# baaivision/Painter

Measured on AMD Instinct MI355X. Metric: images/sec (896x448 pairs) ViT-L fwd+bwd, higher is better.
Workload: dtype bf16; 1 GPU; painter_vit_large_patch16_input896x448 bf16 batch=8/GPU fwd+bwd on 1xMI355X (BASELINE configs[1]); global_batch=8, image=896x448x3 stitched pair, mode=train (DropPath 0.1), parallelism=dp1, rccl_ranks=0, backend=n/a, grad_allreduce=n/a

## Files before the change

### include/painter_hip.h

```cpp
#ifndef PAINTER_HIP_H
#define PAINTER_HIP_H

#include <stdint.h>

#ifdef __cplusplus
extern "C" {
#endif

#ifndef __HIP__
typedef struct ihipStream_t* hipStream_t;
#endif

enum { PA_F32 = 0, PA_BF16 = 1 };
enum {
    PA_EPI_BIAS = 0,
    PA_EPI_BIAS_F32 = 1,
    PA_EPI_BIAS_GELU = 2,
    PA_EPI_BIAS_RESID = 3
};

#define PA_ABI_VERSION 9
int pa_abi_version(void);
int pa_debug_set(int which, int value);
int pa_debug_get(int which);

int pa_linear_fwd(int dtype, int epilogue, const void* x , int64_t ldx, const void* w ,
                  const float* bias , void* out, void* out2, int64_t ldo, const float* resid ,
                  const float* rowscale , int rows_per_sample, int M, int N, int K,
                  hipStream_t stream);
int pa_linear_fwd_skip(int dtype, int epilogue, const void* x, int64_t ldx, const void* w, const float* bias, void* out, void* out2,
                       int64_t ldo, const float* resid, const float* rowscale, int rows_per_sample, int M, int N, int K,
                       const float* rowskip, int skip_rows_per_sample, hipStream_t stream);
int pa_linear_pixshuf(int dtype, const void* x, int64_t ldx, const void* w , const float* bias,
                      void* out_nhwc, int batch, int Hp, int Wp, int P, int C, int K, hipStream_t stream);
int64_t pa_linear_dgrad_workspace_bytes(int M, int K);
int pa_linear_dgrad(int dtype, const void* dy , int64_t lddy, const void* w ,
                    const void* gelu_aux , void* dx , int64_t lddx, float* dx_colsum,
                    void* workspace, int M, int N, int K, hipStream_t stream);
int pa_linear_dgrad_skip(int dtype, const void* dy, int64_t lddy, const void* w, const void* gelu_aux, void* dx, int64_t lddx, float* dx_colsum,
                         void* workspace, int M, int N, int K, const float* rowskip , int skip_rows_per_sample,
                         hipStream_t stream);
int64_t pa_linear_wgrad_workspace_bytes(int dtype, int M, int N, int K);
int pa_linear_wgrad(int dtype, const void* dy , int64_t lddy, const void* x , int64_t ldx,
                    float* dw , void* workspace, int M, int N, int K, hipStream_t stream);
int64_t pa_colsum_workspace_bytes(int M, int N);
int pa_colsum(int dtype, const void* x , int64_t ld, int M, int N, float* out , void* workspace,
              hipStream_t stream);
int pa_slab_reduce(const float* in, float* out, int64_t n, int nz, int64_t stride, int accumulate, hipStream_t stream);

int pa_layernorm_fwd(int dtype, const float* x, int64_t ldx, const float* gamma, const float* beta, float eps,
                     void* y , int64_t ldy, float* mean, float* rstd,
                     int R, int D, hipStream_t stream);
int64_t pa_layernorm_bwd_workspace_bytes(int R, int D);
int pa_layernorm_bwd(int dtype, const void* dy, int64_t lddy, const float* x, int64_t ldx, const float* mean,
                     const float* rstd, const float* gamma, const float* dres, float* dx, int64_t lddx, void* dxT,
                     int64_t lddxT, const float* rowscale, int rows_per_sample, float* dgamma_dbeta, float* dxT_colsum,
                     void* workspace, int R, int D, hipStream_t stream);
int pa_layernorm_bwd_reduce(const void* workspace, float* dgamma_dbeta, float* dxT_colsum, int with_colsum, int R, int D,
                            hipStream_t stream);

int pa_relpos_rows_padded(int Hp, int Wp);
int pa_relpos_pack(int dtype, const float* rel_pos_h, const float* rel_pos_w, void* rcat, int Hp, int Wp, int head_dim,
                   hipStream_t stream);
int pa_relpos_pack_batch(int dtype, const void* tabs, void* rcat, void* rcatT, int nblocks, int Hp, int Wp, int head_dim, hipStream_t stream);
int64_t pa_attn_tables_bytes(int dtype, int batch, int L, int heads, int Hp, int Wp, int head_dim);
int pa_attn_set_generation(int generation);
int pa_attn_launch_counts(long long* out6);
int pa_attn_trace(int enable, unsigned long long* host_out);
int pa_attn_fwd(int dtype, const void* qkv, int64_t ldq, const void* rcat, void* out, int64_t ldo, float* lse,
                void* tables, int batch, int L, int heads, int Hp, int Wp, int head_dim, float scale, hipStream_t stream);
int pa_attn_fwd_skip(int dtype, const void* qkv, int64_t ldq, const void* rcat, void* out, int64_t ldo, float* lse,
                     void* tables, int batch, int L, int heads, int Hp, int Wp, int head_dim, float scale, const float* rowskip ,
                     hipStream_t stream);

int pa_relpos_pack_t(int dtype, const float* rel_pos_h, const float* rel_pos_w, void* rcatT, int Hp, int Wp, int head_dim,
                     hipStream_t stream);
int pa_attn_bwd_delta(int dtype, const void* out, int64_t ldo, const void* dout, int64_t lddo, float* delta, int batch,
                      int L, int heads, int head_dim, hipStream_t stream);
int pa_attn_bwd_prep_ok(int dtype, int L, int Hp, int Wp, int head_dim);
int pa_attn_bwd_prep(int dtype, const void* out, int64_t ldo, const void* dout, int64_t lddo, const float* lse, void* tables,
                     int batch, int L, int heads, int Hp, int Wp, int head_dim, float scale, hipStream_t stream);
int64_t pa_attn_bwd_aux_bytes(int batch, int L, int heads, int Hp, int Wp);
int64_t pa_attn_bwd_relpos_partials_bytes(int dtype, int batch, int L, int heads, int Hp, int Wp, int head_dim);
int pa_attn_bwd(int dtype, const void* qkv, int64_t ldq, const void* rcat, const void* rcatT, const void* dout,
                int64_t lddo, const float* lse, const float* delta, void* dqkv, void* dG, void* relpos_part, void* aux,
                void* tables, const void* out, int64_t ldo, int batch, int L, int heads, int Hp, int Wp, int head_dim, float scale,
                hipStream_t stream);
int pa_attn_bwd_skip(int dtype, const void* qkv, int64_t ldq, const void* rcat, const void* rcatT, const void* dout,
                     int64_t lddo, const float* lse, const float* delta, void* dqkv, void* dG, void* relpos_part, void* aux,
                     void* tables, const void* out, int64_t ldo, int batch, int L, int heads, int Hp, int Wp, int head_dim, float scale,
                     const float* rowskip , hipStream_t stream);
int64_t pa_attn_bwd_relpos_workspace_bytes(int dtype, int batch, int L, int heads, int Hp, int Wp, int head_dim);
int pa_attn_bwd_relpos_reduce(const void* relpos_part, float* drcat, void* workspace, int batch, int L, int heads, int Hp, int Wp,
                              int head_dim, hipStream_t stream);
int pa_attn_bwd_relpos(int dtype, const void* dG, const void* qkv, int64_t ldq, float* drcat, void* workspace,
                       int batch, int L, int heads, int Hp, int Wp, int head_dim, hipStream_t stream);

int pa_patch_weight_pack(int dtype, const float* w , void* out , int D, int P, hipStream_t stream);
int pa_patch_embed_fwd(int dtype, const float* imgs, const float* tgts, const void* w, int64_t ldw, const float* bias,
                       const float* mask_token, const float* seg_x, const float* seg_y, const float* pos,
                       const unsigned char* mask, int mask_batch_stride, const float* type_cls, const float* type_ins,
                       const float* seg_type, float* tokens, int batch, int Hp, int Wp, int P, int D, hipStream_t stream);
int pa_patch_cols_ok(int batch, int L, int P, int D);
int pa_patch_im2col(const float* imgs, const float* tgts, void* cols, int batch, int Hp, int Wp, int P, hipStream_t stream);
int pa_patch_embed_fwd_cols(const void* cols, const void* w , int64_t ldw, const float* bias, const float* mask_token,
                            const float* seg_x, const float* seg_y, const float* pos, const unsigned char* mask, int mask_batch_stride,
                            const float* type_cls, const float* type_ins, const float* seg_type, float* tokens, int batch, int L, int K,
                            int D, hipStream_t stream);
int64_t pa_patch_embed_wgrad_workspace_bytes(int D, int P);
int pa_patch_embed_wgrad(int dtype, const void* dpe , const float* imgs, const float* tgts,
                         float* dw , void* workspace, int batch, int Hp, int Wp, int P, int D,
                         hipStream_t stream);
int pa_patch_embed_dgrad(int dtype, const void* dpe, const void* w, int64_t ldw, float* dimgs, float* dtgts, const float* addend,
                         float alpha, int batch, int Hp, int Wp, int P, int D, hipStream_t stream);
int pa_pos_fwd(const int* idx , const float* val , int K, const float* pe , float* pos , int L, int D,
               hipStream_t stream);
int pa_pos_bwd(const int* idxT , const float* valT , int KT, const float* gx , const float* gy ,
               float* dpe , int S, int D, hipStream_t stream);
int pa_tokens_bwd(int dtype, const float* dx0, const unsigned char* mask, int mask_batch_stride, void* dpe, float* sums,
                  int batch, int L, int D, hipStream_t stream);

int pa_merge_fwd(const float* x, float* out, int64_t n_out, hipStream_t stream);
int pa_merge_bwd(int dtype, const float* dmerged, float* dx, void* dxT, const float* rowscale, int rows_per_sample,
                 int64_t rows_half, int D, hipStream_t stream);
int pa_scale_cast(int dtype, const float* in, void* out, const float* rowscale, int rows_per_sample, int64_t rows, int D,
                  hipStream_t stream);
int pa_cast_bf16(const float* in, void* out, int64_t n, hipStream_t stream);
int pa_debug_rmw(const float* src, float* scratch, int64_t n, int passes, int nblocks, hipStream_t stream);
int pa_ensemble_resid(const float* x0, const float* a, float* x1, int batch, int group, int L, int D, hipStream_t stream);

int pa_conv3x3_pack(int dtype, const float* w3 , void* w3r , void* wf ,
                    hipStream_t stream);
int pa_decoder_tail_fwd(int dtype, const void* x_nhwc, const void* w3r, const float* b3, const float* ln_gamma,
                        const float* ln_beta, const float* w1 , const float* b1, void* y3 ,
                        float* pred , int batch, int Hi, int Wi, float eps, hipStream_t stream);
int64_t pa_decoder_tail_bwd_workspace_bytes(int batch, int Hi, int Wi);
int pa_decoder_tail_bwd_pointwise(int dtype, const float* dpred, const void* y3, const float* ln_gamma,
                                  const float* ln_beta, const float* w1, void* dy3, float* grads, void* workspace,
                                  int batch, int Hi, int Wi, float eps, hipStream_t stream);
int pa_conv3x3_dgrad_unshuffle(int dtype, const void* dy3, const void* wf, void* dE, int batch, int Hp, int Wp, int P,
                               hipStream_t stream);
int64_t pa_conv3x3_wgrad_workspace_bytes(int batch, int Hi, int Wi);
int pa_conv3x3_wgrad(int dtype, const void* dy3, const void* x_nhwc, float* dw , void* workspace,
                     int batch, int Hi, int Wi, hipStream_t stream);

int pa_live_rows_max(void);
int pa_live_rows(const unsigned char* mask, int mask_batch_stride, int* rowmap, int* live, int* count, int batch, int Hp, int Wp,
                 hipStream_t stream);
int pa_conv3x3_dgrad_unshuffle_live(const void* dy3, const void* wf, void* dE_compact, const int* rowmap, const int* count, int batch,
                                    int Hp, int Wp, int P, hipStream_t stream);
int pa_gather_rows(const void* src, int64_t src_row_bytes, void* dst, int64_t dst_row_bytes, int64_t row_bytes, const int* live,
                   const int* count, int M, hipStream_t stream);
int pa_linear_dgrad_live(const void* dy, int64_t lddy, const void* w, void* dx, int64_t lddx, const int* live, const int* rowmap,
                         const int* count, int M, int N, int K, hipStream_t stream);
int pa_linear_wgrad_live(const void* dy, int64_t lddy, const void* x, int64_t ldx, float* dw, const int* count, int M, int N, int K,
                         hipStream_t stream);
int pa_colsum_live(int dtype, const void* x, int64_t ld, int M, int N, float* out, void* workspace, const int* count, hipStream_t stream);
int pa_fill_dead_rows(void* x, int64_t pitch_bytes, int64_t row_bytes, const int* rowmap, int M, hipStream_t stream);
int pa_decoder_live_ok(int dtype, int batch, int Hp, int Wp, int P, int Kin);

int64_t pa_loss_workspace_bytes(int batch, int Hi, int Wi);
int pa_loss_fwd(const float* pred, const float* tgts, float* valid, const unsigned char* mask, int mask_batch_stride,
                float* out, void* workspace, int batch, int Hi, int Wi, int P, int ignore_rule, float eps_den, int kind,
                float beta, hipStream_t stream);
int pa_loss_bwd(const float* pred, const float* tgts, const float* valid, const unsigned char* mask,
                int mask_batch_stride, const float* dloss, const float* loss_out, float* dpred, int batch, int Hi, int Wi,
                int P, int kind, float beta, hipStream_t stream);
int pa_patchify(const float* img, float* out, int batch, int Hp, int Wp, int P, hipStream_t stream);
int pa_pred_bwd(const float* pred, const float* tgts, const float* valid, const unsigned char* mask, int mask_batch_stride,
                const float* dloss, const float* loss_out, const float* dpatch, float* dpred, float* dpred_loss, int batch, int Hi,
                int Wi, int P, int kind, float beta, hipStream_t stream);

typedef struct PaOptTensor {
    void* p; const void* g; void* m; void* v;
    void* w16;
    int64_t n;
    int32_t group;
    int32_t first_chunk;
} PaOptTensor;
typedef struct PaOptGroups {
    float lr[64], wd[64];
} PaOptGroups;
int pa_opt_chunk_elems(void);
int64_t pa_grad_sumsq_workspace_bytes(int nchunks);
int pa_grad_sumsq(const PaOptTensor* table, int ntensors, int nchunks, float* out2, void* workspace, hipStream_t stream);
int pa_adamw_step(const PaOptTensor* table, int ntensors, int nchunks, const PaOptGroups* groups, double beta1, double beta2,
                  float eps, float* steps, const float* norm_info, const float* grad_scale, const float* found_inf,
                  float max_norm, hipStream_t stream);

int pa_resample_u8(const void* src, int src_h, int src_w, void* dst, int dst_h, int dst_w, int channels, const void* bounds,
                   const void* coeffs, int ksize, int vertical, hipStream_t stream);
int pa_gather_u8(const void* src, int src_h, int src_w, void* dst, int dst_h, int dst_w, int channels, const void* ytab,
                 const void* xtab, hipStream_t stream);
int pa_seggpt_stitch(const void* prompts, const void* targets, const void* target_div, const void* query, float* imgs,
                     float* tgts, int n_prompts, int res_h, int res_w, hipStream_t stream);
int pa_seggpt_decode(const float* pred, void* out_f64, int res_h, int res_w, int patch, hipStream_t stream);
int pa_seggpt_mask(const float* pred, void* out_u8, int res_h, int res_w, int patch, hipStream_t stream);
int pa_seggpt_blend(const float* pred, const void* image, void* out, int out_h, int out_w, const void* ytab, const void* xtab,
                    int res_h, int res_w, int patch, hipStream_t stream);

int pa_resample_u8_box(const void* src, int64_t src_row_bytes, int src_h, int src_w, void* dst, int dst_h, int dst_w, int channels,
                       const void* bounds, const void* coeffs, int ksize, int vertical, hipStream_t stream);
int pa_gather_u8_box(const void* src, int64_t src_row_bytes, int src_h, int src_w, void* dst, int dst_h, int dst_w, int channels,
                     const void* ytab, const void* xtab, hipStream_t stream);
int64_t pa_color_jitter_workspace_bytes(int batch);
int pa_color_jitter(void* images, const void* ops, const void* factors, const void* ops_host, void* workspace, int batch, int h, int w,
                    hipStream_t stream);
int pa_to_tensor_normalize(const void* images, const void* flip, float* canvas, int batch, int h, int w, int canvas_h, int row0,
                           hipStream_t stream);
int pa_resized_crop_f32(const float* src, float* dst, const void* boxes, int batch, int channels, int h, int w, int nearest,
                        hipStream_t stream);
int pa_resized_crop_f32_modes(const float* src, float* dst, const void* boxes, const void* modes, int batch, int channels, int h, int w,
                              hipStream_t stream);
typedef struct pa_crop_job {
    const void* src;
    void* dst;
    const void* xbounds;
    const void* xcoeffs;
    const void* ybounds;
    const void* ycoeffs;
    int64_t src_row_bytes;
    int32_t h, w;
    int32_t xksize, yksize;
    int32_t nearest;
    int32_t mid_row0;
} pa_crop_job;
int pa_resized_crop_u8_batch(const pa_crop_job* jobs, void* mid, int n_jobs, int max_h, int max_w, int out_h, int out_w, hipStream_t stream);
int64_t pa_pair_valid_workspace_bytes(int batch);
int pa_pair_valid(const float* tgts, float* valid, const void* modes, const void* thres, void* workspace, int batch, int plane,
                  hipStream_t stream);

int pa_painter_stitch(const void* prompt, const void* prompt_target, const void* queries, float* imgs, float* tgts, int n_queries,
                      int res_h, int res_w, hipStream_t stream);
typedef struct pa_decode_job {
    void* out;
    void* out2;
    int32_t sample;
    int32_t out_h, out_w;
    int32_t reserved;
} pa_decode_job;
int pa_painter_decode_u8(const float* pred, const pa_decode_job* jobs, int n_jobs, int n_samples, int max_h, int max_w, int res_h,
                         int res_w, int patch, int nearest, hipStream_t stream);
int pa_painter_decode_depth(const float* pred, const pa_decode_job* jobs, int n_jobs, int n_samples, int max_h, int max_w, int res_h,
                            int res_w, int patch, hipStream_t stream);
int pa_painter_decode_f64(const float* pred, const pa_decode_job* jobs, int n_jobs, int n_samples, int max_h, int max_w, int res_h,
                          int res_w, int patch, hipStream_t stream);
int pa_palette_argmin(const void* image, const float* palette, void* out_i32, int h, int w, int n_colours, int dist_type,
                      hipStream_t stream);
int64_t pa_inst_workspace_bytes(int h, int w, int n_colours, int n_thr, int nms_pre);
int64_t pa_inst_workspace_offset(int h, int w, int n_colours, int n_thr, int nms_pre, int section);
int pa_inst_stats(const void* image, const float* palette, const float* thresholds, void* n_u32, void* s_u64, int h, int w, int n_colours,
                  int n_thr, hipStream_t stream);
int pa_inst_intersections(const void* masks_u32, int n_rows, int words, void* inter_i32, int ld, hipStream_t stream);
int pa_inst_decode(const void* image, const float* palette, const float* thresholds, int h, int w, int n_colours, int n_thr, int nms_pre,
                   int max_num, float sigma, int kernel, void* workspace, void* out_count, float* out_scores, void* out_scores_f64,
                   void* out_candidates, void* out_masks, void* out_masks_u8, hipStream_t stream);

typedef struct pa_pano_segment {
    int id;
    int isthing;
    int category_id;
    int instance_id;
    int area;
    float score;
} pa_pano_segment;
int64_t pa_pano_workspace_bytes(int h, int w, int n_colours, int n_things, int max_inst);
int pa_pack_mask_bits(const void* masks_u8, int n_rows, int h, int w, void* out_u32, hipStream_t stream);
int pa_pano_vote(const void* image, const float* palette, const void* masks_u32, const void* n_dev, int h, int w, int n_colours, int n_things,
                 int dist_type, int max_inst, void* out_s_u64, void* out_classes, hipStream_t stream);
int pa_pano_merge(const void* semmap_i32, const void* masks_u32, const float* scores, const void* classes_i32, const void* n_dev, int h, int w,
                  int n_colours, int n_things, int max_inst, double overlap_threshold, double stuff_area_thresh, double instances_score_thresh,
                  void* workspace, void* out_panoptic, void* out_rgb, void* out_count, void* out_segments, hipStream_t stream);
int pa_pano_decode(const void* image, const float* palette, const void* masks_u32, const float* scores, const void* n_dev,
                   const void* classes_i32, int h, int w, int n_colours, int n_things, int dist_type, int max_inst, double overlap_threshold,
                   double stuff_area_thresh, double instances_score_thresh, void* workspace, void* out_panoptic, void* out_rgb, void* out_count,
                   void* out_segments, void* out_classes, hipStream_t stream);

int64_t pa_pose_workspace_bytes(int n, int n_keypoints);
int pa_pose_keypoints(const void* pictures, const void* flipped, const void* palette_i32, const void* pair_i32, int n, int h, int w,
                      int n_keypoints, int shift, void* workspace, float* out_preds, float* out_maxvals, hipStream_t stream);
int pa_pose_heatmaps(const void* pictures, const void* flipped, const void* palette_i32, const void* pair_i32, int n, int h, int w,
                     int n_keypoints, int shift, float* out_heatmaps, hipStream_t stream);

typedef struct pa_score_job {
    const void* picture;
    const void* gt;
    int32_t h, w;
} pa_score_job;
int pa_semseg_lds_bins(int n_colours);
int pa_semseg_confusion(const pa_score_job* jobs, int n_jobs, int64_t total_pixels, const float* palette, int n_colours, int dist_type,
                        int ignore_label, int bins, void* conf_i64, void* invalid_i64, hipStream_t stream);
typedef struct pa_depth_job {
// ... 50 lines not shown
```

### painter_amd/csrc/attn3.h

```cpp
#pragma once
#include "common.h"
bool attn3_ok(int L, int Hp, int Wp);
int64_t attn3_table_bytes(int Bn, int L, int H, int Hp, int Wp);
int attn3_fwd(const bf16* qkv, int64_t ldq, const bf16* rcat, bf16* out, int64_t ldo, float* lse, void* tables, int Bn, int L, int H,
              int Hp, int Wp, float scale, hipStream_t st, const float* rowskip = nullptr);
int attn3_bwd(const bf16* qkv, int64_t ldq, const bf16* rcatT, const bf16* dout, int64_t lddo, const float* lse, const float* delta,
              void* tables, bf16* dqkv, bf16* dG, float* part, int Bn, int L, int H, int Hp, int Wp, float scale, const bf16* out, int64_t ldo,
              hipStream_t st, const float* rowskip = nullptr);
int attn3_bwd_prep(const bf16* out, int64_t ldo, const bf16* dout, int64_t lddo, const float* lse, void* tables, int Bn, int L, int H, int Hp,
                   float scale, hipStream_t st);
int64_t attn3_relpos_partials_bytes(int Bn, int L, int H, int Hp, int Wp);
int attn3_relpos_reduce(const float* part, float* drcat, float* tmp, int Bn, int L, int H, int Hp, int Wp, hipStream_t st);
```

### painter_amd/csrc/attn3.hip

```cpp
#include "attn3_common.h"
#include "../../include/painter_hip.h"
#include "attn3.h"
#include <cstdlib>

#ifndef A3_PRIO
#define A3_PRIO 0
#endif
#ifndef A3_HOIST
#define A3_HOIST 1
#endif
#ifndef A3_NDL
#define A3_NDL true
#endif
#define A3_PRIO_UP() do { if (A3_PRIO) __builtin_amdgcn_s_setprio(1); } while (0)
#define A3_PRIO_DOWN() do { if (A3_PRIO) __builtin_amdgcn_s_setprio(0); } while (0)

namespace a3 {

template <int STAGES, bool SKIP = false>
__global__ __launch_bounds__(NT, STAGES == 1 ? 4 : 2) void fwd_kernel(const bf16* __restrict__ qkv, size_t ldq, const bf16* __restrict__ rcat,
                                                                      bf16* __restrict__ out, size_t ldo, float* __restrict__ lse,
                                                                      unsigned char* __restrict__ tables, int L, int H, int Hp, int NRP,
                                                                      float scale, int nblk, int xcd_map, int abl, const float* __restrict__ rowskip) {
    extern __shared__ __attribute__((aligned(16))) unsigned char smem[];
// ... 4 lines not shown
    else wg_coords(nblk, xcd_map, blk, bh, (L / 32) / NW);
    const int b = bh / H, h = bh % H, D = H * ATT_HD;
    const bf16* base = qkv + (size_t)b * L * ldq + h * ATT_HD;
    const bf16* kbase = base + D;
    const bf16* vbase = base + 2 * D;
    const int qt = blk * NW + wave;
    const bool valid = qt * 32 < L && !drop;
    const int q = qt * 32 + ql;
    const int ntile = L / 32;
    unsigned char* thT = smem + STAGES * STAGE_QK + wave * Hp * 64;
    unsigned char* eimg = smem + STAGES * STAGE_QK + NW * Hp * 64;
    unsigned char* twimg = eimg + wave * 2048;
    LaneAddr la;
    la.init(lane);
    EAddr ea;
    ea.init(lane);
    Stager ks, vs;
    ks.load(kbase, ldq, tid);
    vs.load(vbase, ldq, tid);

    bf16x8 qf[4];
    uint4 T0 = zero4(), T1 = zero4();
    if (valid) {
#pragma unroll
        for (int s = 0; s < 4; ++s) qf[s] = gfrag(base + (size_t)q * ldq, s, g);
        if (!(abl & 32)) build_tables3(twimg, thT, rcat, NRP, qf, q / WP, q % WP, Hp, 1.f / scale, lane, smem + tid * 2);
        T0 = *reinterpret_cast<const uint4*>(twimg + ql * 64 + 16 * g);
        T1 = *reinterpret_cast<const uint4*>(twimg + ql * 64 + 32 + 16 * g);
        if (tables != nullptr) {
            unsigned char* tt = tables + ((size_t)bh * ntile + qt) * ttile_bytes(Hp);
#pragma unroll
            for (int i = 0; i < 2; ++i) *reinterpret_cast<uint4*>(tt + (lane + 64 * i) * 16) = *reinterpret_cast<const uint4*>(twimg + (lane + 64 * i) * 16);
            for (int c = lane; c < Hp * 4; c += 64) *reinterpret_cast<uint4*>(tt + 2048 + c * 16) = *reinterpret_cast<const uint4*>(thT + c * 16);
        }
    }
    __syncthreads();
    build_eimg(eimg, tid);
    ks.store(smem, tid);
    vs.store(smem + IMG, tid);
    __syncthreads();

    f32x16 oacc[2];
    oacc[0] = zero16();
    oacc[1] = zero16();
    float m = 0.f, l = 0.f;
    const float sl = scale * LOG2E_F;
    const unsigned char* thw = thT + ql * 2;

    auto body = [&](auto pc, int a) {
        constexpr int P = decltype(pc)::value;
        const int j = a * PH + P;
        {
            const int jn = min(j + 1, ntile - 1);
            ks.load(kbase + (size_t)jn * 32 * ldq, ldq, tid);
            vs.load(vbase + (size_t)jn * 32 * ldq, ldq, tid);
        }
        const unsigned char* kimg = smem + (STAGES == 2 ? (j & 1) * STAGE_QK : 0);
        const unsigned char* vimg = kimg + IMG;
        if (valid) {
            const unsigned char* thr = thw + a * (RPP * 64);
            if constexpr (P == 0) win_set<0>(T1.w, thr);
            win_set<(P + 1) & 1>(T1.w, thr + (P + 1) * 64);
            const unsigned char* ei = eimg + P * EIMG;
            const bf16x8 ef0 = efrag(ei, ea, 0), ef1 = efrag(ei, ea, 1);
            bf16x8 kfr[4];
#pragma unroll
            for (int s = 0; s < 4; ++s) kfr[s] = rowfrag(kimg, la, s);
            __builtin_amdgcn_sched_barrier(0);
            f32x16 sacc = zero16();
            A3_PRIO_UP();
            sacc = mfma(ef0, as_frag(T0), sacc);
            sacc = mfma(ef1, as_frag(T1), sacc);
#pragma unroll
            for (int s = 0; s < 4; ++s) sacc = mfma(kfr[s], qf[s], sacc);
            A3_PRIO_DOWN();
            bf16x8 vtr[2][2];
            vtr[0][0] = trfrag(vimg, la, 0, 0);
            vtr[0][1] = trfrag(vimg, la, 0, 1);
            if constexpr (STAGES == 2) { vtr[1][0] = trfrag(vimg, la, 1, 0); vtr[1][1] = trfrag(vimg, la, 1, 1); }
            __builtin_amdgcn_sched_barrier(0);
            float p[16];
            const float nm = -m;
#pragma unroll
            for (int r = 0; r < 16; ++r) p[r] = fmaf(sacc[r], sl, nm);
            float tmax = max16(p);
            tmax = fmaxf(tmax, xor32(tmax));
            if (j == 0 || __any(tmax > THR)) {
                const float delta = (j == 0) ? tmax : fmaxf(tmax, 0.f);
                const float alpha = __builtin_amdgcn_exp2f(-delta);
                m += delta;
                l *= alpha;
#pragma unroll
                for (int r = 0; r < 16; ++r) { oacc[0][r] *= alpha; oacc[1][r] *= alpha; p[r] -= delta; }
            }
#pragma unroll
            for (int r = 0; r < 16; ++r) p[r] = __builtin_amdgcn_exp2f(p[r]);
            l += sum16(p);
            const bf16x8 pf0 = packfrag(p), pf1 = packfrag(p + 8);
            if constexpr (STAGES == 1) { vtr[1][0] = trfrag(vimg, la, 1, 0); vtr[1][1] = trfrag(vimg, la, 1, 1); }
            A3_PRIO_UP();
#pragma unroll
            for (int db = 0; db < 2; ++db) {
                oacc[db] = mfma(vtr[db][0], pf0, oacc[db]);
                oacc[db] = mfma(vtr[db][1], pf1, oacc[db]);
            }
            A3_PRIO_DOWN();
        }
        if constexpr (STAGES == 1) __syncthreads();
        if (j + 1 < ntile) {
            ks.store(smem + (STAGES == 2 ? ((j + 1) & 1) * STAGE_QK : 0), tid);
            vs.store(smem + (STAGES == 2 ? ((j + 1) & 1) * STAGE_QK : 0) + IMG, tid);
        }
        __syncthreads();
    };
    for (int a = 0; a < (((abl & 16) || drop) ? 0 : Hp / RPP); ++a) {
        body(std::integral_constant<int, 0>{}, a);
        body(std::integral_constant<int, 1>{}, a);
        body(std::integral_constant<int, 2>{}, a);
        body(std::integral_constant<int, 3>{}, a);
        body(std::integral_constant<int, 4>{}, a);
        body(std::integral_constant<int, 5>{}, a);
        body(std::integral_constant<int, 6>{}, a);
    }
    unsigned char* stg = smem + wave * IMG;
    if constexpr (STAGES == 1) { if (wave >= 2) stg = eimg + (wave - 2) * IMG; }
    if (valid) {
        const float lt = l + xor32(l);
        if (g == 0) {
            const float lse_q = (m + __builtin_amdgcn_logf(lt)) * LN2_F;
            lse[(size_t)bh * L + q] = lse_q;
            if (tables != nullptr) {
                unsigned char* tt = tables + ((size_t)bh * ntile + qt) * ttile_bytes(Hp);
                const float x = -lse_q * (1.f / scale);
                const bf16 hi = (bf16)x;
                *reinterpret_cast<bf16*>(tt + 2048 + Hp * 64 + ql * 2) = hi;
                *reinterpret_cast<bf16*>(tt + 2048 + (Hp + 1) * 64 + ql * 2) = (bf16)(x - (float)hi);
            }
        }
        stage_rows(stg, oacc, 1.f / lt, lane);
        write_rows(stg, out + (size_t)(b * L + qt * 32) * ldo + h * ATT_HD, ldo, lane);
    }
    if (drop && qt * 32 < L) {
        zero_rows(out + (size_t)(b * L + qt * 32) * ldo + h * ATT_HD, ldo, lane);
        if (g == 0) lse[(size_t)bh * L + q] = 0.f;
        if (tables != nullptr) {
            unsigned char* tt = tables + ((size_t)bh * ntile + qt) * ttile_bytes(Hp);
            for (int c = lane; c < ttile_bytes(Hp) / 16; c += 64) *reinterpret_cast<uint4*>(tt + c * 16) = zero4();
        }
    }
}

__device__ unsigned long long g_trace[2 * 2 * 64 * 8];
constexpr int NSMAX = 12;
template <int MINW, bool NDL, bool TR = false, bool FUSE = false>
__global__ __launch_bounds__(NT, MINW) void bwd_dq_kernel(const bf16* __restrict__ qkv, size_t ldq, const bf16* __restrict__ rcatT,
                                                          const bf16* __restrict__ dout, size_t lddo, const float* __restrict__ lse,
                                                          unsigned char* __restrict__ tables, bf16* __restrict__ dqkv,
                                                          bf16* __restrict__ dG, float* __restrict__ part, int L, int H, int Hp, int NRP,
                                                          float scale, int nblk, int xcd_map, int abl, int tile0, int pslot0,
                                                          const bf16* __restrict__ oatt, size_t ldo, const float* __restrict__ rowskip) {
    extern __shared__ __attribute__((aligned(16))) unsigned char smem[];
    const int tid = threadIdx.x, lane = tid & 63, wave = tid >> 6, g = lane >> 5, ql = lane & 31;
    const int trwg = blockIdx.x == 0 ? 0 : (blockIdx.x == gridDim.x / 2 ? 1 : -1);
    auto coarse = [&](int pt) {
        if constexpr (TR) {
            if constexpr (MINW < 3 && A3_HOIST) __builtin_amdgcn_sched_barrier(0);
            const unsigned long long t = __builtin_amdgcn_s_memtime();
            if (trwg >= 0 && wave < 2 && lane == 0) g_trace[((trwg * 2 + wave) * 64 + pt) * 8] = t;
            if constexpr (MINW < 3 && A3_HOIST) __builtin_amdgcn_sched_barrier(0);
        }
    };
    coarse(60);
    int blk, bh, pslot = blockIdx.x;
    bool drop = false;
    if (rowskip != nullptr) drop = wg_coords_skip(nblk, xcd_map, blk, bh, rowskip, H, &pslot);
    else wg_coords(nblk, xcd_map, blk, bh, (L / 32 - tile0) / NW);
    const int b = bh / H, h = bh % H, D = H * ATT_HD;
    const bf16* base = qkv + (size_t)b * L * ldq + h * ATT_HD;
    const bf16* kbase = base + D;
    const bf16* vbase = base + 2 * D;
    const int qt = tile0 + blk * NW + wave;
    const bool valid = qt * 32 < L;
    const int q = qt * 32 + ql;
    const int qh = q / WP, qw = q % WP;
    if (drop) {
        if (valid) {
            zero_rows(dqkv + (size_t)(b * L + qt * 32) * ldq + h * ATT_HD, ldq, lane);
            if (g == 0) *reinterpret_cast<float*>(tables + ((size_t)bh * (L / 32) + qt) * ttile_bytes(Hp) + 2048 + (Hp + 2) * 64 + ql * 4) = 0.f;
            if constexpr (!FUSE) {
                bf16* dgrow = dG + ((size_t)(b * L + qt * 32) * H + h) * NRP;
                for (int c = lane; c < 32 * (NRP / 8); c += 64)
                    *reinterpret_cast<uint4*>(dgrow + (size_t)(c / (NRP / 8)) * H * NRP + (c % (NRP / 8)) * 8) = zero4();
            }
        }
        if constexpr (FUSE) {
            float4* pw = reinterpret_cast<float4*>(part + (size_t)(pslot0 + pslot) * NRP * ATT_HD);
            for (int c = tid; c < NRP * ATT_HD / 4; c += NT) pw[c] = make_float4(0.f, 0.f, 0.f, 0.f);
        }
        return;
    }
    unsigned char* thT = smem + 2 * STAGE_QK + wave * Hp * 64;
    unsigned char* eimg = smem + 2 * STAGE_QK + NW * Hp * 64;
    unsigned char* rimg = eimg + PH * EIMG;
    const int rpitch = NRP * 2 + 16;
    LaneAddr la;
    la.init(lane);
    EAddr ea;
    ea.init(lane);
    const int ntile = L / 32;
    const float sl = scale * LOG2E_F;
    Stager ks, vs;
    ks.load(kbase, ldq, tid);
    vs.load(vbase, ldq, tid);
    const int rchunks = ATT_HD * (NRP / 8);

    bf16x8 qf[4], dof[4];
    uint4 T0 = zero4(), T1 = zero4();
    uint4 tch[4] = {zero4(), zero4(), zero4(), zero4()};
    float nlse2 = 0.f, ndlt = 0.f;
    unsigned char* tt = tables + ((size_t)bh * ntile + qt) * ttile_bytes(Hp);
    if (valid) {
#pragma unroll
        for (int s = 0; s < 4; ++s) {
            qf[s] = gfrag(base + (size_t)q * ldq, s, g);
            dof[s] = gfrag(dout + (size_t)(b * L + q) * lddo + h * ATT_HD, s, g);
        }
        if (oatt != nullptr) {
            float dl = 0.f;
#pragma unroll
            for (int s = 0; s < 4; ++s) {
                const bf16x8 of = gfrag(oatt + (size_t)(b * L + q) * ldo + h * ATT_HD, s, g);
#pragma unroll
                for (int t = 0; t < 8; ++t) dl = fmaf((float)of[t], (float)dof[s][t], dl);
            }
            dl += xor32(dl);
            ndlt = -dl;
            if (g == 0) *reinterpret_cast<float*>(tt + 2048 + (Hp + 2) * 64 + ql * 4) = ndlt;
        }
        T0 = *reinterpret_cast<const uint4*>(tt + ql * 64 + 16 * g);
        T1 = *reinterpret_cast<const uint4*>(tt + ql * 64 + 32 + 16 * g);
#pragma unroll
        for (int i = 0; i < 4; ++i)
            if (lane + 64 * i < Hp * 4) tch[i] = *reinterpret_cast<const uint4*>(tt + 2048 + (lane + 64 * i) * 16);
        nlse2 = -lse[(size_t)bh * L + q] * LOG2E_F;
        if (oatt == nullptr) ndlt = *reinterpret_cast<const float*>(tt + 2048 + (Hp + 2) * 64 + ql * 4);
    }
    build_eimg(eimg, tid);
    {
        const int per_row = NRP / 8;
        for (int c = tid; c < rchunks; c += 2 * NT) {
            const int c2 = c + NT;
            const uint4 v0 = *reinterpret_cast<const uint4*>(rcatT + (size_t)c * 8);
            const uint4 v1 = c2 < rchunks ? *reinterpret_cast<const uint4*>(rcatT + (size_t)c2 * 8) : zero4();
            *reinterpret_cast<uint4*>(rimg + (c / per_row) * rpitch + (c % per_row) * 16) = v0;
            if (c2 < rchunks) *reinterpret_cast<uint4*>(rimg + (c2 / per_row) * rpitch + (c2 % per_row) * 16) = v1;
        }
    }
    if (valid) {
#pragma unroll
        for (int i = 0; i < 4; ++i)
            if (lane + 64 * i < Hp * 4) *reinterpret_cast<uint4*>(thT + (lane + 64 * i) * 16) = tch[i];
        for (int c = lane + 256; c < Hp * 4; c += 64) *reinterpret_cast<uint4*>(thT + c * 16) = *reinterpret_cast<const uint4*>(tt + 2048 + c * 16);
    }
    f32x16 ndl;
#pragma unroll
    for (int r = 0; r < 16; ++r) ndl[r] = NDL ? ndlt : 0.f;
    ks.store(smem, tid);
    vs.store(smem + IMG, tid);
    __syncthreads();

    f32x16 dq[2], eacc;
    dq[0] = zero16();
    dq[1] = zero16();
    eacc = zero16();
    unsigned char* thw = thT + ql * 2;

    coarse(61);
    auto body = [&](auto pc, int a) {
        constexpr int P = decltype(pc)::value;
        const int j = a * PH + P;
        auto mark = [&](int pt) {
            if constexpr (TR) {
                if constexpr (MINW < 3 && A3_HOIST) __builtin_amdgcn_sched_barrier(0);
                const unsigned long long t = __builtin_amdgcn_s_memtime();
                if (trwg >= 0 && wave < 2 && lane == 0 && j < 60) g_trace[((trwg * 2 + wave) * 64 + j) * 8 + pt] = t;
                if constexpr (MINW < 3 && A3_HOIST) __builtin_amdgcn_sched_barrier(0);
            }
        };
        mark(0);
        if (j + 1 < ntile) {
            ks.load(kbase + (size_t)(j + 1) * 32 * ldq, ldq, tid);
            vs.load(vbase + (size_t)(j + 1) * 32 * ldq, ldq, tid);
        }
        const unsigned char* kimg = smem + (j & 1) * STAGE_QK;
        const unsigned char* vimg = kimg + IMG;
        if (valid) {
            unsigned char* thr = thw + a * (RPP * 64);
            if constexpr (P == 0) win_set<0>(T1.w, thr);
            win_set<(P + 1) & 1>(T1.w, thr + (P + 1) * 64);
            const unsigned char* ei = eimg + P * EIMG;
            const bf16x8 ef0 = efrag(ei, ea, 0), ef1 = efrag(ei, ea, 1);
            bf16x8 kfr[4], vfr[4];
#pragma unroll
            for (int s = 0; s < 4; ++s) { vfr[s] = rowfrag(vimg, la, s); kfr[s] = rowfrag(kimg, la, s); }
            if constexpr (MINW < 3 && A3_HOIST) __builtin_amdgcn_sched_barrier(0);
            if constexpr (TR) { asm volatile("s_waitcnt lgkmcnt(0)" ::: "memory"); }
            mark(1);
            f32x16 sacc = zero16(), dpacc;
            A3_PRIO_UP();
            sacc = mfma(ef0, as_frag(T0), sacc);
            dpacc = mfma(vfr[0], dof[0], ndl);
            sacc = mfma(ef1, as_frag(T1), sacc);
#pragma unroll
            for (int s = 1; s < 4; ++s) dpacc = mfma(vfr[s], dof[s], dpacc);
#pragma unroll
            for (int s = 0; s < 4; ++s) sacc = mfma(kfr[s], qf[s], sacc);
            A3_PRIO_DOWN();
            bf16x8 ktr[2][2], etr[2];
#pragma unroll
            for (int db = 0; db < 2; ++db) { ktr[db][0] = trfrag(kimg, la, db, 0); ktr[db][1] = trfrag(kimg, la, db, 1); }
            etr[0] = etrfrag(ei, ea, 0);
            etr[1] = etrfrag(ei, ea, 1);
            if constexpr (MINW < 3 && A3_HOIST) __builtin_amdgcn_sched_barrier(0);
            mark(2);
            float ds[16];
#pragma unroll
            for (int r = 0; r < 16; ++r) {
                const float pr = __builtin_amdgcn_exp2f(fmaf(sacc[r], sl, nlse2));
                ds[r] = NDL ? pr * dpacc[r] : pr * (dpacc[r] + ndlt);
            }
            const bf16x8 dsf0 = packfrag(ds), dsf1 = packfrag(ds + 8);
            mark(3);
            A3_PRIO_UP();
#pragma unroll
            for (int db = 0; db < 2; ++db) {
                dq[db] = mfma(ktr[db][0], dsf0, dq[db]);
                dq[db] = mfma(ktr[db][1], dsf1, dq[db]);
            }
            eacc = mfma(etr[0], dsf0, eacc);
            eacc = mfma(etr[1], dsf1, eacc);
            A3_PRIO_DOWN();
            if (g) {
                *reinterpret_cast<bf16*>(thr + P * 64) = (bf16)eacc[win_reg(P & 3)];
                eacc[win_reg(P & 3)] = 0.f;
                if constexpr (P == PH - 1) {
                    *reinterpret_cast<bf16*>(thr + (P + 1) * 64) = (bf16)eacc[win_reg((P + 1) & 3)];
                    eacc[win_reg((P + 1) & 3)] = 0.f;
                }
            }
        }
        mark(4);
        if (j + 1 < ntile) {
            ks.store(smem + ((j + 1) & 1) * STAGE_QK, tid);
            vs.store(smem + ((j + 1) & 1) * STAGE_QK + IMG, tid);
        }
        mark(5);
        __syncthreads();
        mark(6);
    };
    for (int a = 0; a < ((abl & 16) ? 0 : Hp / RPP); ++a) {
        body(std::integral_constant<int, 0>{}, a);
        body(std::integral_constant<int, 1>{}, a);
        body(std::integral_constant<int, 2>{}, a);
        body(std::integral_constant<int, 3>{}, a);
        body(std::integral_constant<int, 4>{}, a);
        body(std::integral_constant<int, 5>{}, a);
        body(std::integral_constant<int, 6>{}, a);
    }
    coarse(62);
    float* twg = reinterpret_cast<float*>(eimg + wave * (32 * WP * 4));
    unsigned char* stg = smem + wave * IMG;
    uint4 gfs[FUSE ? NSMAX : 1];
    if constexpr (FUSE) {
#pragma unroll
        for (int s = 0; s < NSMAX; ++s) gfs[s] = zero4();
    }
    if (valid) {
#pragma unroll
        for (int reg = 0; reg < 16; ++reg) {
            const int rho = acc_row(reg, lane);
            if (rho < 22) twg[ql * WP + rho] = eacc[reg];
            else if (rho >= 24 && rho < 30) twg[ql * WP + rho - 2] = eacc[reg];
        }
#pragma unroll
        for (int r = 0; r < 16; ++r) { dq[0][r] *= scale; dq[1][r] *= scale; }
        bf16* dgrow = dG + ((size_t)(b * L + q) * H + h) * NRP;
        const int nkh = 2 * Hp - 1;
        auto gather = [&](int s, float (&gv)[8]) {
            const int r0 = 16 * s + 8 * g;
            if (r0 + 7 < nkh) {
                const int kh0 = qh + Hp - 1 - r0;
                const unsigned char* base = thT + ql * 2 + (kh0 - 7) * 64;
#pragma unroll
                for (int t = 0; t < 8; ++t) {
                    const float v = (float)*reinterpret_cast<const bf16*>(base + (7 - t) * 64);
                    gv[t] = (unsigned)(kh0 - t) < (unsigned)Hp ? v : 0.f;
                }
            } else if (r0 >= nkh) {
                const int kw0 = qw + WP - 1 - (r0 - nkh);
                const float* base = twg + ql * WP + (kw0 - 7);
#pragma unroll
                for (int t = 0; t < 8; ++t) {
                    const float v = base[7 - t];
                    gv[t] = (unsigned)(kw0 - t) < (unsigned)WP ? v : 0.f;
                }
            } else {
#pragma unroll
                for (int t = 0; t < 8; ++t) {
                    const int r = r0 + t;
                    const int khh = qh + Hp - 1 - r;
                    const int kww = qw + WP - 1 - (r - nkh);
                    const bool okh = r < nkh && (unsigned)khh < (unsigned)Hp;
                    const bool okw = r >= nkh && (unsigned)kww < (unsigned)WP;
                    const float vh = (float)*reinterpret_cast<const bf16*>(thT + (okh ? khh : 0) * 64 + ql * 2);
                    const float vw = twg[ql * WP + (okw ? kww : 0)];
                    gv[t] = okh ? vh : (okw ? vw : 0.f);
                }
            }
        };
        const int nstep = NRP / 16;
        const unsigned char* r0 = rimg + ql * rpitch + 16 * g, *r1 = r0 + 32 * rpitch;
        auto rfrag = [&](const unsigned char* rp, int s) { return __builtin_bit_cast(bf16x8, *reinterpret_cast<const uint4*>(rp + 32 * s)); };
        bf16x8 rf[2] = {rfrag(r0, 0), rfrag(r1, 0)};
        float gcur[8];
        gather(0, gcur);
        auto rstep = [&](int s, uint4& keep) {
            const int sn = min(s + 1, nstep - 1);
            const bf16x8 rn[2] = {rfrag(r0, sn), rfrag(r1, sn)};
            float gnext[8];
            if (abl & 32) {
#pragma unroll
                for (int t = 0; t < 8; ++t) gnext[t] = gcur[t] + 1.f;
            } else {
                gather(sn, gnext);
            }
            const bf16x8 gf = packfrag(gcur);
            if constexpr (FUSE) keep = __builtin_bit_cast(uint4, gf);
            else if (!(abl & 2)) *reinterpret_cast<uint4*>(dgrow + 16 * s + 8 * g) = __builtin_bit_cast(uint4, gf);
#pragma unroll
            for (int db = 0; db < 2; ++db) {
                if (!(abl & 64)) dq[db] = mfma(rf[db], gf, dq[db]);
                rf[db] = rn[db];
            }
#pragma unroll
            for (int t = 0; t < 8; ++t) gcur[t] = gnext[t];
        };
        if constexpr (FUSE) {
#pragma unroll
            for (int s = 0; s < NSMAX; ++s)
                if (s < ((abl & 1) ? 0 : nstep)) rstep(s, gfs[s]);
        } else {
            uint4 none;
            for (int s = 0; s < ((abl & 1) ? 0 : nstep); ++s) rstep(s, none);
        }
        stage_rows(stg, dq, 1.f, lane);
        if (!(abl & 4)) write_rows(stg, dqkv + (size_t)(b * L + qt * 32) * ldq + h * ATT_HD, ldq, lane);
    }
    if constexpr (FUSE) {
        __syncthreads();
        const int nimg = (NRP + 63) >> 6;
        unsigned char* wimg = smem + wave * (nimg + 1) * IMG;
        if (valid) {
            const int rsw = vsw(ql);
#pragma unroll
            for (int s = 0; s < NSMAX; ++s)
                if (s < NRP / 16) *reinterpret_cast<uint4*>(wimg + (s >> 2) * IMG + ql * 128 + ((((2 * s + g) & 7) ^ rsw) << 4)) = gfs[s];
#pragma unroll
            for (int s = 0; s < 4; ++s)
                *reinterpret_cast<uint4*>(wimg + nimg * IMG + ql * 128 + (((2 * s + g) ^ rsw) << 4)) = __builtin_bit_cast(uint4, qf[s]);
        }
        __syncthreads();
        float* pw = part + (size_t)(pslot0 + pslot) * NRP * ATT_HD;
        for (int u = wave; u < 2 * (NRP / 32); u += NW) {
            const int rb = u >> 1, db = u & 1;
            f32x16 acc = zero16();
            for (int w2 = 0; w2 < NW; ++w2) {
                if ((tile0 + blk * NW + w2) * 32 >= L) break;
                const unsigned char* im = smem + w2 * (nimg + 1) * IMG;
#pragma unroll
                for (int ks = 0; ks < 2; ++ks)
                    acc = mfma(trfrag(im + (rb >> 1) * IMG, la, rb & 1, ks), trfrag(im + nimg * IMG, la, db, ks), acc);
            }
            float* pcol = pw + (size_t)(rb * 32 + 4 * g) * ATT_HD + db * 32 + ql;
#pragma unroll
            for (int reg = 0; reg < 16; ++reg) pcol[((reg & 3) + 8 * (reg >> 2)) * ATT_HD] = acc[reg];
        }
    }
    if constexpr (TR) { asm volatile("s_waitcnt vmcnt(0)" ::: "memory"); }
    coarse(63);
}

constexpr int DKV_TW = 2 * IMG, DKV_TH = DKV_TW + 2048, DKV_ND = DKV_TH + 512, DKV_STAGE = DKV_ND + 128;
template <int MINW>
__global__ __launch_bounds__(NT, MINW) void bwd_dkv_kernel(const bf16* __restrict__ qkv, size_t ldq, const bf16* __restrict__ dout,
                                                           size_t lddo, const unsigned char* __restrict__ tables, bf16* __restrict__ dqkv,
                                                           int L, int H, int Hp, float scale, int nblk, int xcd_map, int abl, int tile0,
                                                           const float* __restrict__ rowskip) {
    extern __shared__ __attribute__((aligned(16))) unsigned char smem[];
    const int tid = threadIdx.x, lane = tid & 63, wave = tid >> 6, g = lane >> 5, ql = lane & 31;
    int blk, bh;
    bool drop = false;
    if (rowskip != nullptr) drop = wg_coords_skip(nblk, xcd_map, blk, bh, rowskip, H);
    else wg_coords(nblk, xcd_map, blk, bh, (L / 32 - tile0) / NW);
    const int b = bh / H, h = bh % H, D = H * ATT_HD;
    const bf16* qbase = qkv + (size_t)b * L * ldq + h * ATT_HD;
    const bf16* dobase = dout + (size_t)b * L * lddo + h * ATT_HD;
    const int kt = tile0 + blk * NW + wave;
    const bool valid = kt * 32 < L;
    if (drop) {
        if (valid) {
            bf16* orow = dqkv + (size_t)(b * L + kt * 32) * ldq + h * ATT_HD;
            zero_rows(orow + D, ldq, lane);
            zero_rows(orow + 2 * D, ldq, lane);
        }
        return;
    }
    const int key = kt * 32 + ql;
    const int kh = key / WP, kw = key % WP;
    const int khlo = ((tile0 + blk * NW) * 32) / WP;
    const int kha = (kt * 32) / WP;
    const int ntile = L / 32;
    const int TB = ttile_bytes(Hp);
    const unsigned char* tbase = tables + (size_t)bh * ntile * TB;
    LaneAddr la;
    la.init(lane);
    EAddr ea;
    ea.init(lane);
    const float sl = scale * LOG2E_F;
    const int sa = kha & 3, sb = (kha + 1) & 3;

    bf16x8 kf[4], vf[4], eb0, eb1;
    int woff[2];
    {
        uint32_t e0[4] = {0, 0, 0, 0}, e1[4] = {0, 0, 0, 0};
#pragma unroll
        for (int t = 0; t < 8; ++t) {
            const uint32_t bit = 0x3F80u << (16 * (t & 1));
            if (kw == 8 * g + t) e0[t >> 1] |= bit;
            if (t < 6) {
                if (kw == 16 + 6 * g + t) e1[t >> 1] |= bit;
            } else {
                const int slot = 2 * g + (t - 6);
                if (slot == (kh & 3) || (slot != sa && slot != sb)) e1[t >> 1] |= bit;
            }
        }
        eb0 = __builtin_bit_cast(bf16x8, make_uint4(e0[0], e0[1], e0[2], e0[3]));
        eb1 = __builtin_bit_cast(bf16x8, make_uint4(e1[0], e1[1], e1[2], e1[3]));
#pragma unroll
        for (int hs = 0; hs < 2; ++hs) {
            const int slot = 2 * g + hs;
            int row;
            if (slot == sa) row = kha - khlo;
            else if (slot == sb) row = kha + 1 - khlo;
            else {
                int rank = 0;
                for (int s2 = 0; s2 < slot; ++s2) rank += (s2 != sa && s2 != sb) ? 1 : 0;
                row = 6 + rank;
            }
            woff[hs] = DKV_TH + row * 64 + ql * 2;
        }
    }
    if (valid) {
#pragma unroll
        for (int s = 0; s < 4; ++s) {
            kf[s] = gfrag(qbase + D + (size_t)key * ldq, s, g);
            vf[s] = gfrag(qbase + 2 * D + (size_t)key * ldq, s, g);
        }
    }
    Stager qs, dos;
    uint4 rx = zero4();
    int xsrc = 0, xdst = 0;
    if (tid < 128) {
        const int qi = tid >> 2, c = tid & 3;
        xsrc = tid * 16;
        xdst = DKV_TW + qi * 64 + ((c ^ ((qi >> 2) & 3)) << 4);
    } else if (tid < 160) {
        const int k = tid - 128, rs = k >> 2, c = k & 3;
        const int srow = rs < 6 ? min(khlo + rs, Hp - 1) : Hp + (rs - 6);
        xsrc = 2048 + srow * 64 + c * 16;
        xdst = DKV_TH + rs * 64 + c * 16;
    } else if (tid < 168) {
        xsrc = 2048 + (Hp + 2) * 64 + (tid - 160) * 16;
        xdst = DKV_ND + (tid - 160) * 16;
    }
    auto load_all = [&](int j) {
        qs.load(qbase + (size_t)j * 32 * ldq, ldq, tid);
        dos.load(dobase + (size_t)j * 32 * lddo, lddo, tid);
        if (tid < 168) rx = *reinterpret_cast<const uint4*>(tbase + (size_t)j * TB + xsrc);
    };
    auto store_all = [&](int stage) {
        unsigned char* s0 = smem + stage * DKV_STAGE;
        qs.store(s0, tid);
        dos.store(s0 + IMG, tid);
        if (tid < 168) *reinterpret_cast<uint4*>(s0 + xdst) = rx;
    };
    load_all(0);
    store_all(0);
    __syncthreads();

    f32x16 dk[2], dv[2];
    dk[0] = zero16(); dk[1] = zero16(); dv[0] = zero16(); dv[1] = zero16();

    for (int j = 0; j < ((abl & 16) ? 0 : ntile); ++j) {
        if (j + 1 < ntile) load_all(j + 1);
        const unsigned char* qimg = smem + (j & 1) * DKV_STAGE;
        const unsigned char* doimg = qimg + IMG;
        if (valid) {
            const uint4 a0 = *reinterpret_cast<const uint4*>(qimg + DKV_TW + ea.row[0]);
            uint4 a1 = *reinterpret_cast<const uint4*>(qimg + DKV_TW + ea.row[1]);
            const uint32_t wlo = *reinterpret_cast<const uint16_t*>(qimg + woff[0]);
            const uint32_t whi = *reinterpret_cast<const uint16_t*>(qimg + woff[1]);
            f32x16 dpacc;
#pragma unroll
            for (int rg = 0; rg < 4; ++rg) {
                const float4 nd = *reinterpret_cast<const float4*>(qimg + DKV_ND + (8 * rg + 4 * g) * 4);
                dpacc[rg * 4 + 0] = nd.x; dpacc[rg * 4 + 1] = nd.y; dpacc[rg * 4 + 2] = nd.z; dpacc[rg * 4 + 3] = nd.w;
            }
            bf16x8 qfr[4], dofr[4];
#pragma unroll
            for (int s = 0; s < 4; ++s) { qfr[s] = rowfrag(qimg, la, s); dofr[s] = rowfrag(doimg, la, s); }
            if constexpr (MINW < 3 && A3_HOIST) __builtin_amdgcn_sched_barrier(0);
            a1.w = wlo | (whi << 16);
            f32x16 sacc = zero16();
            A3_PRIO_UP();
            sacc = mfma(as_frag(a0), eb0, sacc);
            sacc = mfma(as_frag(a1), eb1, sacc);
#pragma unroll
            for (int s = 0; s < 4; ++s) {
                sacc = mfma(qfr[s], kf[s], sacc);
                dpacc = mfma(dofr[s], vf[s], dpacc);
            }
            A3_PRIO_DOWN();
            bf16x8 dotr[2][2], qtr[2][2];
#pragma unroll
            for (int db = 0; db < 2; ++db) {
                dotr[db][0] = trfrag(doimg, la, db, 0); dotr[db][1] = trfrag(doimg, la, db, 1);
                qtr[db][0] = trfrag(qimg, la, db, 0); qtr[db][1] = trfrag(qimg, la, db, 1);
            }
            if constexpr (MINW < 3 && A3_HOIST) __builtin_amdgcn_sched_barrier(0);
            float p[16], ds[16];
#pragma unroll
            for (int r = 0; r < 16; ++r) {
                p[r] = __builtin_amdgcn_exp2f(sacc[r] * sl);
                ds[r] = p[r] * dpacc[r];
            }
            const bf16x8 pf0 = packfrag(p), pf1 = packfrag(p + 8), dsf0 = packfrag(ds), dsf1 = packfrag(ds + 8);
            A3_PRIO_UP();
#pragma unroll
            for (int db = 0; db < 2; ++db) {
                dv[db] = mfma(dotr[db][0], pf0, dv[db]);
                dv[db] = mfma(dotr[db][1], pf1, dv[db]);
                dk[db] = mfma(qtr[db][0], dsf0, dk[db]);
                dk[db] = mfma(qtr[db][1], dsf1, dk[db]);
            }
            A3_PRIO_DOWN();
        }
        if (j + 1 < ntile) store_all((j + 1) & 1);
        __syncthreads();
    }
    unsigned char* stg = smem + wave * 2 * IMG;
    if (valid) {
        stage_rows(stg, dk, scale, lane);
        stage_rows(stg + IMG, dv, 1.f, lane);
        bf16* orow = dqkv + (size_t)(b * L + kt * 32) * ldq + h * ATT_HD;
        write_rows(stg, orow + D, ldq, lane);
        write_rows(stg + IMG, orow + 2 * D, ldq, lane);
    }
}

__global__ void prep_kernel(const float* __restrict__ lse, const float* __restrict__ delta, unsigned char* __restrict__ tables, int L, int Hp,
                            float inv_scale, int total) {
    const int idx = blockIdx.x * blockDim.x + threadIdx.x;
    if (idx >= total) return;
    const int bh = idx / L, q = idx - bh * L, qt = q >> 5, qi = q & 31;
    unsigned char* tt = tables + ((size_t)bh * (L / 32) + qt) * ttile_bytes(Hp);
    const float x = -lse[idx] * inv_scale;
    const bf16 hi = (bf16)x;
    const bf16 lo = (bf16)(x - (float)hi);
    *reinterpret_cast<bf16*>(tt + 2048 + Hp * 64 + qi * 2) = hi;
    *reinterpret_cast<bf16*>(tt + 2048 + (Hp + 1) * 64 + qi * 2) = lo;
    *reinterpret_cast<float*>(tt + 2048 + (Hp + 2) * 64 + qi * 4) = -delta[idx];
}

__global__ __launch_bounds__(256) void prep_delta_kernel(const bf16* __restrict__ o, size_t ldo, const bf16* __restrict__ d_o, size_t lddo,
                                                         const float* __restrict__ lse, unsigned char* __restrict__ tables, int R, int L, int H,
                                                         int Hp, float inv_scale) {
    const int lane = threadIdx.x & 63, wave = threadIdx.x >> 6;
    const int row = blockIdx.x * 4 + wave;
    if (row >= R) return;
    const int b = row / L, l = row - b * L, qt = l >> 5, qi = l & 31;
    const int D = H * ATT_HD, TB = ttile_bytes(Hp);
    for (int c = lane * 16; c < D; c += 1024) {
        const uint4 o0 = *reinterpret_cast<const uint4*>(o + (size_t)row * ldo + c), o1 = *reinterpret_cast<const uint4*>(o + (size_t)row * ldo + c + 8);
        const uint4 d0 = *reinterpret_cast<const uint4*>(d_o + (size_t)row * lddo + c), d1 = *reinterpret_cast<const uint4*>(d_o + (size_t)row * lddo + c + 8);
        float s = 0.f;
        const uint32_t ow[8] = {o0.x, o0.y, o0.z, o0.w, o1.x, o1.y, o1.z, o1.w}, dw[8] = {d0.x, d0.y, d0.z, d0.w, d1.x, d1.y, d1.z, d1.w};
#pragma unroll
        for (int e = 0; e < 8; ++e) {
            s += bf16_lo(ow[e]) * bf16_lo(dw[e]);
            s += bf16_hi(ow[e]) * bf16_hi(dw[e]);
        }
        s = quad_sum(s);
        if ((lane & 3) == 0) {
            const int bh = b * H + c / ATT_HD;
            unsigned char* tt = tables + ((size_t)bh * (L / 32) + qt) * TB;
            const float x = -lse[(size_t)bh * L + l] * inv_scale;
            const bf16 hi = (bf16)x;
            const bf16 lo = (bf16)(x - (float)hi);
            *reinterpret_cast<bf16*>(tt + 2048 + Hp * 64 + qi * 2) = hi;
            *reinterpret_cast<bf16*>(tt + 2048 + (Hp + 1) * 64 + qi * 2) = lo;
            *reinterpret_cast<float*>(tt + 2048 + (Hp + 2) * 64 + qi * 4) = -s;
        }
    }
}

}

int attn3_bwd_prep(const bf16* out, int64_t ldo, const bf16* dout, int64_t lddo, const float* lse, void* tables, int Bn, int L, int H, int Hp,
                   float scale, hipStream_t st) {
    const int R = Bn * L;
    PA_LAUNCH(a3::prep_delta_kernel, dim3((R + 3) / 4), dim3(256), 0, st, out, (size_t)ldo, dout, (size_t)lddo, lse,
              reinterpret_cast<unsigned char*>(tables), R, L, H, Hp, 1.f / scale);
    return (int)hipGetLastError();
}

static int g_attn_generation = 0;
extern "C" int pa_attn_set_generation(int generation) {
    if (generation != 0 && generation != 2 && generation != 3) return (int)hipErrorInvalidValue;
    g_attn_generation = generation;
    return 0;
}
static int g_attn_trace = 0;
extern "C" int pa_attn_trace(int enable, unsigned long long* host_out) {
    g_attn_trace = enable;
    if (host_out != nullptr) return (int)hipMemcpyFromSymbol(host_out, HIP_SYMBOL(a3::g_trace), sizeof(a3::g_trace));
    return 0;
}
bool attn3_ok(int L, int Hp, int Wp) {
    static const int on = [] { const char* e = getenv("PA_ATTN3"); return e ? atoi(e) : 1; }();
    return on && g_attn_generation != 2 && Wp == a3::WP && Hp % a3::RPP == 0 && Hp >= a3::RPP && L == Hp * Wp;
}
int64_t attn3_table_bytes(int Bn, int L, int H, int Hp, int Wp) {
    if (!attn3_ok(L, Hp, Wp)) return 0;
    return (int64_t)Bn * H * (L / 32) * a3::ttile_bytes(Hp);
}
static int a3_xcd_map_on() {
    static const int v = [] {
        const char* e = getenv("PA_ATTN_XCD");
        const char* l = getenv("PA_ATTN_LIGHT_LAST");
        return ((e ? atoi(e) : 1) ? 1 : 0) | ((l ? atoi(l) : 0) ? 2 : 0);
    }();
    if (g_knob[KNOB_ATTN_LIGHT_LAST] == 1) return v & 1;
    if (g_knob[KNOB_ATTN_LIGHT_LAST] == 2) return v | 2;
    return v;
}

int attn3_fwd(const bf16* qkv, int64_t ldq, const bf16* rcat, bf16* out, int64_t ldo, float* lse, void* tables, int Bn, int L, int H,
              int Hp, int Wp, float scale, hipStream_t st, const float* rowskip) {
    using namespace a3;
    const int NRP = pa_relpos_rows_padded(Hp, Wp);
    if (Bn > 63) rowskip = nullptr;
    static const int stages = [] { const char* v = getenv("PA_ATTN3_FWD_STAGES"); return v ? atoi(v) : 1; }();
    const size_t smem = (size_t)(stages == 2 ? 2 : 1) * STAGE_QK + (size_t)NW * Hp * 64 + PH * EIMG;
    static bool done1 = false, done2 = false;
    static bool done1s = false, done2s = false;
    auto kern = rowskip != nullptr ? (stages == 2 ? fwd_kernel<2, true> : fwd_kernel<1, true>) : (stages == 2 ? fwd_kernel<2> : fwd_kernel<1>);
    if (int e = set_smem(reinterpret_cast<const void*>(kern), rowskip != nullptr ? (stages == 2 ? done2s : done1s) : (stages == 2 ? done2 : done1))) return e;
    const int nblk = (L / 32 + NW - 1) / NW;
    PA_LAUNCH(kern, dim3(nblk * Bn * H), dim3(NT), smem, st, qkv, (size_t)ldq, rcat, out, (size_t)ldo, lse,
              reinterpret_cast<unsigned char*>(tables), L, H, Hp, NRP, scale, nblk, a3_xcd_map_on(), [] { const char* v = getenv("PA_ATTN3_FWD_ABL"); return v ? atoi(v) : 0; }(), rowskip);
    return (int)hipGetLastError();
}

namespace a3 {
constexpr int RED_ZC = 32;
__global__ __launch_bounds__(256) void relpos_part_reduce_kernel(const float4* __restrict__ part, float4* __restrict__ tmp, int n4, int nz) {
    __shared__ float4 sh[4][64];
    const int c = blockIdx.x * 64 + (threadIdx.x & 63), zl = threadIdx.x >> 6;
    const int z0 = (int)((int64_t)nz * blockIdx.y / gridDim.y), z1 = (int)((int64_t)nz * (blockIdx.y + 1) / gridDim.y);
    float4 s = make_float4(0, 0, 0, 0);
    if (c < n4) {
#pragma unroll 4
        for (int z = z0 + zl; z < z1; z += 4) {
            const float4 v = part[(size_t)z * n4 + c];
            s.x += v.x; s.y += v.y; s.z += v.z; s.w += v.w;
        }
    }
    sh[zl][threadIdx.x & 63] = s;
    __syncthreads();
    if (zl == 0 && c < n4) {
        float4 t = sh[0][threadIdx.x];
#pragma unroll
        for (int k = 1; k < 4; ++k) { const float4 v = sh[k][threadIdx.x]; t.x += v.x; t.y += v.y; t.z += v.z; t.w += v.w; }
        tmp[(size_t)blockIdx.y * n4 + c] = t;
    }
}
}
extern "C" int pa_slab_reduce(const float* in, float* out, int64_t n, int nz, int64_t stride, int accumulate, hipStream_t st);
static int a3_fuse_on() {
    static const int v = [] { const char* e = getenv("PA_ATTN3_FUSE_RELPOS"); return e ? atoi(e) : 1; }();
    return g_knob[KNOB_ATTN3_FUSE] == 1 ? 0 : (g_knob[KNOB_ATTN3_FUSE] == 2 ? 1 : v);
}
static int a3_blocks(int L) { return (L / 32 + a3::NW - 1) / a3::NW; }
static int64_t a3_num_partials(int Bn, int L, int H, int, int) { return (int64_t)a3_blocks(L) * Bn * H; }
int64_t attn3_relpos_partials_bytes(int Bn, int L, int H, int Hp, int Wp) {
    if (!a3_fuse_on() || !attn3_ok(L, Hp, Wp)) return 0;
    const int NRP = pa_relpos_rows_padded(Hp, Wp);
    if (NRP > 16 * a3::NSMAX) return 0;
    return a3_num_partials(Bn, L, H, Hp, Wp) * NRP * ATT_HD * sizeof(float);
}
int attn3_relpos_reduce(const float* part, float* drcat, float* tmp, int Bn, int L, int H, int Hp, int Wp, hipStream_t st) {
    using namespace a3;
    const int NRP = pa_relpos_rows_padded(Hp, Wp);
    const int nz = (int)a3_num_partials(Bn, L, H, Hp, Wp), n4 = NRP * ATT_HD / 4;
    const int zc = nz < RED_ZC ? nz : RED_ZC;
    PA_LAUNCH(relpos_part_reduce_kernel, dim3((n4 + 63) / 64, zc), dim3(256), 0, st, reinterpret_cast<const float4*>(part),
              reinterpret_cast<float4*>(tmp), n4, nz);
    if (int e = (int)hipGetLastError()) return e;
    return pa_slab_reduce(tmp, drcat, (int64_t)n4 * 4, zc, (int64_t)n4 * 4, 0, st);
}

int attn3_bwd(const bf16* qkv, int64_t ldq, const bf16* rcatT, const bf16* dout, int64_t lddo, const float* lse, const float* delta,
              void* tables, bf16* dqkv, bf16* dG, float* part, int Bn, int L, int H, int Hp, int Wp, float scale, const bf16* out, int64_t ldo,
              hipStream_t st, const float* rowskip) {
    using namespace a3;
    const int NRP = pa_relpos_rows_padded(Hp, Wp);
    if (part != nullptr && NRP > 16 * NSMAX) return (int)hipErrorInvalidValue;
    if (Bn > 63) rowskip = nullptr;
    if (part == nullptr && dG == nullptr) return (int)hipErrorInvalidValue;
    unsigned char* tb = reinterpret_cast<unsigned char*>(tables);
    int e;
    if (delta != nullptr) {
        const int total = Bn * H * L;
        PA_LAUNCH(prep_kernel, dim3((total + 255) / 256), dim3(256), 0, st, lse, delta, tb, L, Hp, 1.f / scale, total);
        if ((e = (int)hipGetLastError())) return e;
    }
    const int tile0 = 0;
    const int nblk = a3_blocks(L);
    static const int dq_w = [] { const char* v = getenv("PA_ATTN3_DQ_WAVES"); return v ? atoi(v) : 2; }();
    static const int dkv_w = [] { const char* v = getenv("PA_ATTN3_DKV_WAVES"); return v ? atoi(v) : 2; }();
    if (nblk > 0) {
        static const size_t pad = [] { const char* v = getenv("PA_ATTN3_LDS_PAD"); return v ? (size_t)atoi(v) : (size_t)0; }();
        size_t smem = 2 * (size_t)STAGE_QK + (size_t)NW * Hp * 64 + PH * EIMG + (size_t)ATT_HD * (NRP * 2 + 16) + pad;
        const bool fuse = part != nullptr;
        if (fuse) {
            const size_t need = (size_t)NW * ((NRP + 63) / 64 + 1) * IMG;
            if (smem < need) smem = need;
        }
        auto kern = fuse ? bwd_dq_kernel<2, A3_NDL, false, true>
                         : (g_attn_trace ? bwd_dq_kernel<2, true, true> : (dq_w == 3 ? bwd_dq_kernel<3, false> : bwd_dq_kernel<2, A3_NDL>));
        static bool done2 = false, done3 = false, donet = false, donef = false;
        if ((e = set_smem(reinterpret_cast<const void*>(kern), fuse ? donef : (g_attn_trace ? donet : (dq_w == 3 ? done3 : done2))))) return e;
        const char* ablv = getenv("PA_ATTN3_DQ_ABL");
        PA_LAUNCH(kern, dim3(nblk * Bn * H), dim3(NT), smem, st, qkv, (size_t)ldq, rcatT, dout, (size_t)lddo, lse, tb, dqkv, dG, part, L, H,
                  Hp, NRP, scale, nblk, a3_xcd_map_on(), ablv ? atoi(ablv) : 0, tile0, 0, delta == nullptr ? out : nullptr, (size_t)ldo, rowskip);
        if ((e = (int)hipGetLastError())) return e;
    }
    const int tile0_kv = 0, nblk_kv = a3_blocks(L);
    if (nblk_kv > 0) {
        size_t smem = 2 * (size_t)DKV_STAGE;
        if (smem < (size_t)NW * 2 * IMG) smem = (size_t)NW * 2 * IMG;
        static const size_t pad = [] { const char* v = getenv("PA_ATTN3_LDS_PAD"); return v ? (size_t)atoi(v) : (size_t)0; }();
        smem += pad;
        auto kern = dkv_w == 3 ? bwd_dkv_kernel<3> : bwd_dkv_kernel<2>;
        static bool done2 = false, done3 = false;
        if ((e = set_smem(reinterpret_cast<const void*>(kern), dkv_w == 3 ? done3 : done2))) return e;
        PA_LAUNCH(kern, dim3(nblk_kv * Bn * H), dim3(NT), smem, st, qkv, (size_t)ldq, dout, (size_t)lddo, tb, dqkv, L, H, Hp, scale, nblk_kv,
                  a3_xcd_map_on(), [] { const char* v = getenv("PA_ATTN3_DKV_ABL"); return v ? atoi(v) : 0; }(), tile0_kv, rowskip);
        if ((e = (int)hipGetLastError())) return e;
    }
    return 0;
}
```

### painter_amd/csrc/attn_bwd.hip

```cpp
#include "attn_common.h"
#include <cstdlib>
#include "gemm_engine.h"
#include "../../include/painter_hip.h"
#include "attn2.h"
#include "attn3.h"

template <typename T> DEVI void load16(const T* p, float* v);
template <> DEVI void load16<bf16>(const bf16* p, float* v) {
    const uint4 a = *reinterpret_cast<const uint4*>(p), b = *reinterpret_cast<const uint4*>(p + 8);
    v[0] = bf16_lo(a.x); v[1] = bf16_hi(a.x); v[2] = bf16_lo(a.y); v[3] = bf16_hi(a.y);
    v[4] = bf16_lo(a.z); v[5] = bf16_hi(a.z); v[6] = bf16_lo(a.w); v[7] = bf16_hi(a.w);
    v[8] = bf16_lo(b.x); v[9] = bf16_hi(b.x); v[10] = bf16_lo(b.y); v[11] = bf16_hi(b.y);
    v[12] = bf16_lo(b.z); v[13] = bf16_hi(b.z); v[14] = bf16_lo(b.w); v[15] = bf16_hi(b.w);
}
template <> DEVI void load16<float>(const float* p, float* v) {
#pragma unroll
    for (int i = 0; i < 4; ++i) {
        const float4 a = *reinterpret_cast<const float4*>(p + 4 * i);
        v[4 * i] = a.x; v[4 * i + 1] = a.y; v[4 * i + 2] = a.z; v[4 * i + 3] = a.w;
    }
}
template <typename T, bool VEC>
__global__ __launch_bounds__(256) void attn_delta_kernel(const T* o, size_t ldo, const T* d_o, size_t lddo, float* delta, int R, int L, int H, int hd) {
    __shared__ float part[4][128];
// ... 437 lines not shown
    if (head_dim <= 0 || head_dim % 16) return (int)hipErrorInvalidValue;
    const int NRP = pa_relpos_rows_padded(Hp, Wp);
    const int n = NRP * head_dim;
    if (dtype == PA_BF16)
        PA_LAUNCH(relpos_pack_t_kernel<bf16>, dim3((n + 255) / 256), dim3(256), 0, st, rel_pos_h, 2 * Hp - 1, rel_pos_w, 2 * Wp - 1, (bf16*)rcatT, NRP, head_dim);
    else
        PA_LAUNCH(relpos_pack_t_kernel<float>, dim3((n + 255) / 256), dim3(256), 0, st, rel_pos_h, 2 * Hp - 1, rel_pos_w, 2 * Wp - 1, (float*)rcatT, NRP, head_dim);
    LAUNCH_CHECK();
}

extern "C" int64_t pa_attn_bwd_aux_bytes(int batch, int L, int heads, int Hp, int Wp) {
    const int64_t gen1 = (int64_t)batch * heads * (L / 32) * (Hp + Wp + 2) * 32 * sizeof(float);
    const int64_t gen2 = (attn2_ok(L, Hp, Wp, 64) || attn2_ok(L, Hp, Wp, 80)) ? attn2_aux_bytes(batch, L, heads, Hp, Wp) : 0;
    return gen1 > gen2 ? gen1 : gen2;
}

template <typename T, int NW, int HD>
static int attn_bwd_dq_launch(const T* qkv, int64_t ldq, const T* rcat, const T* rcatT, const T* dout, int64_t lddo, const float* lse,
                              const float* delta, T* dqkv, T* dG, float* aux, int Bn, int L, int H, int Hp, int Wp, float scale, size_t smem,
                              int ts, hipStream_t st) {
    const int NRP = pa_relpos_rows_padded(Hp, Wp);
    auto kern = attn_bwd_dq_kernel<T, NW, HD>;
    static bool done = false;
    if (!done) {
        hipError_t e = hipFuncSetAttribute(reinterpret_cast<const void*>(kern), hipFuncAttributeMaxDynamicSharedMemorySize, 160 * 1024);
        if (e != hipSuccess) return (int)e;
        done = true;
    }
    const int qtiles = L / 32;
    PA_LAUNCH(kern, dim3((qtiles + NW - 1) / NW, Bn * H), dim3(NW * 64), smem, st, qkv, (size_t)ldq, rcat, rcatT, dout,
              (size_t)lddo, lse, delta, dqkv, dG, aux, L, H, Hp, Wp, NRP, scale, ts);
    return (int)hipGetLastError();
}

template <typename T, int HD>
static int attn_bwd_t(const T* qkv, int64_t ldq, const T* rcat, const T* rcatT, const T* dout, int64_t lddo, const float* lse,
                      const float* delta, T* dqkv, T* dG, float* aux, int Bn, int L, int H, int Hp, int Wp, float scale, hipStream_t st) {
    typedef KvTile<T, HD> KV;
    const int TS = Hp + Wp;
    const int qtiles = L / 32;
    {
        int ts = 2 * 32 * TS * 4;
        const int stg = 32 * HD * (int)sizeof(T);
        if (ts < stg) ts = stg;
        ts = (ts + 15) / 16 * 16;
        const size_t stages = 2 * (size_t)(2 * KV::KB + KV::VB);
        int e = (int)hipErrorInvalidValue;
        if (stages + 4 * (size_t)ts <= 160 * 1024) {
            e = attn_bwd_dq_launch<T, 4, HD>(qkv, ldq, rcat, rcatT, dout, lddo, lse, delta, dqkv, dG, aux, Bn, L, H, Hp, Wp, scale, stages + 4 * (size_t)ts, ts, st);
        } else if constexpr (HD != 64) {
            if (stages + 3 * (size_t)ts <= 160 * 1024)
                e = attn_bwd_dq_launch<T, 3, HD>(qkv, ldq, rcat, rcatT, dout, lddo, lse, delta, dqkv, dG, aux, Bn, L, H, Hp, Wp, scale, stages + 3 * (size_t)ts, ts, st);
        }
        if (e) return e;
    }
    {
        constexpr int NW = 4;
        const int AUXB = (TS + 2) * AUX_LD * 4;
        size_t smem = 2 * (size_t)(2 * KV::KB + 2 * KV::VB + AUXB);
        const size_t stg = (size_t)NW * 2 * 32 * HD * sizeof(T);
        if (smem < stg) smem = stg;
        if (smem > 160 * 1024 || (TS + 2) * 8 > (HD == 64 ? 3 : 4) * NW * 64) return (int)hipErrorInvalidValue;
        auto kern = attn_bwd_dkv_kernel<T, NW, HD>;
        static bool done = false;
        if (!done) {
            hipError_t e = hipFuncSetAttribute(reinterpret_cast<const void*>(kern), hipFuncAttributeMaxDynamicSharedMemorySize, 160 * 1024);
            if (e != hipSuccess) return (int)e;
            done = true;
        }
        PA_LAUNCH(kern, dim3((qtiles + NW - 1) / NW, Bn * H), dim3(NW * 64), smem, st, qkv, (size_t)ldq, dout, (size_t)lddo,
                           aux, dqkv, L, H, Hp, Wp, scale);
        return (int)hipGetLastError();
    }
}

extern "C" int pa_attn_bwd_prep_ok(int dtype, int L, int Hp, int Wp, int head_dim) {
    return (dtype == PA_BF16 && head_dim == ATT_HD && L == Hp * Wp && attn3_ok(L, Hp, Wp)) ? 1 : 0;
}
extern "C" int pa_attn_bwd_prep(int dtype, const void* out, int64_t ldo, const void* dout, int64_t lddo, const float* lse, void* tables,
                                int batch, int L, int heads, int Hp, int Wp, int head_dim, float scale, hipStream_t st) {
    if (!pa_attn_bwd_prep_ok(dtype, L, Hp, Wp, head_dim) || tables == nullptr || ldo % 8 || lddo % 8) return (int)hipErrorInvalidValue;
    return attn3_bwd_prep((const bf16*)out, ldo, (const bf16*)dout, lddo, lse, tables, batch, L, heads, Hp, scale, st);
}
extern "C" int64_t pa_attn_bwd_relpos_partials_bytes(int dtype, int batch, int L, int heads, int Hp, int Wp, int head_dim) {
    if (dtype != PA_BF16 || head_dim != ATT_HD || L != Hp * Wp) return 0;
    return attn3_relpos_partials_bytes(batch, L, heads, Hp, Wp);
}
extern "C" int pa_attn_bwd_skip(int dtype, const void* qkv, int64_t ldq, const void* rcat, const void* rcatT, const void* dout, int64_t lddo,
                                const float* lse, const float* delta, void* dqkv, void* dG, void* relpos_part, void* aux, void* tables,
                                const void* out, int64_t ldo, int batch, int L, int heads, int Hp, int Wp, int head_dim, float scale,
                                const float* rowskip, hipStream_t st) {
    if (L != Hp * Wp || L % 32 || Hp % 4 || Wp % 4 || (head_dim != 64 && head_dim != 80)) return (int)hipErrorInvalidValue;
    if (dtype == PA_BF16 && head_dim == ATT_HD && tables != nullptr && attn3_ok(L, Hp, Wp)) {
        if (relpos_part != nullptr && attn3_relpos_partials_bytes(batch, L, heads, Hp, Wp) == 0) return (int)hipErrorInvalidValue;
        ++g_attn_counts[5];
        if (out != nullptr && ldo % 8) return (int)hipErrorInvalidValue;
        return attn3_bwd((const bf16*)qkv, ldq, (const bf16*)rcatT, (const bf16*)dout, lddo, lse, delta, tables, (bf16*)dqkv, (bf16*)dG,
                         (float*)relpos_part, batch, L, heads, Hp, Wp, scale, (const bf16*)out, ldo, st, drop_skip_on() ? rowskip : nullptr);
    }
    if (relpos_part != nullptr || dG == nullptr || delta == nullptr) return (int)hipErrorInvalidValue;
    if (dtype == PA_BF16 && attn2_ok(L, Hp, Wp, head_dim)) {
        ++g_attn_counts[4];
        return attn2_bwd((const bf16*)qkv, ldq, (const bf16*)rcat, (const bf16*)rcatT, (const bf16*)dout, lddo, lse, delta, (bf16*)dqkv,
                         (bf16*)dG, aux, batch, L, heads, Hp, Wp, head_dim, scale, st);
    }
    ++g_attn_counts[3];
#define PA_ATTN_BWD(TT_, HD_) attn_bwd_t<TT_, HD_>((const TT_*)qkv, ldq, (const TT_*)rcat, (const TT_*)rcatT, (const TT_*)dout, lddo, lse, delta, \
                                                   (TT_*)dqkv, (TT_*)dG, (float*)aux, batch, L, heads, Hp, Wp, scale, st)
    if (dtype == PA_BF16) return head_dim == 80 ? PA_ATTN_BWD(bf16, 80) : PA_ATTN_BWD(bf16, 64);
    return head_dim == 80 ? PA_ATTN_BWD(float, 80) : PA_ATTN_BWD(float, 64);
#undef PA_ATTN_BWD
}
extern "C" int pa_attn_bwd(int dtype, const void* qkv, int64_t ldq, const void* rcat, const void* rcatT, const void* dout, int64_t lddo,
                           const float* lse, const float* delta, void* dqkv, void* dG, void* relpos_part, void* aux, void* tables,
                           const void* out, int64_t ldo, int batch, int L, int heads, int Hp, int Wp, int head_dim, float scale, hipStream_t st) {
    return pa_attn_bwd_skip(dtype, qkv, ldq, rcat, rcatT, dout, lddo, lse, delta, dqkv, dG, relpos_part, aux, tables, out, ldo, batch, L, heads, Hp, Wp,
                            head_dim, scale, nullptr, st);
}

extern "C" int64_t pa_attn_bwd_relpos_workspace_bytes(int dtype, int batch, int L, int heads, int Hp, int Wp, int head_dim) {
    const int NRP = pa_relpos_rows_padded(Hp, Wp);
    return (int64_t)heads * 32 * NRP * head_dim * sizeof(float);
}
template <typename T>
static int relpos_grad_t(const T* dG, const T* qkv, int64_t ldq, float* drcat, float* ws, int Bn, int L, int H, int NRP, int hd, hipStream_t st) {
    const int R = Bn * L;
    OpT<T> A{dG, (size_t)H * NRP, NRP, (size_t)NRP};
    OpT<T> B{qkv, (size_t)ldq, hd, (size_t)hd};
    const int nku = (R + TT<T>::BK - 1) / TT<T>::BK;
    static const int want = [] { const char* v = getenv("PA_RELPOS_SPLITS"); return v ? atoi(v) : 16; }();
    static const bool from_env = getenv("PA_RELPOS_SPLITS") != nullptr;
    int splits = (!from_env && g_knob[KNOB_RELPOS_SPLITS] > 0) ? g_knob[KNOB_RELPOS_SPLITS] : want;
    if (splits > 32) splits = 32;
    if (splits < 1) splits = 1;
    if (splits > nku) splits = nku;
    struct Epi {
        float* out; size_t slab; int M, N;
        DEVI void operator()(const f32x16 (&acc)[2][2], int ib, int jb, int lane, int z) const {
            float* o = out + (size_t)z * slab;
            foreach_acc(acc, ib, jb, lane, [&](int i, int j, float v) {
                if (i < M && j < N) o[(size_t)i * N + j] = v;
            });
        }
    };
    int e = launch_gemm<T, 2, 2>(A, B, Epi{ws, (size_t)NRP * hd, NRP, hd}, NRP, hd, R, splits, H, st);
    if (e) return e;
    return pa_slab_reduce(ws, drcat, (int64_t)NRP * hd, splits * H, (int64_t)NRP * hd, 0, st);
}
extern "C" int pa_attn_bwd_relpos_reduce(const void* relpos_part, float* drcat, void* workspace, int batch, int L, int heads, int Hp, int Wp,
                                         int head_dim, hipStream_t st) {
    if (head_dim != ATT_HD || relpos_part == nullptr || attn3_relpos_partials_bytes(batch, L, heads, Hp, Wp) == 0) return (int)hipErrorInvalidValue;
    return attn3_relpos_reduce((const float*)relpos_part, drcat, (float*)workspace, batch, L, heads, Hp, Wp, st);
}
extern "C" int pa_attn_bwd_relpos(int dtype, const void* dG, const void* qkv, int64_t ldq, float* drcat, void* workspace, int batch, int L,
                                  int heads, int Hp, int Wp, int head_dim, hipStream_t st) {
    if (head_dim <= 0 || head_dim % 16) return (int)hipErrorInvalidValue;
    const int NRP = pa_relpos_rows_padded(Hp, Wp);
    if (dtype == PA_BF16) return relpos_grad_t<bf16>((const bf16*)dG, (const bf16*)qkv, ldq, drcat, (float*)workspace, batch, L, heads, NRP, head_dim, st);
    return relpos_grad_t<float>((const float*)dG, (const float*)qkv, ldq, drcat, (float*)workspace, batch, L, heads, NRP, head_dim, st);
}
```

### painter_amd/csrc/attn_tile.h

```cpp
#pragma once
#include "attn_common.h"

namespace atile {

constexpr int NW = 4, NT = 256, ROWS = 128, IMG = 4096, STAGE_QK = 2 * IMG;
typedef __attribute__((ext_vector_type(4))) short s16x4;
typedef __attribute__((address_space(3))) s16x4 lds_s16x4;
typedef __attribute__((ext_vector_type(2))) uint32_t u32x2;
typedef __attribute__((ext_vector_type(8))) float f32x8;

DEVI int xcd_run(int n, int total) {
    const int xq = total >> 3, xr = total & 7, xcd = n & 7;
    return (xcd < xr ? xcd * (xq + 1) : xr * (xq + 1) + (xcd - xr) * xq) + (n >> 3);
}
DEVI void wg_coords(int nblk, int xcd_map, int& blk, int& bh, int nfull = 0) {
    const int n = blockIdx.x, total = gridDim.x;
    if ((xcd_map & 2) && nfull > 0 && nfull < nblk) {
        const int nbh = total / nblk, heavy = nfull * nbh;
        if (n < heavy) {
            const int v = (xcd_map & 1) ? xcd_run(n, heavy) : n;
            bh = v / nfull;
            blk = v - bh * nfull;
        } else {
            const int m = n - heavy, per = nblk - nfull, lt = nbh * per;
            const int v = (xcd_map & 1) ? xcd_run(m, lt) : m;
            bh = v / per;
            blk = nfull + (v - bh * per);
        }
        return;
    }
    const int v = (xcd_map & 1) ? xcd_run(n, total) : n;
    bh = v / nblk;
    blk = v - bh * nblk;
}

DEVI bool wg_coords_skip(int nblk, int xcd_map, int& blk, int& bh, const float* __restrict__ rowskip, int H, int* slot = nullptr) {
    const int n = blockIdx.x, total = gridDim.x, per = nblk * H, ns = total / per;
    const int lane = threadIdx.x & 63;
    const float fv = lane < ns ? rowskip[lane] : 1.f;
    const unsigned long long dmask = __ballot(fv == 0.f);
    const int nk = (ns - __builtin_popcountll(dmask)) * per;
    const bool drop = n >= nk;
    const int v = drop ? n - nk : ((xcd_map & 1) ? xcd_run(n, nk) : n);
    const int rank = v / per, rem = v - rank * per;
    int b = rank;
    if (dmask != 0) {
        unsigned long long m = drop ? dmask : ~dmask;
        for (int c = 0; c < rank; ++c) m &= m - 1;
        b = __builtin_ctzll(m);
    }
    bh = b * H + rem / nblk;
    blk = rem % nblk;
    if (slot != nullptr) {
        const int u = bh * nblk + blk;
        if (xcd_map & 1) {
            const int xq = total >> 3, xr = total & 7, lim = xr * (xq + 1);
            const int c = u < lim ? u / (xq + 1) : xr + (u - lim) / xq;
            const int o = u < lim ? u - c * (xq + 1) : (u - lim) - (c - xr) * xq;
            *slot = o * 8 + c;
        } else {
            *slot = u;
        }
    }
    return drop;
}

DEVI int vsw(int row) { return (((row >> 1) & 1) << 2) | (((row >> 2) & 1) << 1) | ((row >> 3) & 1); }

struct Stager {
    uint4 r;
    DEVI void load(const bf16* src, size_t ld, int tid) { r = *reinterpret_cast<const uint4*>(src + (size_t)(tid >> 3) * ld + (tid & 7) * 8); }
    DEVI void store(unsigned char* img, int tid) const {
        const int row = tid >> 3, c = tid & 7;
        *reinterpret_cast<uint4*>(img + row * 128 + ((c ^ vsw(row)) << 4)) = r;
    }
};

struct LaneAddr {
    int rowbase, t;
    int tr[2][2];
    DEVI void init(int lane) {
        const int row = lane & 31, g = lane >> 5;
        rowbase = row * 128;
        t = vsw(row) ^ g;
        const int i = lane & 15, half = (lane >> 4) & 1;
#pragma unroll
        for (int db = 0; db < 2; ++db)
#pragma unroll
            for (int hi = 0; hi < 2; ++hi) {
                const int r = 4 * g + (i >> 2) + 8 * hi;
                const int chunk = 4 * db + 2 * half + ((i & 3) >> 1);
                tr[db][hi] = r * 128 + ((chunk ^ vsw(r)) << 4) + (i & 1) * 8;
            }
    }
};
DEVI bf16x8 rowfrag(const unsigned char* img, const LaneAddr& a, int s) {
    return __builtin_bit_cast(bf16x8, *reinterpret_cast<const uint4*>(img + a.rowbase + (((2 * s) ^ a.t) << 4)));
}
DEVI u32x2 ldtr(const unsigned char* p) {
    return __builtin_bit_cast(u32x2, __builtin_amdgcn_ds_read_tr16_b64_v4i16((lds_s16x4*)p));
}
DEVI bf16x8 trfrag(const unsigned char* img, const LaneAddr& a, int db, int s) {
    const u32x2 l = ldtr(img + a.tr[db][0] + s * 2048), h = ldtr(img + a.tr[db][1] + s * 2048);
    return __builtin_bit_cast(bf16x8, __builtin_shufflevector(l, h, 0, 1, 2, 3));
}
DEVI bf16x8 gfrag(const bf16* p, int s, int g) { return __builtin_bit_cast(bf16x8, *reinterpret_cast<const uint4*>(p + 16 * s + 8 * g)); }
DEVI bf16x8 packfrag(const float* v) {
    const f32x8 f = {v[0], v[1], v[2], v[3], v[4], v[5], v[6], v[7]};
    return __builtin_convertvector(f, bf16x8);
}
DEVI float xor32(float v) {
    const uint32_t u = __builtin_bit_cast(uint32_t, v);
    const auto r = __builtin_amdgcn_permlane32_swap(u, u, false, false);
    return __builtin_bit_cast(float, (threadIdx.x & 32) ? r[0] : r[1]);
}
DEVI float max3f(float a, float b, float c) { return fmaxf(fmaxf(a, b), c); }
DEVI float max16(const float* p) {
    const float a = max3f(p[0], p[1], p[2]), b = max3f(p[3], p[4], p[5]), c = max3f(p[6], p[7], p[8]), d = max3f(p[9], p[10], p[11]),
                e = max3f(p[12], p[13], p[14]);
    return max3f(max3f(a, b, c), max3f(d, e, p[15]), -INFINITY);
}
DEVI float sum16(const float* p) {
    float a = p[0] + p[4], b = p[1] + p[5], c = p[2] + p[6], d = p[3] + p[7];
    a += p[8]; b += p[9]; c += p[10]; d += p[11];
    a += p[12]; b += p[13]; c += p[14]; d += p[15];
    return (a + b) + (c + d);
}
DEVI f32x16 mfma(bf16x8 a, bf16x8 b, f32x16 c) { return __builtin_amdgcn_mfma_f32_32x32x16_bf16(a, b, c, 0, 0, 0); }

DEVI void stage_rows(unsigned char* stg, const f32x16 (&acc)[2], float mul, int lane) {
    const int g = lane >> 5;
#pragma unroll
    for (int db = 0; db < 2; ++db)
#pragma unroll
        for (int rg = 0; rg < 4; ++rg) {
            const int d0 = db * 32 + 8 * rg + 4 * g;
            *reinterpret_cast<uint2*>(stg + (lane & 31) * 128 + d0 * 2) =
                make_uint2(pack_bf16x2(acc[db][rg * 4] * mul, acc[db][rg * 4 + 1] * mul), pack_bf16x2(acc[db][rg * 4 + 2] * mul, acc[db][rg * 4 + 3] * mul));
        }
}
DEVI void write_rows(const unsigned char* stg, bf16* dst, size_t ld, int lane) {
#pragma unroll
    for (int i = 0; i < 4; ++i) {
        const int c = lane + 64 * i, row = c >> 3, ch = c & 7;
        *reinterpret_cast<uint4*>(dst + (size_t)row * ld + ch * 8) = *reinterpret_cast<const uint4*>(stg + row * 128 + ch * 16);
    }
}

DEVI void zero_rows(bf16* dst, size_t ld, int lane) {
#pragma unroll
    for (int i = 0; i < 4; ++i) {
        const int c = lane + 64 * i, row = c >> 3, ch = c & 7;
        *reinterpret_cast<uint4*>(dst + (size_t)row * ld + ch * 8) = make_uint4(0, 0, 0, 0);
    }
}

static inline int set_smem(const void* kern, bool& done) {
    if (!done) {
        hipError_t e = hipFuncSetAttribute(kern, hipFuncAttributeMaxDynamicSharedMemorySize, 160 * 1024);
        if (e != hipSuccess) return (int)e;
        done = true;
    }
    return 0;
}

}
```

### painter_amd/csrc/elementwise.hip

```cpp
#include "common.h"
#include "../../include/painter_hip.h"

extern "C" int pa_slab_reduce(const float* in, float* out, int64_t n, int nz, int64_t stride, int accumulate, hipStream_t st);

__global__ void cast_bf16_kernel(const float* __restrict__ in, bf16* __restrict__ out, size_t n) {
    size_t i = ((size_t)blockIdx.x * blockDim.x + threadIdx.x) * 4;
    if (i + 4 <= n) {
        const float4 v = *reinterpret_cast<const float4*>(in + i);
        *reinterpret_cast<uint2*>(out + i) = make_uint2(pack_bf16x2(v.x, v.y), pack_bf16x2(v.z, v.w));
    } else {
        for (; i < n; ++i) out[i] = (bf16)in[i];
    }
}
extern "C" int pa_cast_bf16(const float* in, void* out, int64_t n, hipStream_t st) {
    if (n <= 0) return 0;
    PA_LAUNCH(cast_bf16_kernel, dim3((unsigned)((n + 1023) / 1024)), dim3(256), 0, st, in, (bf16*)out, (size_t)n);
    LAUNCH_CHECK();
}

__global__ __launch_bounds__(256) void sparse_rows_kernel(const int* __restrict__ idx, const float* __restrict__ val, int K, const float* __restrict__ x0,
                                                          const float* __restrict__ x1, float* __restrict__ out, int D) {
    __shared__ float red[4][64];
    const int r = blockIdx.y, cl = threadIdx.x & 63, jl = threadIdx.x >> 6, n = blockIdx.x * 64 + cl;
    float acc = 0.f;
    if (n < D) {
        for (int j = jl; j < K; j += 4) {
            const float m = val[(size_t)r * K + j];
            if (m == 0.f) continue;
            const size_t o = (size_t)idx[(size_t)r * K + j] * D + n;
            acc = fmaf(m, x1 ? x0[o] + x1[o] : x0[o], acc);
        }
    }
    red[jl][cl] = acc;
    __syncthreads();
    if (jl == 0 && n < D) out[(size_t)r * D + n] = (red[0][cl] + red[1][cl]) + (red[2][cl] + red[3][cl]);
}
extern "C" int pa_pos_fwd(const int* idx, const float* val, int K, const float* pe, float* pos, int L, int D, hipStream_t st) {
    if (K < 1) return (int)hipErrorInvalidValue;
    PA_LAUNCH(sparse_rows_kernel, dim3((D + 63) / 64, L), dim3(256), 0, st, idx, val, K, pe, (const float*)nullptr, pos, D);
    LAUNCH_CHECK();
}
extern "C" int pa_pos_bwd(const int* idxT, const float* valT, int KT, const float* gx, const float* gy, float* dpe, int S, int D, hipStream_t st) {
    if (KT < 1) return (int)hipErrorInvalidValue;
    PA_LAUNCH(sparse_rows_kernel, dim3((D + 63) / 64, S), dim3(256), 0, st, idxT, valT, KT, gx, gy, dpe, D);
    LAUNCH_CHECK();
}

template <typename T>
__global__ void tokens_bwd_kernel(const float* __restrict__ dx0, const unsigned char* __restrict__ mask, int mbs, T* __restrict__ dpe,
                                  float* __restrict__ sums, int Bn, int L, int D) {
    const int l = blockIdx.y, n = (blockIdx.x * blockDim.x + threadIdx.x) * 4;
    if (n >= D) return;
    float4 sx = make_float4(0, 0, 0, 0), sy = sx, sm = sx;
    for (int b = 0; b < Bn; ++b) {
        const size_t rx = ((size_t)b * L + l) * D + n, ry = ((size_t)(Bn + b) * L + l) * D + n;
        const float4 gx = *reinterpret_cast<const float4*>(dx0 + rx), gy = *reinterpret_cast<const float4*>(dx0 + ry);
        const float w = mask[(size_t)b * mbs + l] ? 1.f : 0.f;
        sx.x += gx.x; sx.y += gx.y; sx.z += gx.z; sx.w += gx.w;
        sy.x += gy.x; sy.y += gy.y; sy.z += gy.z; sy.w += gy.w;
        sm.x += w * gy.x; sm.y += w * gy.y; sm.z += w * gy.z; sm.w += w * gy.w;
        const float k = 1.f - w;
        *reinterpret_cast<typename TT<T>::Vec4*>(dpe + rx) = cvt4(gx.x, gx.y, gx.z, gx.w, (T*)nullptr);
        *reinterpret_cast<typename TT<T>::Vec4*>(dpe + ry) = cvt4(gy.x * k, gy.y * k, gy.z * k, gy.w * k, (T*)nullptr);
    }
    const size_t o = (size_t)l * D + n, LD = (size_t)L * D;
    *reinterpret_cast<float4*>(sums + o) = sx;
    *reinterpret_cast<float4*>(sums + LD + o) = sy;
    *reinterpret_cast<float4*>(sums + 2 * LD + o) = sm;
}
extern "C" int pa_tokens_bwd(int dtype, const float* dx0, const unsigned char* mask, int mask_batch_stride, void* dpe, float* sums,
                             int batch, int L, int D, hipStream_t st) {
    if (D % 4) return (int)hipErrorInvalidValue;
    dim3 grid((D / 4 + 63) / 64, L);
    if (dtype == PA_BF16) PA_LAUNCH(tokens_bwd_kernel<bf16>, grid, dim3(64), 0, st, dx0, mask, mask_batch_stride, (bf16*)dpe, sums, batch, L, D);
    else PA_LAUNCH(tokens_bwd_kernel<float>, grid, dim3(64), 0, st, dx0, mask, mask_batch_stride, (float*)dpe, sums, batch, L, D);
    LAUNCH_CHECK();
}

__global__ void merge_fwd_kernel(const float* __restrict__ x, float* __restrict__ out, size_t n) {
    const size_t i = ((size_t)blockIdx.x * blockDim.x + threadIdx.x) * 4;
    if (i >= n) return;
    const float4 a = *reinterpret_cast<const float4*>(x + i), b = *reinterpret_cast<const float4*>(x + n + i);
    *reinterpret_cast<float4*>(out + i) = make_float4((a.x + b.x) * 0.5f, (a.y + b.y) * 0.5f, (a.z + b.z) * 0.5f, (a.w + b.w) * 0.5f);
}
extern "C" int pa_merge_fwd(const float* x, float* out, int64_t n_out, hipStream_t st) {
    if (n_out % 4) return (int)hipErrorInvalidValue;
    PA_LAUNCH(merge_fwd_kernel, dim3((unsigned)((n_out / 4 + 255) / 256)), dim3(256), 0, st, x, out, (size_t)n_out);
    LAUNCH_CHECK();
}
template <typename T>
__global__ void merge_bwd_kernel(const float* __restrict__ dm, float* __restrict__ dx, T* __restrict__ dxT, const float* __restrict__ rowscale,
                                 int rps, size_t rows_half, int D) {
    const size_t i = ((size_t)blockIdx.x * blockDim.x + threadIdx.x) * 4;
    const size_t n = rows_half * D;
    if (i >= n) return;
    const float4 g = *reinterpret_cast<const float4*>(dm + i);
    const float4 h = make_float4(g.x * 0.5f, g.y * 0.5f, g.z * 0.5f, g.w * 0.5f);
    *reinterpret_cast<float4*>(dx + i) = h;
    *reinterpret_cast<float4*>(dx + n + i) = h;
    const size_t row = i / D;
    const float s0 = rowscale ? rowscale[row / rps] : 1.f, s1 = rowscale ? rowscale[(row + rows_half) / rps] : 1.f;
    *reinterpret_cast<typename TT<T>::Vec4*>(dxT + i) = cvt4(h.x * s0, h.y * s0, h.z * s0, h.w * s0, (T*)nullptr);
    *reinterpret_cast<typename TT<T>::Vec4*>(dxT + n + i) = cvt4(h.x * s1, h.y * s1, h.z * s1, h.w * s1, (T*)nullptr);
}
extern "C" int pa_merge_bwd(int dtype, const float* dmerged, float* dx, void* dxT, const float* rowscale, int rows_per_sample,
                            int64_t rows_half, int D, hipStream_t st) {
    if (D % 4) return (int)hipErrorInvalidValue;
    const size_t n = (size_t)rows_half * D;
    dim3 grid((unsigned)((n / 4 + 255) / 256));
    if (dtype == PA_BF16) PA_LAUNCH(merge_bwd_kernel<bf16>, grid, dim3(256), 0, st, dmerged, dx, (bf16*)dxT, rowscale, rows_per_sample, (size_t)rows_half, D);
    else PA_LAUNCH(merge_bwd_kernel<float>, grid, dim3(256), 0, st, dmerged, dx, (float*)dxT, rowscale, rows_per_sample, (size_t)rows_half, D);
    LAUNCH_CHECK();
}
template <typename T>
__global__ void scale_cast_kernel(const float* __restrict__ in, T* __restrict__ out, const float* __restrict__ rowscale, int rps, size_t n, int D) {
    const size_t i = ((size_t)blockIdx.x * blockDim.x + threadIdx.x) * 4;
    if (i >= n) return;
    const float4 g = *reinterpret_cast<const float4*>(in + i);
    const float s = rowscale ? rowscale[(i / D) / rps] : 1.f;
    *reinterpret_cast<typename TT<T>::Vec4*>(out + i) = cvt4(g.x * s, g.y * s, g.z * s, g.w * s, (T*)nullptr);
}
extern "C" int pa_scale_cast(int dtype, const float* in, void* out, const float* rowscale, int rows_per_sample, int64_t rows, int D,
                             hipStream_t st) {
    if (D % 4) return (int)hipErrorInvalidValue;
    const size_t n = (size_t)rows * D;
    dim3 grid((unsigned)((n / 4 + 255) / 256));
    if (dtype == PA_BF16) PA_LAUNCH(scale_cast_kernel<bf16>, grid, dim3(256), 0, st, in, (bf16*)out, rowscale, rows_per_sample, n, D);
    else PA_LAUNCH(scale_cast_kernel<float>, grid, dim3(256), 0, st, in, (float*)out, rowscale, rows_per_sample, n, D);
    LAUNCH_CHECK();
}

__global__ void ensemble_resid_kernel(const float* __restrict__ x0, const float* __restrict__ a, float* __restrict__ x1, int Bn, int G,
                                      int L, int D) {
    const int l = blockIdx.y, n = (blockIdx.x * blockDim.x + threadIdx.x) * 4;
    if (n >= D) return;
    const bool ens = l >= L / 2;
    for (int g0 = 0; g0 < Bn; g0 += G) {
        float4 m = make_float4(0, 0, 0, 0);
        if (ens) {
            for (int b = g0; b < g0 + G; ++b) {
                const float4 v = *reinterpret_cast<const float4*>(a + ((size_t)b * L + l) * D + n);
                m.x += v.x; m.y += v.y; m.z += v.z; m.w += v.w;
            }
            const float inv = 1.f / (float)G;
            m.x *= inv; m.y *= inv; m.z *= inv; m.w *= inv;
        }
        for (int b = g0; b < g0 + G; ++b) {
            const size_t o = ((size_t)b * L + l) * D + n;
            const float4 r = *reinterpret_cast<const float4*>(x0 + o);
            const float4 v = ens ? m : *reinterpret_cast<const float4*>(a + o);
            *reinterpret_cast<float4*>(x1 + o) = make_float4(r.x + v.x, r.y + v.y, r.z + v.z, r.w + v.w);
        }
    }
}
extern "C" int pa_ensemble_resid(const float* x0, const float* a, float* x1, int batch, int group, int L, int D, hipStream_t st) {
    if (D % 4 || group <= 0 || batch % group) return (int)hipErrorInvalidValue;
// ... 31 lines not shown
        const int m = pix_mask(mask, mbs, b, rem, Wi, P, Wp);
        s += (tgts[(size_t)b * n + e] * c_std[c] + c_mean[c]) * (1.f - (float)m);
    }
    const float r = block_sum(s, sh);
    if (threadIdx.x == 0) part[(size_t)b * gridDim.x + blockIdx.x] = r;
}
__global__ void loss_ignore_flag_kernel(const float* __restrict__ part, int nblk, float* __restrict__ flag, float thresh) {
    __shared__ float sh[LOSS_BLK / 64];
    const int b = blockIdx.x;
    float s = 0.f;
    for (int i = threadIdx.x; i < nblk; i += LOSS_BLK) s += part[(size_t)b * nblk + i];
    const float r = block_sum(s, sh);
    if (threadIdx.x == 0) flag[b] = (r < thresh) ? 1.f : 0.f;
}
DEVI float loss_elem(float d, int kind, float beta) {
    const float a = fabsf(d);
    if (kind == 0) return a < beta ? 0.5f * d * d / beta : a - 0.5f * beta;
    if (kind == 1) return a;
    if (kind == 2) return d * d;
    return (a + d * d) * 0.5f;
}
DEVI float loss_grad_elem(float d, int kind, float beta) {
    const float sg = d > 0.f ? 1.f : (d < 0.f ? -1.f : 0.f);
    if (kind == 0) return fabsf(d) < beta ? d / beta : sg;
    if (kind == 1) return sg;
    if (kind == 2) return 2.f * d;
    return (sg + 2.f * d) * 0.5f;
}
__global__ void loss_part_kernel(const float* __restrict__ pred, const float* __restrict__ tgts, float* valid, const unsigned char* __restrict__ mask,
                                 int mbs, const float* __restrict__ flag, float* __restrict__ part, int HW, int Wi, int P, int Wp, int kind,
                                 float beta) {
    __shared__ float sh[LOSS_BLK / 64];
    const int b = blockIdx.y, n = 3 * HW;
    const bool ign = flag && flag[b] != 0.f;
    float num = 0.f, den = 0.f;
    const int e0 = blockIdx.x * LOSS_CHUNK;
    for (int e = e0 + threadIdx.x; e < min(n, e0 + LOSS_CHUNK); e += LOSS_BLK) {
        const size_t idx = (size_t)b * n + e;
        float v = valid[idx];
        if (ign) { v = 0.f; valid[idx] = 0.f; }
        const float mv = (float)pix_mask(mask, mbs, b, e % HW, Wi, P, Wp) * v;
        num += loss_elem(pred[idx] - tgts[idx], kind, beta) * mv;
        den += mv;
    }
    const float rn = block_sum(num, sh);
    const float rd = block_sum(den, sh);
    if (threadIdx.x == 0) {
        const size_t o = ((size_t)b * gridDim.x + blockIdx.x) * 2;
        part[o] = rn;
        part[o + 1] = rd;
    }
}
__global__ void loss_final_kernel(const float* __restrict__ part, int nparts, float eps_den, float* __restrict__ out) {
    __shared__ float sh[LOSS_BLK / 64];
    float num = 0.f, den = 0.f;
    for (int i = threadIdx.x; i < nparts; i += LOSS_BLK) { num += part[2 * (size_t)i]; den += part[2 * (size_t)i + 1]; }
    const float rn = block_sum(num, sh);
    const float rd = block_sum(den, sh);
    if (threadIdx.x == 0) {
        out[0] = rn / (rd + eps_den);
        out[1] = rd + eps_den;
    }
}
extern "C" int64_t pa_loss_workspace_bytes(int batch, int Hi, int Wi) {
    const int nblk = (3 * Hi * Wi + LOSS_CHUNK - 1) / LOSS_CHUNK;
    return (int64_t)batch * nblk * 3 * sizeof(float) + (int64_t)batch * sizeof(float) + 64;
}
extern "C" int pa_loss_fwd(const float* pred, const float* tgts, float* valid, const unsigned char* mask, int mask_batch_stride,
                           float* out, void* workspace, int batch, int Hi, int Wi, int P, int ignore_rule, float eps_den, int kind,
                           float beta, hipStream_t st) {
    const int HW = Hi * Wi, Wp = Wi / P;
    const int nblk = (3 * HW + LOSS_CHUNK - 1) / LOSS_CHUNK;
    float* part = reinterpret_cast<float*>(workspace);
    float* ipart = part + (size_t)batch * nblk * 2;
    float* flag = ipart + (size_t)batch * nblk;
    if (ignore_rule) {
        PA_LAUNCH(loss_ignore_part_kernel, dim3(nblk, batch), dim3(LOSS_BLK), 0, st, tgts, mask, mask_batch_stride, ipart, HW, Wi, P, Wp);
        PA_LAUNCH(loss_ignore_flag_kernel, dim3(batch), dim3(LOSS_BLK), 0, st, ipart, nblk, flag, 300.f);
    }
    PA_LAUNCH(loss_part_kernel, dim3(nblk, batch), dim3(LOSS_BLK), 0, st, pred, tgts, valid, mask, mask_batch_stride,
                       ignore_rule ? flag : (const float*)nullptr, part, HW, Wi, P, Wp, kind, beta);
    PA_LAUNCH(loss_final_kernel, dim3(1), dim3(LOSS_BLK), 0, st, part, batch * nblk, eps_den, out);
    LAUNCH_CHECK();
}
__global__ void loss_bwd_kernel(const float* __restrict__ pred, const float* __restrict__ tgts, const float* __restrict__ valid,
                                const unsigned char* __restrict__ mask, int mbs, const float* __restrict__ dloss, const float* __restrict__ lossden,
                                float* __restrict__ dpred, int HW, int Wi, int P, int Wp, int kind, float beta) {
    const int b = blockIdx.y, n = 3 * HW;
    const int e = blockIdx.x * blockDim.x + threadIdx.x;
    if (e >= n) return;
    const size_t idx = (size_t)b * n + e;
    const float mv = (float)pix_mask(mask, mbs, b, e % HW, Wi, P, Wp) * valid[idx];
    dpred[idx] = dloss[0] / lossden[1] * mv * loss_grad_elem(pred[idx] - tgts[idx], kind, beta);
}
extern "C" int pa_loss_bwd(const float* pred, const float* tgts, const float* valid, const unsigned char* mask, int mask_batch_stride,
                           const float* dloss, const float* loss_out, float* dpred, int batch, int Hi, int Wi, int P, int kind,
                           float beta, hipStream_t st) {
    const int HW = Hi * Wi;
    PA_LAUNCH(loss_bwd_kernel, dim3((3 * HW + 255) / 256, batch), dim3(256), 0, st, pred, tgts, valid, mask, mask_batch_stride,
                       dloss, loss_out, dpred, HW, Wi, P, Wi / P, kind, beta);
    LAUNCH_CHECK();
}

__global__ void pred_bwd_kernel(const float* __restrict__ pred, const float* __restrict__ tgts, const float* __restrict__ valid,
                                const unsigned char* __restrict__ mask, int mbs, const float* __restrict__ dloss, const float* __restrict__ lossden,
                                const float* __restrict__ dpatch, float* __restrict__ dpred, float* __restrict__ dpred_loss, int HW, int Wi,
                                int P, int Wp, int kind, float beta) {
    const int b = blockIdx.y, n = 3 * HW;
    const int e = blockIdx.x * blockDim.x + threadIdx.x;
    if (e >= n) return;
    const size_t idx = (size_t)b * n + e;
    float g = 0.f;
    if (dloss) {
        const float mv = (float)pix_mask(mask, mbs, b, e % HW, Wi, P, Wp) * valid[idx];
        g = dloss[0] / lossden[1] * mv * loss_grad_elem(pred[idx] - tgts[idx], kind, beta);
        if (dpred_loss) dpred_loss[idx] = g;
    }
    if (dpatch) {
        const int c = e / HW, rem = e - c * HW, y = rem / Wi, x = rem - y * Wi;
        const int L = (HW / Wi / P) * Wp, l = (y / P) * Wp + x / P, k = ((y % P) * P + x % P) * 3 + c;
        g += dpatch[((size_t)b * L + l) * (size_t)(3 * P * P) + k];
    }
    dpred[idx] = g;
}
extern "C" int pa_pred_bwd(const float* pred, const float* tgts, const float* valid, const unsigned char* mask, int mask_batch_stride,
                           const float* dloss, const float* loss_out, const float* dpatch, float* dpred, float* dpred_loss, int batch, int Hi,
                           int Wi, int P, int kind, float beta, hipStream_t st) {
    if ((dloss == nullptr && dpatch == nullptr) || (dpred_loss != nullptr && dloss == nullptr) || P < 1 || Hi % P || Wi % P)
        return (int)hipErrorInvalidValue;
    const int HW = Hi * Wi;
    PA_LAUNCH(pred_bwd_kernel, dim3((3 * HW + 255) / 256, batch), dim3(256), 0, st, pred, tgts, valid, mask, mask_batch_stride,
              dloss, loss_out, dpatch, dpred, dpred_loss, HW, Wi, P, Wi / P, kind, beta);
    LAUNCH_CHECK();
}

__global__ void patchify_kernel(const float* __restrict__ img, float* __restrict__ out, int Hp, int Wp, int P, size_t n) {
    const size_t i = (size_t)blockIdx.x * blockDim.x + threadIdx.x;
    if (i >= n) return;
    const int PP3 = P * P * 3, L = Hp * Wp;
    const int k = (int)(i % PP3);
    const size_t t = i / PP3;
    const int l = (int)(t % L), b = (int)(t / L);
    const int c = k % 3, q = (k / 3) % P, p = k / (3 * P), h = l / Wp, w = l % Wp;
    out[i] = img[(((size_t)b * 3 + c) * Hp * P + h * P + p) * (size_t)(Wp * P) + w * P + q];
}
extern "C" int pa_patchify(const float* img, float* out, int batch, int Hp, int Wp, int P, hipStream_t st) {
    const size_t n = (size_t)batch * Hp * Wp * P * P * 3;
    PA_LAUNCH(patchify_kernel, dim3((unsigned)((n + 255) / 256)), dim3(256), 0, st, img, out, Hp, Wp, P, n);
    LAUNCH_CHECK();
}

#define TAILP 324
DEVI float oct_sum(float v) { v = quad_sum(v); v += lane_dpp<0x141>(v); return v; }
template <typename T>
__global__ __launch_bounds__(256) void tail_bwd_kernel(const float* __restrict__ dpred, const T* __restrict__ y3, const float* __restrict__ gamma,
                                                       const float* __restrict__ beta, const float* __restrict__ w1, T* __restrict__ dy3,
                                                       float* __restrict__ part, int HW, int npix, float eps) {
    const int lane = threadIdx.x & 63, wave = threadIdx.x >> 6;
    const int sub = lane & 7, slot = (threadIdx.x >> 3);
    const int c0 = sub * 8;
    f32x2_t g2[4], b2[4], w2[3][4];
#pragma unroll
    for (int k = 0; k < 4; ++k) {
        g2[k] = (f32x2_t){gamma[c0 + 2 * k], gamma[c0 + 2 * k + 1]};
        b2[k] = (f32x2_t){beta[c0 + 2 * k], beta[c0 + 2 * k + 1]};
#pragma unroll
        for (int o = 0; o < 3; ++o) w2[o][k] = (f32x2_t){w1[o * 64 + c0 + 2 * k], w1[o * 64 + c0 + 2 * k + 1]};
    }
    const f32x2_t zero2 = {0.f, 0.f};
    f32x2_t ag[4] = {zero2, zero2, zero2, zero2}, ab[4] = {zero2, zero2, zero2, zero2};
    f32x2_t aw[3][4] = {{zero2, zero2, zero2, zero2}, {zero2, zero2, zero2, zero2}, {zero2, zero2, zero2, zero2}};
    float ab1[3] = {0.f, 0.f, 0.f};
    const int stride = gridDim.x * 32;
    struct In { uint4 a, b; float d0, d1, d2; };
    struct Pos { int pix, b, rem; };
    auto advance = [&](Pos& p) {
        p.pix += stride;
        p.rem += stride;
        while (p.rem >= HW) { p.rem -= HW; ++p.b; }
    };
    auto fetch = [&](const Pos& p) {
        In in;
        const int q = min(p.pix, npix - 1);
        const int bb = p.pix < npix ? p.b : (npix - 1) / HW, rr = p.pix < npix ? p.rem : (npix - 1) % HW;
        in.a = *reinterpret_cast<const uint4*>(y3 + (size_t)q * 64 + c0);
        if constexpr (sizeof(T) == 4) in.b = *reinterpret_cast<const uint4*>(y3 + (size_t)q * 64 + c0 + 4);
        else in.b = in.a;
        const float* dp = dpred + (size_t)bb * 3 * HW + rr;
        in.d0 = dp[0]; in.d1 = dp[(size_t)HW]; in.d2 = dp[(size_t)2 * HW];
        return in;
    };
    Pos cur, nxt;
    cur.pix = blockIdx.x * 32 + slot;
    cur.b = cur.pix / HW;
    cur.rem = cur.pix - cur.b * HW;
    nxt = cur;
    In in0 = fetch(nxt);
    advance(nxt);
    In in1 = fetch(nxt);
    advance(nxt);
    for (; cur.pix < npix; advance(cur)) {
        const In in = in0;
        in0 = in1;
        in1 = fetch(nxt);
        advance(nxt);
        const int pix = cur.pix;
        f32x2_t y[4];
        if constexpr (sizeof(T) == 2) {
            const uint4 raw = in.a;
            y[0] = (f32x2_t){bf16_lo(raw.x), bf16_hi(raw.x)}; y[1] = (f32x2_t){bf16_lo(raw.y), bf16_hi(raw.y)};
            y[2] = (f32x2_t){bf16_lo(raw.z), bf16_hi(raw.z)}; y[3] = (f32x2_t){bf16_lo(raw.w), bf16_hi(raw.w)};
        } else {
            y[0] = (f32x2_t){__builtin_bit_cast(float, in.a.x), __builtin_bit_cast(float, in.a.y)};
            y[1] = (f32x2_t){__builtin_bit_cast(float, in.a.z), __builtin_bit_cast(float, in.a.w)};
            y[2] = (f32x2_t){__builtin_bit_cast(float, in.b.x), __builtin_bit_cast(float, in.b.y)};
            y[3] = (f32x2_t){__builtin_bit_cast(float, in.b.z), __builtin_bit_cast(float, in.b.w)};
        }
        const float d0 = in.d0, d1 = in.d1, d2 = in.d2;
        f32x2_t s2 = (y[0] + y[1]) + (y[2] + y[3]);
        const float mu = oct_sum(s2[0] + s2[1]) * (1.f / 64);
        const f32x2_t mu2 = {mu, mu};
        f32x2_t q2 = zero2;
#pragma unroll
        for (int k = 0; k < 4; ++k) { y[k] = y[k] - mu2; q2 = __builtin_elementwise_fma(y[k], y[k], q2); }
        const float rs = 1.f / sqrtf(oct_sum(q2[0] + q2[1]) * (1.f / 64) + eps);
        const f32x2_t rs2 = {rs, rs}, dd0 = {d0, d0}, dd1 = {d1, d1}, dd2 = {d2, d2};
        f32x2_t dxh[4], m1 = zero2, m2 = zero2;
#pragma unroll
        for (int k = 0; k < 4; ++k) {
            const f32x2_t xh = y[k] * rs2;
            const f32x2_t z = __builtin_elementwise_fma(xh, g2[k], b2[k]);
            f32x2_t a, gz;
            if constexpr (sizeof(T) == 2) {
                gelu_both2(z[0], z[1], a, gz);
            } else {
                a = (f32x2_t){gelu_f(z[0]), gelu_f(z[1])};
                gz = (f32x2_t){gelu_grad_f(z[0]), gelu_grad_f(z[1])};
            }
            const f32x2_t da = __builtin_elementwise_fma(dd2, w2[2][k], __builtin_elementwise_fma(dd1, w2[1][k], dd0 * w2[0][k]));
            const f32x2_t dz = da * gz;
            ag[k] = __builtin_elementwise_fma(dz, xh, ag[k]);
            ab[k] = ab[k] + dz;
            aw[0][k] = __builtin_elementwise_fma(dd0, a, aw[0][k]);
            aw[1][k] = __builtin_elementwise_fma(dd1, a, aw[1][k]);
            aw[2][k] = __builtin_elementwise_fma(dd2, a, aw[2][k]);
            dxh[k] = dz * g2[k];
            m1 = m1 + dxh[k];
            m2 = __builtin_elementwise_fma(dxh[k], xh, m2);
            y[k] = xh;
        }
        if (sub == 0) { ab1[0] += d0; ab1[1] += d1; ab1[2] += d2; }
        const float m1s = oct_sum(m1[0] + m1[1]) * (1.f / 64), m2s = oct_sum(m2[0] + m2[1]) * (1.f / 64);
        const f32x2_t mm1 = {m1s, m1s}, nm2 = {-m2s, -m2s};
        f32x2_t r[4];
#pragma unroll
        for (int k = 0; k < 4; ++k) r[k] = rs2 * (__builtin_elementwise_fma(y[k], nm2, dxh[k]) - mm1);
        if constexpr (sizeof(T) == 2) {
            *reinterpret_cast<uint4*>(dy3 + (size_t)pix * 64 + c0) = make_uint4(pack_bf16x2(r[0][0], r[0][1]), pack_bf16x2(r[1][0], r[1][1]),
                                                                                 pack_bf16x2(r[2][0], r[2][1]), pack_bf16x2(r[3][0], r[3][1]));
        } else {
            *reinterpret_cast<float4*>(dy3 + (size_t)pix * 64 + c0) = make_float4(r[0][0], r[0][1], r[1][0], r[1][1]);
            *reinterpret_cast<float4*>(dy3 + (size_t)pix * 64 + c0 + 4) = make_float4(r[2][0], r[2][1], r[3][0], r[3][1]);
        }
    }
    auto wsum = [&](float v) { v += lane_dpp<0x128>(v); v += lane_xor16(v); v += lane_xor32(v); return v; };
    __shared__ float red[4][TAILP];
#pragma unroll
    for (int k = 0; k < 4; ++k)
#pragma unroll
        for (int e = 0; e < 2; ++e) {
            const float vg = wsum(ag[k][e]), vb = wsum(ab[k][e]), v0 = wsum(aw[0][k][e]), v1 = wsum(aw[1][k][e]), v2 = wsum(aw[2][k][e]);
            if (lane < 8) {
                const int c = c0 + 2 * k + e;
                red[wave][c] = vg; red[wave][64 + c] = vb; red[wave][128 + c] = v0; red[wave][192 + c] = v1; red[wave][256 + c] = v2;
            }
        }
    {
        const float t0 = wsum(ab1[0]), t1 = wsum(ab1[1]), t2 = wsum(ab1[2]);
        if (lane == 0) { red[wave][320] = t0; red[wave][321] = t1; red[wave][322] = t2; red[wave][323] = 0.f; }
    }
    __syncthreads();
    for (int i = threadIdx.x; i < TAILP; i += 256) part[(size_t)blockIdx.x * TAILP + i] = (red[0][i] + red[1][i]) + (red[2][i] + red[3][i]);
}
static int tail_bwd_blocks(int npix) {
    int b = (npix + 31) / 32;
    return b > 2048 ? 2048 : b;
}
extern "C" int64_t pa_decoder_tail_bwd_workspace_bytes(int batch, int Hi, int Wi) { return (int64_t)tail_bwd_blocks(batch * Hi * Wi) * TAILP * sizeof(float); }
extern "C" int pa_decoder_tail_bwd_pointwise(int dtype, const float* dpred, const void* y3, const float* ln_gamma, const float* ln_beta,
                                             const float* w1, void* dy3, float* grads, void* workspace, int batch, int Hi, int Wi, float eps,
                                             hipStream_t st) {
    const int npix = batch * Hi * Wi, nb = tail_bwd_blocks(npix);
    float* part = reinterpret_cast<float*>(workspace);
    if (dtype == PA_BF16)
        PA_LAUNCH(tail_bwd_kernel<bf16>, dim3(nb), dim3(256), 0, st, dpred, (const bf16*)y3, ln_gamma, ln_beta, w1, (bf16*)dy3, part, Hi * Wi, npix, eps);
    else
        PA_LAUNCH(tail_bwd_kernel<float>, dim3(nb), dim3(256), 0, st, dpred, (const float*)y3, ln_gamma, ln_beta, w1, (float*)dy3, part, Hi * Wi, npix, eps);
    int e = (int)hipGetLastError();
    if (e) return e;
    return pa_slab_reduce(part, grads, TAILP, nb, TAILP, 0, st);
}

#define LIVE_NT 1024
#define LIVE_MAX_ROWS 49152
__global__ __launch_bounds__(LIVE_NT) void live_rows_kernel(const unsigned char* __restrict__ mask, int mbs, int* __restrict__ rowmap, int* __restrict__ live,
                                                            int* __restrict__ count, int Bn, int Hp, int Wp) {
    __shared__ int sc[2][LIVE_NT];
    extern __shared__ unsigned char flag[];
    const int L = Hp * Wp, n = Bn * L, per = (n + LIVE_NT - 1) / LIVE_NT;
    for (int t = threadIdx.x; t < n; t += LIVE_NT) {
        const int b = t / L, l = t - b * L, i = l / Wp, j = l - i * Wp;
        const unsigned char* m = mask + (size_t)b * mbs;
        unsigned int any = 0;
#pragma unroll
        for (int di = -1; di <= 1; ++di)
#pragma unroll
            for (int dj = -1; dj <= 1; ++dj) {
                const int ii = i + di, jj = j + dj;
                const bool in = ii >= 0 && ii < Hp && jj >= 0 && jj < Wp;
                any |= in ? (unsigned int)m[in ? ii * Wp + jj : 0] : 0u;
            }
        flag[t] = any ? 1 : 0;
    }
    __syncthreads();
    const int t0 = min(n, (int)threadIdx.x * per), t1 = min(n, t0 + per);
    int mine = 0;
    for (int t = t0; t < t1; ++t) mine += flag[t];
    sc[0][threadIdx.x] = mine;
    __syncthreads();
    int cur = 0;
    for (int d = 1; d < LIVE_NT; d <<= 1) {
        const int v = sc[cur][threadIdx.x] + ((int)threadIdx.x >= d ? sc[cur][threadIdx.x - d] : 0);
        sc[cur ^ 1][threadIdx.x] = v;
        cur ^= 1;
        __syncthreads();
    }
    int at = sc[cur][threadIdx.x] - mine;
    for (int t = t0; t < t1; ++t) {
        if (flag[t]) { rowmap[t] = at; live[at] = t; ++at; }
        else rowmap[t] = -1;
    }
    if (threadIdx.x == LIVE_NT - 1) count[0] = sc[cur][LIVE_NT - 1];
}
extern "C" int pa_live_rows_max(void) { return LIVE_MAX_ROWS; }
extern "C" int pa_live_rows(const unsigned char* mask, int mask_batch_stride, int* rowmap, int* live, int* count, int batch, int Hp, int Wp,
                            hipStream_t st) {
    if (batch < 1 || Hp < 1 || Wp < 1 || (int64_t)batch * Hp * Wp > LIVE_MAX_ROWS) return (int)hipErrorInvalidValue;
    const int n = batch * Hp * Wp;
    PA_LAUNCH(live_rows_kernel, dim3(1), dim3(LIVE_NT), (size_t)((n + 15) & ~15), st, mask, mask_batch_stride, rowmap, live, count, batch, Hp, Wp);
    LAUNCH_CHECK();
}
__global__ __launch_bounds__(256) void gather_rows_kernel(const uint4* __restrict__ src, size_t lds16, uint4* __restrict__ dst, size_t ldd16, int row16,
                                                          const int* __restrict__ live, const int* __restrict__ count) {
    const int r = blockIdx.x, cnt = *count;
    if (r >= ((cnt + 127) & ~127)) return;
    if (r < cnt && src == nullptr) return;
    const uint4* s = r < cnt ? src + (size_t)live[r] * lds16 : nullptr;
    uint4* d = dst + (size_t)r * ldd16;
    for (int c = threadIdx.x; c < row16; c += 256) d[c] = s ? s[c] : zero4();
}
extern "C" int pa_gather_rows(const void* src, int64_t src_row_bytes, void* dst, int64_t dst_row_bytes, int64_t row_bytes, const int* live,
                              const int* count, int M, hipStream_t st) {
    if (M < 1 || row_bytes % 16 || src_row_bytes % 16 || dst_row_bytes % 16 || row_bytes > dst_row_bytes || (src != nullptr && row_bytes > src_row_bytes))
        return (int)hipErrorInvalidValue;
    if (((uintptr_t)src | (uintptr_t)dst) & 15) return (int)hipErrorInvalidValue;
    const int Mp = (M + 127) / 128 * 128;
    PA_LAUNCH(gather_rows_kernel, dim3(Mp), dim3(256), 0, st, (const uint4*)src, (size_t)(src_row_bytes / 16), (uint4*)dst, (size_t)(dst_row_bytes / 16),
              (int)(row_bytes / 16), live, count);
    LAUNCH_CHECK();
}
__global__ __launch_bounds__(256) void fill_dead_rows_kernel(uint4* __restrict__ x, size_t pitch16, size_t row16, const int* __restrict__ rowmap) {
    const int r = blockIdx.x;
    if (rowmap[r] >= 0) return;
    uint4* d = x + (size_t)r * pitch16;
    for (size_t c = threadIdx.x; c < row16; c += 256) d[c] = zero4();
}
extern "C" int pa_fill_dead_rows(void* x, int64_t pitch_bytes, int64_t row_bytes, const int* rowmap, int M, hipStream_t st) {
    if (M < 1 || row_bytes % 16 || pitch_bytes % 16 || row_bytes > pitch_bytes || ((uintptr_t)x & 15)) return (int)hipErrorInvalidValue;
    PA_LAUNCH(fill_dead_rows_kernel, dim3(M), dim3(256), 0, st, (uint4*)x, (size_t)(pitch_bytes / 16), (size_t)(row_bytes / 16), rowmap);
    LAUNCH_CHECK();
}

__global__ __launch_bounds__(256) void debug_rmw_kernel(const float* __restrict__ src, float* __restrict__ scratch, size_t n4, int passes) {
    for (int p = 0; p < passes; ++p)
        for (size_t i = (size_t)blockIdx.x * blockDim.x + threadIdx.x; i < n4; i += (size_t)gridDim.x * blockDim.x) {
            const float4 a = reinterpret_cast<const float4*>(src)[i];
            float4 b = reinterpret_cast<float4*>(scratch)[i];
            b.x = 0.5f * (a.x + b.x); b.y = 0.5f * (a.y + b.y); b.z = 0.5f * (a.z + b.z); b.w = 0.5f * (a.w + b.w);
            reinterpret_cast<float4*>(scratch)[i] = b;
        }
}
extern "C" int pa_debug_rmw(const float* src, float* scratch, int64_t n, int passes, int nblocks, hipStream_t st) {
    if (n % 4 || nblocks < 1 || passes < 1) return (int)hipErrorInvalidValue;
    PA_LAUNCH(debug_rmw_kernel, dim3(nblocks), dim3(256), 0, st, src, scratch, (size_t)(n / 4), passes);
    LAUNCH_CHECK();
}
```

### painter_amd/engine.py

```python
import os
from typing import NamedTuple

import torch

from . import hostmath, ops
from ._lib import EPI_BIAS, EPI_BIAS_F32, EPI_BIAS_RESID, KNOB_RELPOS_SPLITS, KNOB_WGRAD_TARGET


_SIDE_STREAM = os.environ.get("PAINTER_AMD_SIDE_STREAM", "1") != "0"
_DBG_SERIAL = os.environ.get("PAINTER_AMD_DEBUG_SERIAL", "0") == "1"
_DBG_TRACE = os.environ.get("PAINTER_AMD_DEBUG_TRACE", "0") == "1"
_configured = False
WGRAD_SIDE_TARGET = 96
RELPOS_SIDE_SPLITS = 8


def _configure_library():
    global _configured
    if _configured:
        return
    from ._lib import lib
    lib.pa_debug_set(KNOB_RELPOS_SPLITS, RELPOS_SIDE_SPLITS if _SIDE_STREAM else 0)
    lib.pa_debug_set(KNOB_WGRAD_TARGET, WGRAD_SIDE_TARGET if _SIDE_STREAM else 0)
    _configured = True
# ... 230 lines not shown
        ws = [P["blocks.%d.attn.rel_pos_w" % k] for k in range(c.depth)]
        hd = rh.shape[1]
        for t in hs + ws:
            assert t.dtype == torch.float32 and t.is_contiguous() and t.device == rh.device and t.shape[1] == hd
        ptr = [(h.data_ptr(), w.data_ptr()) for h, w in zip(hs, ws)]
        same = bool(st) and st["dev"] == rh.device and st["ptr"] == ptr
        tabs = st["tabs"] if same else torch.tensor([q[0] for q in ptr] + [q[1] for q in ptr], dtype=torch.int64).to(rh.device)
        rcat, rcatT = ops.relpos_pack_batch(tabs, c.depth, c.Hp, c.Wp, hd, self.T, rcat=st["rcat"] if same else None, rcatT=st["rcatT"] if same else None)
        st.clear()
        st.update(dev=rh.device, ptr=ptr, ver=[(h._version, w._version) for h, w in zip(hs, ws)], tabs=tabs, rcat=rcat, rcatT=rcatT)
        return (rcatT if transposed else rcat)[i]

    def relpos_stale(self):
        st = self._rcache
        if st:
            st["ver"] = [None] * len(st["ver"])

    def invalidate(self):
        self._wcache.clear()
        self._pcache.clear()
        self._rcache.clear()

    def shadow_buffers(self):
        return {key[1]: ent[1] for key, ent in self._wcache.items()}

    def mark_fresh(self, params):
        by_ptr = {p.data_ptr(): p for p in params}
        for key, ent in list(self._wcache.items()):
            p = by_ptr.get(key[1])
            if p is not None:
                self._wcache[key] = (p._version, ent[1])

    def forward(self, P, imgs, tgts, mask_u8, valid, seg_type=None, merge_between_batch=-1, drop_scales=None, need_grad=True, want=None):
        c, T = self.cfg, self.T
        dev = imgs.device
        B = imgs.shape[0]
        L, D = c.L, c.D
        S = _Saved()
        S.B, S.need_grad = B, need_grad
        keep = lambda n: need_grad and (want is None or n in want)
        S.imgs, S.tgts, S.mask, S.valid = imgs, tgts, mask_u8, valid
        S.drop = drop_scales
        S.seg_type = seg_type if c.seggpt else None
        pe = P["pos_embed"][0, c.cls:]
        pos = ops.pos_fwd(self.pos_operator(dev)[0], pe, L, D)
        tok_args = (P["patch_embed.proj.bias"], P["mask_token"], P["segment_token_x"], P["segment_token_y"], pos, mask_u8,
                    P.get("type_token_cls") if c.seggpt else None, P.get("type_token_ins") if c.seggpt else None,
                    seg_type if c.seggpt else None)
        S.cols = None
        if ops.patch_cols_ok(T, B, L, c.P, D):
            cols = ops.patch_im2col(imgs, tgts, B, c.Hp, c.Wp, c.P)
            x = ops.patch_embed_fwd_cols(cols, self.w_patch(P), *tok_args, B, L, D)
            if keep("patch_embed.proj.weight"):
                S.cols = cols
        else:
            x = ops.patch_embed_fwd(T, imgs, tgts, self.w_patch(P), *tok_args, B, c.Hp, c.Wp, c.P, D)
        concat = torch.empty((B * L, 4 * D), dtype=T, device=dev)
        S.blocks, S.taps = [], []
        Bc = 2 * B
        for i in range(c.depth):
            pre = "blocks.%d." % i
            R = Bc * L
            merge = 0
            if c.seggpt and merge_between_batch >= 0 and i >= merge_between_batch:
                merge = 1 if c.merge_idx >= i else 2
            ds_a, ds_m = (None, None) if drop_scales is None else drop_scales[i]
            sk_a = None if merge > 0 else ds_a
            ln1, mean1, rstd1 = ops.layernorm_fwd(x, P[pre + "norm1.weight"], P[pre + "norm1.bias"], c.ln_eps, T)
            qkv = ops.linear_fwd(ln1, self.w(pre + "attn.qkv.weight", P), P[pre + "attn.qkv.bias"], EPI_BIAS, rowskip=sk_a, skip_rows_per_sample=L)
            rcat = self.relpos(pre, P, False)
            ao, lse, atab = ops.attn_fwd(qkv, rcat, Bc, L, c.heads, c.Hp, c.Wp, c.scale, need_tables=True, rowskip=sk_a) if need_grad else \
                ops.attn_fwd(qkv, rcat, Bc, L, c.heads, c.Hp, c.Wp, c.scale, rowskip=sk_a) + (None,)
            group = 0
            if merge > 0:
                a = ops.linear_fwd(ao, self.w(pre + "attn.proj.weight", P), P[pre + "attn.proj.bias"], EPI_BIAS_F32)
                group = Bc // 2 if merge == 1 else Bc
                if ds_a is None:
                    x1 = ops.ensemble_resid(x, a, Bc, group, L, D)
                else:
                    e = ops.ensemble_resid(torch.zeros_like(x), a, Bc, group, L, D)
                    x1 = ops.ensemble_resid(x, ops.scale_cast(torch.float32, e, ds_a, L), Bc, 1, L, D)
                    del e
            else:
                x1 = ops.linear_fwd(ao, self.w(pre + "attn.proj.weight", P), P[pre + "attn.proj.bias"], EPI_BIAS_RESID,
                                    resid=x, rowscale=ds_a, rows_per_sample=L, rowskip=sk_a)
            ln2, mean2, rstd2 = ops.layernorm_fwd(x1, P[pre + "norm2.weight"], P[pre + "norm2.bias"], c.ln_eps, T)
            act, gaux = ops.linear_gelu(ln2, self.w(pre + "mlp.fc1.weight", P), P[pre + "mlp.fc1.bias"], need_aux=need_grad, rowskip=ds_m, rows_per_sample=L)
            x2 = ops.linear_fwd(act, self.w(pre + "mlp.fc2.weight", P), P[pre + "mlp.fc2.bias"], EPI_BIAS_RESID,
                                resid=x1, rowscale=ds_m, rows_per_sample=L, rowskip=ds_m)
            if need_grad:
                S.blocks.append(_Block(x, mean1, rstd1, ln1, qkv, rcat, ao, lse, x1, mean2, rstd2, ln2, gaux, act, Bc, atab, group))
            x = x2
            if i == c.merge_idx:
                Bc = B
                x = ops.merge_fwd(x, B * L, D)
            if i in c.taps:
                k = c.taps.index(i)
                _, mt, rt = ops.layernorm_fwd(x, P["norm.weight"], P["norm.bias"], c.ln_eps, T, out=concat[:, k * D:(k + 1) * D])
                if need_grad:
                    S.taps.append(_Tap(x, mt, rt))
        E = ops.linear_pixshuf(concat, self.w("decoder_embed.weight", P), P["decoder_embed.bias"], B, c.Hp, c.Wp, c.P, c.dec)
        w3r, wf = ops.conv3x3_pack(P["decoder_pred.0.weight"], T)
        w1 = P["decoder_pred.3.weight"].reshape(3, c.dec)
        pred, y3 = ops.decoder_tail_fwd(E, w3r, P["decoder_pred.0.bias"], P["decoder_pred.1.weight"], P["decoder_pred.1.bias"],
                                        w1, P["decoder_pred.3.bias"], 1e-6, save_y3=need_grad)
        loss_out = ops.loss_fwd(pred, tgts, valid, mask_u8, c.P, ignore_rule=not c.seggpt,
                                eps_den=0.0 if c.seggpt else 1e-2, kind=c.loss_func)
        pred_patch = ops.patchify(pred, c.Hp, c.Wp, c.P)
        if need_grad:
            S.y3, S.pred, S.loss_out, S.wf = y3, pred, loss_out, wf
            S.concat = concat if keep("decoder_embed.weight") else None
            S.E = E if keep("decoder_pred.0.weight") else None
        return loss_out, pred, pred_patch, S

    def backward(self, P, S, dloss, sync=None, want=None, want_imgs=False, want_tgts=False, dpatch=None):
        dev = S.imgs.device
        if sync is not None:
            want = None
        side = self.side_stream(dev) if self.use_side_stream and (want is None or len(want) > 0) else None
        X = _Backward(P, S, sync, want, _Streams(torch.cuda.current_stream(dev), side))
        self.trace = []
        dconcat, dpred_loss = self._backward_decoder(X, dloss, dpatch, want_tgts)
        dx = dyT_next = None
        for i in reversed(range(self.cfg.depth)):
            dx, dyT_next = self._backward_block(X, i, dconcat, dx, dyT_next)
        dimgs, dtgts = self._backward_tokens(X, dx, dpred_loss, want_imgs, want_tgts)
        del dpred_loss
        G = X.G
        if want is not None:
            G = {n: g for n, g in G.items() if g is not None and n in want}
        X.st.join(getattr(self, "tail_probe", None))
        if sync is not None:
            sync.finish()
        if want_imgs or want_tgts:
            return G, dimgs, dtgts
        return G

    def _tr(self, name, t):
        if _DBG_TRACE:
            self.trace.append((name, t.detach().double().abs().sum()))

    def _backward_decoder(self, X, dloss, dpatch, want_tgts):
        c, T, P, S, G, st, need = self.cfg, self.T, X.P, X.S, X.G, X.st, X.need
        B = S.B
        dpred_loss = None
        if dpatch is None:
            dpred = ops.loss_bwd(S.pred, S.tgts, S.valid, S.mask, dloss, S.loss_out, c.P, c.loss_func)
            if want_tgts:
                dpred_loss = dpred
        else:
            dpred, dpred_loss = ops.pred_bwd(S.pred, S.tgts, S.valid, S.mask, dloss, S.loss_out, dpatch, c.P, c.loss_func,
                                             want_loss_term=want_tgts and dloss is not None)
        w1 = P["decoder_pred.3.weight"].reshape(3, c.dec)
        dy3, tg = ops.decoder_tail_bwd_pointwise(dpred, S.y3, P["decoder_pred.1.weight"], P["decoder_pred.1.bias"], w1, 1e-6)
        G["decoder_pred.1.weight"] = tg[0:64]
        G["decoder_pred.1.bias"] = tg[64:128]
        G["decoder_pred.3.weight"] = tg[128:320].reshape(3, c.dec, 1, 1)
        G["decoder_pred.3.bias"] = tg[320:323]
        npix = B * c.H * c.W
        if need("decoder_pred.0.weight") or need("decoder_pred.0.bias"):
            G["decoder_pred.0.weight"], G["decoder_pred.0.bias"] = st.run(
                lambda: (ops.conv3x3_wgrad(dy3, S.E) if need("decoder_pred.0.weight") else None,
                         ops.colsum(dy3.view(npix, c.dec)) if need("decoder_pred.0.bias") else None), dy3, S.E)
        w_de = self.w("decoder_embed.weight", P)
        if dpatch is None and ops.decoder_live_ok(T, B, c.Hp, c.Wp, c.P, w_de.shape[1]):
            rowmap, live, count = ops.live_rows(S.mask, B, c.Hp, c.Wp)
            st.shared(count)
            dE = ops.conv3x3_dgrad_unshuffle_live(dy3, S.wf, rowmap, count, B, c.Hp, c.Wp, c.P)
            del dy3
            X.param_grads("decoder_embed.weight", "decoder_embed.bias", dE, S.concat,
                          wgrad=lambda dy, x: ops.linear_wgrad(dy, x, live=(live, count)),
                          colsum=lambda dy, out=None: ops.colsum_live(dy, count, out=out))
            dconcat = ops.linear_dgrad(dE, w_de, live=(live, rowmap, count))
            if _DBG_TRACE:
                self._tr("dE", dE[:int(count.item())])
        else:
            dE = ops.conv3x3_dgrad_unshuffle(dy3, S.wf, B, c.Hp, c.Wp, c.P)
            del dy3
            X.param_grads("decoder_embed.weight", "decoder_embed.bias", dE, S.concat)
            dconcat = ops.linear_dgrad(dE, w_de)
            self._tr("dE", dE)
        self._tr("dconcat", dconcat)
        del dE
        X.ready(["decoder_embed.weight", "decoder_embed.bias"])
        X.ready([n for n in G if n.startswith("decoder_pred.")])
        return dconcat, dpred_loss

    def block_flat(self, X, i):
        if i not in X.flats:
            D = self.cfg.D
            sizes = [2 * D, 2 * D, 3 * D, D, self.cfg.hidden, D, X.rc_shape[0] * X.rc_shape[1]]
            fb = X.st.shared(torch.empty((sum(sizes),), dtype=torch.float32, device=X.S.imgs.device))
            X.flats[i] = (fb, dict(zip(("n1", "n2", "qkv", "proj", "fc1", "fc2", "rel"), torch.split(fb, sizes))))
        return X.flats[i]

    def _backward_block(self, X, i, dconcat, dx, dyT_next):
        c, T, P, S, G, st, need = self.cfg, self.T, X.P, X.S, X.G, X.st, X.need
        B, L, D = S.B, c.L, c.D
        dev = S.imgs.device
        tr = self._tr
        pre = "blocks.%d." % i
        b = S.blocks[i]
        S.blocks[i] = None
        R = b.Bc * L
        ds_a, ds_m = (None, None) if S.drop is None else S.drop[i]
        sk_a = None if b.group > 0 else ds_a
        nrp, hd = X.rc_shape
        flat, fl = self.block_flat(X, i)
        del X.flats[i]
        if i in c.taps:
            k = c.taps.index(i)
            tap = S.taps[k]
            dyT = torch.empty((R, D), dtype=T, device=dev)
            dx, gb = ops.layernorm_bwd(dconcat[:, k * D:(k + 1) * D], tap.x, tap.mean, tap.rstd, P["norm.weight"], dres=dx, dx=dx, dxT=dyT,
                                       rowscale=ds_m, rows_per_sample=L, dxT_colsum=fl["fc2"])
            G[pre + "mlp.fc2.bias"] = fl["fc2"]
            if need("norm.weight") or need("norm.bias"):
                X.dnorm = gb if X.dnorm is None else _add_(X.dnorm, gb)
        elif i == c.merge_idx:
            dx, dyT = ops.merge_bwd(T, dx, ds_m, L, B * L, D)
        else:
            dyT = dyT_next
        X.param_grads(pre + "mlp.fc2.weight", pre + "mlp.fc2.bias", dyT, b.act, fl["fc2"])
        tr("%d.dyT" % i, dyT)
        dpre = ops.linear_dgrad(dyT, self.w(pre + "mlp.fc2.weight", P), gelu_aux=b.gaux, colsum_out=fl["fc1"], rowskip=ds_m, rows_per_sample=L)
        G[pre + "mlp.fc1.bias"] = fl["fc1"]
        tr("%d.dpre" % i, dpre)
        X.param_grads(pre + "mlp.fc1.weight", pre + "mlp.fc1.bias", dpre, b.ln2, fl["fc1"])
        dln2 = ops.linear_dgrad(dpre, self.w(pre + "mlp.fc1.weight", P), rowskip=ds_m, rows_per_sample=L)
        tr("%d.dln2" % i, dln2)
        del dpre
        dyA = st.private(dyT)
        lnws, lndone = self.ln_workspace(dev, ops.layernorm_bwd_workspace_bytes(R, D), st.main, st.side)
        dx, fin = ops.layernorm_bwd(dln2, b.x1, b.mean2, b.rstd2, P[pre + "norm2.weight"], dres=dx, dx=dx, dxT=dyA,
                                    rowscale=ds_a, rows_per_sample=L, gb=fl["n2"].view(2, D), dxT_colsum=fl["proj"], defer=True, ws=lnws)
        gb = None
        if need(pre + "norm2.weight") or need(pre + "norm2.bias") or need(pre + "attn.proj.bias"):
            gb = st.run(fin)
            lndone()
            G[pre + "norm2.weight"], G[pre + "norm2.bias"] = gb[0], gb[1]
        G[pre + "attn.proj.bias"] = fl["proj"]
        del dyT
        tr("%d.dx_ln2" % i, dx); tr("%d.dyA" % i, dyA)
        if gb is not None:
            tr("%d.gb2" % i, gb)
        if b.group > 0:
            da = ops.ensemble_resid(torch.zeros_like(dx), dx if ds_a is None else ops.scale_cast(torch.float32, dx, ds_a, L), b.Bc, b.group, L, D)
            dyA = da if T == torch.float32 else ops.cast_bf16(da, out=dyA)
            del da
        X.param_grads(pre + "attn.proj.weight", pre + "attn.proj.bias", dyA, b.ao, fl["proj"])
        dao = ops.linear_dgrad(dyA, self.w(pre + "attn.proj.weight", P), out=dln2, rowskip=sk_a, rows_per_sample=L)
        tr("%d.dao" % i, dao)
        del dyA
        rcatT = self.relpos(pre, P, True)
        dqkv, dG = ops.attn_bwd_core(b.qkv, b.rcat, rcatT, b.ao, dao, b.lse, b.Bc, L, c.heads, c.Hp, c.Wp, c.scale, tables=b.atab, rowskip=sk_a)
        if need(pre + "attn.rel_pos_h") or need(pre + "attn.rel_pos_w"):
            drcat = st.run(lambda: ops.attn_bwd_relpos(dG, b.qkv, nrp, b.Bc, L, c.heads, c.Hp, c.Wp, out=fl["rel"].view(nrp, hd)), dG, b.qkv)
            nh, nw = 2 * c.Hp - 1, 2 * c.Wp - 1
            G[pre + "attn.rel_pos_h"] = drcat[:nh]
            G[pre + "attn.rel_pos_w"] = drcat[nh:nh + nw]
        del dG
        tr("%d.dqkv" % i, dqkv)
        X.param_grads(pre + "attn.qkv.weight", pre + "attn.qkv.bias", dqkv, b.ln1, fl["qkv"])
        dln1 = ops.linear_dgrad(dqkv, self.w(pre + "attn.qkv.weight", P), out=dao, rowskip=sk_a, rows_per_sample=L)
        del dqkv
        nxt = i - 1
        if nxt >= 0 and nxt not in c.taps and nxt != c.merge_idx:
            dyT_next = torch.empty((R, D), dtype=T, device=dev)
        else:
            dyT_next = None
        ds_next = None if (S.drop is None or nxt < 0) else S.drop[nxt][1]
        cs_next = None
        if dyT_next is not None:
            cs_next = self.block_flat(X, nxt)[1]["fc2"]
            G["blocks.%d.mlp.fc2.bias" % nxt] = cs_next
        lnws, lndone = self.ln_workspace(dev, ops.layernorm_bwd_workspace_bytes(R, D), st.main, st.side)
        dx, fin = ops.layernorm_bwd(dln1, b.x, b.mean1, b.rstd1, P[pre + "norm1.weight"], dres=dx, dx=dx, dxT=dyT_next,
                                    rowscale=ds_next if dyT_next is not None else None, rows_per_sample=L, gb=fl["n1"].view(2, D),
                                    dxT_colsum=cs_next, defer=True, ws=lnws)
        if need(pre + "norm1.weight") or need(pre + "norm1.bias") or (cs_next is not None and need("blocks.%d.mlp.fc2.bias" % nxt)):
            gb = st.run(fin)
            lndone()
            G[pre + "norm1.weight"], G[pre + "norm1.bias"] = gb[0], gb[1]
        tr("%d.dx_ln1" % i, dx)
        del b
        X.ready([n for n in G if n.startswith(pre)], flat=flat)
        return dx, dyT_next

    def _backward_tokens(self, X, dx, dpred_loss, want_imgs, want_tgts):
        c, T, P, S, G, need = self.cfg, self.T, X.P, X.S, X.G, X.need
        B, L, D = S.B, c.L, c.D
        if X.dnorm is not None:
            G["norm.weight"], G["norm.bias"] = X.dnorm[0], X.dnorm[1]
        dpe, sums = ops.tokens_bwd(T, dx, S.mask, B, L, D)
        if need("patch_embed.proj.weight"):
            if S.cols is not None:
                G["patch_embed.proj.weight"] = ops.linear_wgrad(dpe, S.cols).view(D, 3, c.P, c.P)
            else:
                G["patch_embed.proj.weight"] = ops.patch_embed_wgrad(dpe, S.imgs, S.tgts, B, c.Hp, c.Wp, c.P, D).view(D, 3, c.P, c.P)
        if need("patch_embed.proj.bias"):
            G["patch_embed.proj.bias"] = ops.colsum(dpe)
        if need("pos_embed"):
            dposemb = torch.zeros_like(P["pos_embed"])
            ops.pos_bwd(self.pos_operator(S.imgs.device)[1], sums[0], sums[1], dposemb[0, c.cls:], c.src * c.src, D)
            G["pos_embed"] = dposemb
        for k_, nm in enumerate(("segment_token_x", "segment_token_y", "mask_token")):
            if need(nm):
                G[nm] = ops.colsum(sums[k_]).view(1, 1, 1, D)
        small_tail = []
        if c.seggpt and S.seg_type is not None and (need("type_token_cls") or need("type_token_ins")):
            types_present = set(S.seg_type.reshape(-1).tolist())
            for t_, nm in ((0.0, "type_token_cls"), (1.0, "type_token_ins")):
                if (t_ not in types_present and X.sync is None) or not need(nm):
                    continue
                w = (S.seg_type.reshape(-1) == t_).to(torch.float32)
                sel = ops.scale_cast(torch.float32, dx, torch.cat((w, w)).contiguous(), L)
                G[nm] = ops.colsum(sel).view(1, 1, 1, D)
                small_tail.append(nm)
        X.ready(["norm.weight", "norm.bias", "patch_embed.proj.weight", "patch_embed.proj.bias", "pos_embed",
                 "segment_token_x", "segment_token_y", "mask_token"] + small_tail)
        if not (want_imgs or want_tgts):
            return None, None
        return ops.patch_embed_dgrad(dpe, self.w_patch(P), B, c.Hp, c.Wp, c.P, D, want_imgs, want_tgts,
                                     addend=dpred_loss if want_tgts else None, alpha=-1.0)

def _add_(a, b):
    from ._lib import check, lib
    check(lib.pa_slab_reduce(b.data_ptr(), a.data_ptr(), a.numel(), 1, a.numel(), 1, ops.stream()), "pa_slab_reduce")
    return a
```

### painter_amd/ops.py

```python
import torch

from ._lib import (EPI_BIAS, EPI_BIAS_F32, EPI_BIAS_GELU, EPI_BIAS_RESID, KNOB_DECODER_ROWS, KNOB_DROP_SKIP, PA_BF16, PA_F32, check, lib)

_WS = {}


def stream():
    return torch.cuda.current_stream().cuda_stream


def code(dtype):
    if dtype == torch.bfloat16:
        return PA_BF16
    if dtype == torch.float32:
        return PA_F32
    raise TypeError("painter_amd supports float32 / bfloat16 operand types, got %s" % dtype)


def p(t):
    return 0 if t is None else t.data_ptr()


def workspace(nbytes, device, slot=0):
    key = (device, slot, torch.cuda.current_stream(device).cuda_stream)
# ... 151 lines not shown
def live_rows(mask_u8, batch, Hp, Wp):
    n = batch * Hp * Wp
    assert mask_u8.dtype in (torch.uint8, torch.bool) and mask_u8.is_cuda and mask_u8.stride(-1) == 1 and mask_u8.shape[-1] == Hp * Wp
    assert mask_u8.shape[0] in (1, batch)
    buf = torch.empty((2 * n + 1,), dtype=torch.int32, device=mask_u8.device)
    rowmap, live, count = buf[:n], buf[n:2 * n], buf[2 * n:]
    check(lib.pa_live_rows(p(mask_u8), _mbs(mask_u8), p(rowmap), p(live), p(count), batch, Hp, Wp, stream()), "pa_live_rows")
    return rowmap, live, count


def padded_rows(n):
    return (n + 127) // 128 * 128


def conv3x3_dgrad_unshuffle_live(dy3, wf, rowmap, count, batch, Hp, Wp, P, out=None):
    assert dy3.dtype == torch.bfloat16
    if out is None:
        out = torch.empty((padded_rows(batch * Hp * Wp), P * P * 64), dtype=dy3.dtype, device=dy3.device)
    assert out.shape == (padded_rows(batch * Hp * Wp), P * P * 64) and out.is_contiguous()
    check(lib.pa_conv3x3_dgrad_unshuffle_live(p(dy3), p(wf), p(out), p(rowmap), p(count), batch, Hp, Wp, P, stream()),
          "pa_conv3x3_dgrad_unshuffle_live")
    return out


def gather_rows(x, live, count, out=None):
    M, N = x.shape
    _req(x)
    if out is None:
        out = torch.empty((padded_rows(M), N), dtype=x.dtype, device=x.device)
    es = x.element_size()
    check(lib.pa_gather_rows(p(x), x.stride(0) * es, p(out), out.stride(0) * es, N * es, p(live), p(count), M, stream()), "pa_gather_rows")
    return out


def linear_wgrad_live(dy, x, count, out=None):
    M, N = dy.shape
    K = x.shape[1]
    _req(dy, torch.bfloat16); _req(x, torch.bfloat16)
    assert x.shape[0] == M and M % 128 == 0
    if out is None:
        out = torch.empty((N, K), dtype=torch.float32, device=dy.device)
    check(lib.pa_linear_wgrad_live(p(dy), dy.stride(0), p(x), x.stride(0), p(out), p(count), M, N, K, stream()), "pa_linear_wgrad_live")
    return out


def colsum_live(x, count, out=None):
    M, N = x.shape
    if out is None:
        out = torch.empty((N,), dtype=torch.float32, device=x.device)
    ws = workspace(lib.pa_colsum_workspace_bytes(M, N), x.device)
    check(lib.pa_colsum_live(code(x.dtype), p(x), x.stride(0), M, N, p(out), p(ws), p(count), stream()), "pa_colsum_live")
    return out


def layernorm_fwd(x, gamma, beta, eps, out_dtype, out=None):
    R, D = x.shape
    _req(x, torch.float32)
    if out is None:
        out = torch.empty((R, D), dtype=out_dtype, device=x.device)
    mean = torch.empty((R,), dtype=torch.float32, device=x.device)
    rstd = torch.empty((R,), dtype=torch.float32, device=x.device)
    check(lib.pa_layernorm_fwd(code(out.dtype), p(x), x.stride(0), p(gamma), p(beta), eps, p(out), out.stride(0),
                               p(mean), p(rstd), R, D, stream()), "pa_layernorm_fwd")
    return out, mean, rstd


def layernorm_bwd_workspace_bytes(R, D):
    return int(lib.pa_layernorm_bwd_workspace_bytes(R, D))


def layernorm_bwd(dy, x, mean, rstd, gamma, dres=None, dx=None, dxT=None, rowscale=None, rows_per_sample=1, gb=None, dxT_colsum=None, defer=False, ws=None):
    R, D = x.shape
    if dx is None:
        dx = torch.empty((R, D), dtype=torch.float32, device=x.device)
    if gb is None:
        gb = torch.empty((2, D), dtype=torch.float32, device=x.device)
    assert gb.shape == (2, D) and gb.is_contiguous() and gb.dtype == torch.float32
    nbytes = lib.pa_layernorm_bwd_workspace_bytes(R, D)
    if defer:
        if ws is None:
            ws = torch.empty((nbytes,), dtype=torch.uint8, device=x.device)
        assert ws.dtype == torch.uint8 and ws.numel() >= nbytes and ws.is_contiguous()
    else:
        ws = workspace(nbytes, x.device)
    if dxT_colsum is not None:
        assert dxT is not None and dxT_colsum.shape == (D,) and dxT_colsum.dtype == torch.float32 and dxT_colsum.is_contiguous()
    check(lib.pa_layernorm_bwd(code(dy.dtype), p(dy), dy.stride(0), p(x), x.stride(0), p(mean), p(rstd), p(gamma),
                               p(dres), p(dx), dx.stride(0), p(dxT), 0 if dxT is None else dxT.stride(0), p(rowscale),
                               rows_per_sample, 0 if defer else p(gb), p(dxT_colsum), p(ws), R, D, stream()), "pa_layernorm_bwd")
    if not defer:
        return dx, gb

    def finish():
        check(lib.pa_layernorm_bwd_reduce(p(ws), p(gb), p(dxT_colsum), int(dxT_colsum is not None), R, D, stream()), "pa_layernorm_bwd_reduce")
        return gb
    finish.buffer = ws
    return dx, finish


def relpos_pack(rel_pos_h, rel_pos_w, Hp, Wp, dtype):
    nrp = lib.pa_relpos_rows_padded(Hp, Wp)
    hd = rel_pos_h.shape[1]
    assert rel_pos_h.shape == (2 * Hp - 1, hd) and rel_pos_w.shape == (2 * Wp - 1, hd)
    rcat = torch.empty((nrp, hd), dtype=dtype, device=rel_pos_h.device)
    check(lib.pa_relpos_pack(code(dtype), p(rel_pos_h), p(rel_pos_w), p(rcat), Hp, Wp, hd, stream()), "pa_relpos_pack")
    return rcat


def relpos_pack_batch(tabs, nblocks, Hp, Wp, hd, dtype, rcat=None, rcatT=None):
    nrp = lib.pa_relpos_rows_padded(Hp, Wp)
    assert tabs.dtype == torch.int64 and tabs.numel() == 2 * nblocks and tabs.is_cuda and tabs.is_contiguous()
    if rcat is None:
        rcat = torch.empty((nblocks, nrp, hd), dtype=dtype, device=tabs.device)
    if rcatT is None:
        rcatT = torch.empty((nblocks, hd, nrp), dtype=dtype, device=tabs.device)
    assert rcat.shape == (nblocks, nrp, hd) and rcatT.shape == (nblocks, hd, nrp) and rcat.is_contiguous() and rcatT.is_contiguous()
    assert rcat.dtype == dtype and rcatT.dtype == dtype
    check(lib.pa_relpos_pack_batch(code(dtype), p(tabs), p(rcat), p(rcatT), nblocks, Hp, Wp, hd, stream()), "pa_relpos_pack_batch")
    return rcat, rcatT


def attn_fwd(qkv, rcat, batch, L, heads, Hp, Wp, scale, need_tables=False, *, rowskip=None):
    T = qkv.dtype
    hd = rcat.shape[1]
    assert qkv.shape[1] == 3 * heads * hd
    out = torch.empty((batch * L, heads * hd), dtype=T, device=qkv.device)
    lse = torch.empty((batch * heads, L), dtype=torch.float32, device=qkv.device)
    tables = None
    if need_tables:
        nb = lib.pa_attn_tables_bytes(code(T), batch, L, heads, Hp, Wp, hd)
        if nb > 0:
            tables = torch.empty((nb,), dtype=torch.uint8, device=qkv.device)
    check(lib.pa_attn_fwd_skip(code(T), p(qkv), qkv.stride(0), p(rcat), p(out), out.stride(0), p(lse), p(tables), batch, L, heads,
                               Hp, Wp, hd, float(scale), _skip_args(rowskip, 1, batch)[0], stream()), "pa_attn_fwd_skip")
    return (out, lse, tables) if need_tables else (out, lse)


def attn_launch_counts():
    import ctypes
    buf = (ctypes.c_longlong * 6)()
    check(lib.pa_attn_launch_counts(ctypes.addressof(buf)), "pa_attn_launch_counts")
    v = [int(x) for x in buf]
    return {"fwd": tuple(v[:3]), "bwd": tuple(v[3:])}


def relpos_pack_t(rel_pos_h, rel_pos_w, Hp, Wp, dtype):
    nrp = lib.pa_relpos_rows_padded(Hp, Wp)
    hd = rel_pos_h.shape[1]
    rcatT = torch.empty((hd, nrp), dtype=dtype, device=rel_pos_h.device)
    check(lib.pa_relpos_pack_t(code(dtype), p(rel_pos_h), p(rel_pos_w), p(rcatT), Hp, Wp, hd, stream()), "pa_relpos_pack_t")
    return rcatT


def attn_bwd_core(qkv, rcat, rcatT, out, dout, lse, batch, L, heads, Hp, Wp, scale, tables=None, prep="fused", *, rowskip=None):
    T = qkv.dtype
    dev = qkv.device
    nrp, hd = rcat.shape
    delta = None
    o_arg = None
    if tables is not None and lib.pa_attn_bwd_prep_ok(code(T), L, Hp, Wp, hd):
        if prep == "fused":
            o_arg = out
        else:
            check(lib.pa_attn_bwd_prep(code(T), p(out), out.stride(0), p(dout), dout.stride(0), p(lse), p(tables), batch, L, heads, Hp, Wp, hd,
                                       float(scale), stream()), "pa_attn_bwd_prep")
    else:
        delta = torch.empty((batch * heads, L), dtype=torch.float32, device=dev)
        check(lib.pa_attn_bwd_delta(code(T), p(out), out.stride(0), p(dout), dout.stride(0), p(delta), batch, L, heads, hd,
                                    stream()), "pa_attn_bwd_delta")
    dqkv = torch.empty_like(qkv)
    nb = lib.pa_attn_bwd_relpos_partials_bytes(code(T), batch, L, heads, Hp, Wp, hd) if tables is not None else 0
    dG = part = None
    if nb > 0:
        part = torch.empty((nb,), dtype=torch.uint8, device=dev)
    else:
        dG = torch.empty((batch * L, heads * nrp), dtype=T, device=dev)
    aux = workspace(lib.pa_attn_bwd_aux_bytes(batch, L, heads, Hp, Wp), dev, slot=1)
    check(lib.pa_attn_bwd_skip(code(T), p(qkv), qkv.stride(0), p(rcat), p(rcatT), p(dout), dout.stride(0), p(lse), p(delta),
                               p(dqkv), p(dG), p(part), p(aux), p(tables), p(o_arg), 0 if o_arg is None else o_arg.stride(0), batch, L, heads, Hp, Wp,
                               hd, float(scale), _skip_args(rowskip, 1, batch)[0], stream()), "pa_attn_bwd_skip")
    return dqkv, (dG if part is None else part)


def attn_bwd_relpos(dG, qkv, nrp, batch, L, heads, Hp, Wp, out=None):
    T = qkv.dtype
    hd = qkv.shape[1] // (3 * heads)
    drcat = out if out is not None else torch.empty((nrp, hd), dtype=torch.float32, device=qkv.device)
    assert drcat.shape == (nrp, hd) and drcat.is_contiguous()
    ws = workspace(lib.pa_attn_bwd_relpos_workspace_bytes(code(T), batch, L, heads, Hp, Wp, hd), qkv.device)
    if dG.dtype == torch.uint8:
        check(lib.pa_attn_bwd_relpos_reduce(p(dG), p(drcat), p(ws), batch, L, heads, Hp, Wp, hd, stream()), "pa_attn_bwd_relpos_reduce")
        return drcat
    check(lib.pa_attn_bwd_relpos(code(T), p(dG), p(qkv), qkv.stride(0), p(drcat), p(ws), batch, L, heads, Hp, Wp, hd,
                                 stream()), "pa_attn_bwd_relpos")
    return drcat


def attn_bwd(qkv, rcat, rcatT, out, dout, lse, batch, L, heads, Hp, Wp, scale, tables=None):
    dqkv, dG = attn_bwd_core(qkv, rcat, rcatT, out, dout, lse, batch, L, heads, Hp, Wp, scale, tables=tables)
    return dqkv, attn_bwd_relpos(dG, qkv, rcat.shape[0], batch, L, heads, Hp, Wp)


def cast_bf16(x, out=None):
    if out is None:
        out = torch.empty(x.shape, dtype=torch.bfloat16, device=x.device)
    check(lib.pa_cast_bf16(p(x), p(out), x.numel(), stream()), "pa_cast_bf16")
    return out


def pos_fwd(op, pe, L, D):
    idx, val = op
    assert idx.dtype == torch.int32 and val.dtype == torch.float32 and idx.shape == val.shape == (L, idx.shape[1])
    pos = torch.empty((L, D), dtype=torch.float32, device=pe.device)
    check(lib.pa_pos_fwd(p(idx), p(val), idx.shape[1], p(pe), p(pos), L, D, stream()), "pa_pos_fwd")
    return pos


def pos_bwd(opT, gx, gy, dpe, S, D):
    idx, val = opT
    assert idx.dtype == torch.int32 and val.dtype == torch.float32 and idx.shape == val.shape == (S, idx.shape[1])
    check(lib.pa_pos_bwd(p(idx), p(val), idx.shape[1], p(gx), p(gy), p(dpe), S, D, stream()), "pa_pos_bwd")


def patch_weight_pack(w, T, P, out=None):
    D = w.shape[0]
    kp = (3 * P * P + 7) // 8 * 8
    if out is None:
        out = torch.empty((D, kp), dtype=T, device=w.device)
    check(lib.pa_patch_weight_pack(code(T), p(w), p(out), D, P, stream()), "pa_patch_weight_pack")
    return out


def patch_embed_fwd(T, imgs, tgts, w, bias, mask_token, seg_x, seg_y, pos, mask_u8, type_cls, type_ins, seg_type,
                    batch, Hp, Wp, P, D):
    tokens = torch.empty((2 * batch * Hp * Wp, D), dtype=torch.float32, device=imgs.device)
    assert w.dtype == T and w.shape[0] == D and w.stride(1) == 1
    check(lib.pa_patch_embed_fwd(code(T), p(imgs), p(tgts), p(w), w.stride(0), p(bias), p(mask_token), p(seg_x), p(seg_y), p(pos),
                                 p(mask_u8), _mbs(mask_u8), p(type_cls), p(type_ins), p(seg_type), p(tokens), batch, Hp, Wp, P, D,
                                 stream()), "pa_patch_embed_fwd")
    return tokens


def patch_cols_ok(T, batch, L, P, D):
    return T == torch.bfloat16 and bool(lib.pa_patch_cols_ok(batch, L, P, D))


def patch_im2col(imgs, tgts, batch, Hp, Wp, P):
    cols = torch.empty((2 * batch * Hp * Wp, 3 * P * P), dtype=torch.bfloat16, device=imgs.device)
    check(lib.pa_patch_im2col(p(imgs), p(tgts), p(cols), batch, Hp, Wp, P, stream()), "pa_patch_im2col")
    return cols


def patch_embed_fwd_cols(cols, w, bias, mask_token, seg_x, seg_y, pos, mask_u8, type_cls, type_ins, seg_type, batch, L, D):
    tokens = torch.empty((2 * batch * L, D), dtype=torch.float32, device=cols.device)
    assert w.dtype == torch.bfloat16 and w.shape[0] == D and w.stride(1) == 1 and cols.is_contiguous()
    check(lib.pa_patch_embed_fwd_cols(p(cols), p(w), w.stride(0), p(bias), p(mask_token), p(seg_x), p(seg_y), p(pos), p(mask_u8), _mbs(mask_u8),
                                      p(type_cls), p(type_ins), p(seg_type), p(tokens), batch, L, cols.shape[1], D, stream()), "pa_patch_embed_fwd_cols")
    return tokens


def patch_embed_wgrad(dpe, imgs, tgts, batch, Hp, Wp, P, D):
    dw = torch.empty((D, 3 * P * P), dtype=torch.float32, device=dpe.device)
    ws = workspace(lib.pa_patch_embed_wgrad_workspace_bytes(D, P), dpe.device)
    check(lib.pa_patch_embed_wgrad(code(dpe.dtype), p(dpe), p(imgs), p(tgts), p(dw), p(ws), batch, Hp, Wp, P, D, stream()),
          "pa_patch_embed_wgrad")
    return dw


def patch_embed_dgrad(dpe, w, batch, Hp, Wp, P, D, want_imgs=True, want_tgts=True, addend=None, alpha=-1.0):
    T = dpe.dtype
    assert dpe.shape == (2 * batch * Hp * Wp, D) and dpe.is_contiguous() and w.dtype == T and w.shape[0] == D and w.stride(1) == 1
    shape = (batch, 3, Hp * P, Wp * P)
    dimgs = torch.empty(shape, dtype=torch.float32, device=dpe.device) if want_imgs else None
    dtgts = torch.empty(shape, dtype=torch.float32, device=dpe.device) if want_tgts else None
    if addend is not None:
        assert want_tgts and addend.shape == shape and addend.dtype == torch.float32 and addend.is_contiguous()
    check(lib.pa_patch_embed_dgrad(code(T), p(dpe), p(w), w.stride(0), p(dimgs), p(dtgts), p(addend), float(alpha), batch, Hp, Wp, P, D,
                                   stream()), "pa_patch_embed_dgrad")
    return dimgs, dtgts


def tokens_bwd(T, dx0, mask_u8, batch, L, D):
    dpe = torch.empty((2 * batch * L, D), dtype=T, device=dx0.device)
    sums = torch.empty((3, L, D), dtype=torch.float32, device=dx0.device)
    check(lib.pa_tokens_bwd(code(T), p(dx0), p(mask_u8), _mbs(mask_u8), p(dpe), p(sums), batch, L, D, stream()), "pa_tokens_bwd")
    return dpe, sums


def merge_fwd(x, rows_out, D):
    out = torch.empty((rows_out, D), dtype=torch.float32, device=x.device)
    check(lib.pa_merge_fwd(p(x), p(out), rows_out * D, stream()), "pa_merge_fwd")
    return out


def merge_bwd(T, dmerged, rowscale, rps, rows_half, D):
    dx = torch.empty((2 * rows_half, D), dtype=torch.float32, device=dmerged.device)
    dxT = torch.empty((2 * rows_half, D), dtype=T, device=dmerged.device)
    check(lib.pa_merge_bwd(code(T), p(dmerged), p(dx), p(dxT), p(rowscale), rps, rows_half, D, stream()), "pa_merge_bwd")
    return dx, dxT


def scale_cast(T, x, rowscale, rps, out=None):
    rows, D = x.shape
    if out is None:
        out = torch.empty((rows, D), dtype=T, device=x.device)
    check(lib.pa_scale_cast(code(T), p(x), p(out), p(rowscale), rps, rows, D, stream()), "pa_scale_cast")
    return out


def ensemble_resid(x0, a, batch, group, L, D):
    x1 = torch.empty_like(x0)
    check(lib.pa_ensemble_resid(p(x0), p(a), p(x1), batch, group, L, D, stream()), "pa_ensemble_resid")
    return x1


def conv3x3_pack(w3, T):
    w3r = torch.empty((64, 9, 64), dtype=T, device=w3.device)
    wf = torch.empty((64, 9, 64), dtype=T, device=w3.device)
    check(lib.pa_conv3x3_pack(code(T), p(w3), p(w3r), p(wf), stream()), "pa_conv3x3_pack")
    return w3r, wf


def decoder_tail_fwd(x_nhwc, w3r, b3, gamma, beta, w1, b1, eps, save_y3=True):
    B, Hi, Wi, C = x_nhwc.shape
    T = x_nhwc.dtype
    y3 = torch.empty((B, Hi, Wi, C), dtype=T, device=x_nhwc.device) if save_y3 else None
    pred = torch.empty((B, 3, Hi, Wi), dtype=torch.float32, device=x_nhwc.device)
    check(lib.pa_decoder_tail_fwd(code(T), p(x_nhwc), p(w3r), p(b3), p(gamma), p(beta), p(w1), p(b1), p(y3), p(pred), B, Hi, Wi,
                                  float(eps), stream()), "pa_decoder_tail_fwd")
    return pred, y3


def decoder_tail_bwd_pointwise(dpred, y3, gamma, beta, w1, eps):
    B, Hi, Wi, C = y3.shape
    T = y3.dtype
    dy3 = torch.empty_like(y3)
    grads = torch.empty((324,), dtype=torch.float32, device=y3.device)
    ws = workspace(lib.pa_decoder_tail_bwd_workspace_bytes(B, Hi, Wi), y3.device)
    check(lib.pa_decoder_tail_bwd_pointwise(code(T), p(dpred), p(y3), p(gamma), p(beta), p(w1), p(dy3), p(grads), p(ws), B, Hi, Wi,
                                            float(eps), stream()), "pa_decoder_tail_bwd_pointwise")
    return dy3, grads


def conv3x3_dgrad_unshuffle(dy3, wf, batch, Hp, Wp, P):
    T = dy3.dtype
    dE = torch.empty((batch * Hp * Wp, P * P * 64), dtype=T, device=dy3.device)
    check(lib.pa_conv3x3_dgrad_unshuffle(code(T), p(dy3), p(wf), p(dE), batch, Hp, Wp, P, stream()), "pa_conv3x3_dgrad_unshuffle")
    return dE


def conv3x3_wgrad(dy3, x_nhwc):
    B, Hi, Wi, C = x_nhwc.shape
    dw = torch.empty((64, 64, 3, 3), dtype=torch.float32, device=dy3.device)
    ws = workspace(lib.pa_conv3x3_wgrad_workspace_bytes(B, Hi, Wi), dy3.device)
    check(lib.pa_conv3x3_wgrad(code(dy3.dtype), p(dy3), p(x_nhwc), p(dw), p(ws), B, Hi, Wi, stream()), "pa_conv3x3_wgrad")
    return dw


LOSS_KINDS = {"smoothl1": 0, "l1": 1, "l2": 2, "l1l2": 3}


def loss_fwd(pred, tgts, valid, mask_u8, P, ignore_rule, eps_den, kind, beta=0.01):
    B, _, Hi, Wi = pred.shape
    out = torch.empty((2,), dtype=torch.float32, device=pred.device)
    ws = workspace(lib.pa_loss_workspace_bytes(B, Hi, Wi), pred.device)
    check(lib.pa_loss_fwd(p(pred), p(tgts), p(valid), p(mask_u8), _mbs(mask_u8), p(out), p(ws), B, Hi, Wi, P, int(ignore_rule),
                          float(eps_den), LOSS_KINDS[kind], float(beta), stream()), "pa_loss_fwd")
    return out


def loss_bwd(pred, tgts, valid, mask_u8, dloss, loss_out, P, kind, beta=0.01):
    B, _, Hi, Wi = pred.shape
    dpred = torch.empty_like(pred)
    check(lib.pa_loss_bwd(p(pred), p(tgts), p(valid), p(mask_u8), _mbs(mask_u8), p(dloss), p(loss_out), p(dpred), B, Hi, Wi, P,
                          LOSS_KINDS[kind], float(beta), stream()), "pa_loss_bwd")
    return dpred


def pred_bwd(pred, tgts, valid, mask_u8, dloss, loss_out, dpatch, P, kind, want_loss_term=False, beta=0.01):
    B, _, Hi, Wi = pred.shape
    dpred = torch.empty_like(pred)
    dpred_loss = torch.empty_like(pred) if want_loss_term else None
    if dpatch is not None:
        assert dpatch.shape == (B, (Hi // P) * (Wi // P), 3 * P * P) and dpatch.dtype == torch.float32 and dpatch.is_contiguous()
    check(lib.pa_pred_bwd(p(pred), p(tgts), p(valid), p(mask_u8), _mbs(mask_u8), p(dloss), p(loss_out), p(dpatch), p(dpred), p(dpred_loss), B, Hi, Wi,
                          P, LOSS_KINDS[kind], float(beta), stream()), "pa_pred_bwd")
    return dpred, dpred_loss


def patchify(pred, Hp, Wp, P):
    B = pred.shape[0]
    out = torch.empty((B, Hp * Wp, P * P * 3), dtype=torch.float32, device=pred.device)
    check(lib.pa_patchify(p(pred), p(out), B, Hp, Wp, P, stream()), "pa_patchify")
    return out
```

Before: 164.2 images/sec.

## Fuse qkv-bias and decoder conv-bias gradient column sums into producing backward kernels

The attention backward dq and dkv kernels now compute per-block column sums of their staged dqkv tiles into a partials buffer. A combined param-reduce kernel then produces both the relpos table gradient and the qkv bias gradient in one launch. The decoder tail pointwise backward also emits the column sum of dy3 for the conv bias gradient. Together these replace separate colsum passes over large gradient tensors, at the cost of extra LDS, a few syncthreads per block and a larger partials buffer.

```diff
diff --git a/include/painter_hip.h b/include/painter_hip.h
--- a/include/painter_hip.h
+++ b/include/painter_hip.h
@@ -93,6 +93,8 @@
 int64_t pa_attn_bwd_relpos_workspace_bytes(int dtype, int batch, int L, int heads, int Hp, int Wp, int head_dim);
 int pa_attn_bwd_relpos_reduce(const void* relpos_part, float* drcat, void* workspace, int batch, int L, int heads, int Hp, int Wp,
                               int head_dim, hipStream_t stream);
+int pa_attn_bwd_param_reduce(const void* relpos_part, float* drcat, float* dqkv_bias, void* workspace, int batch, int L, int heads,
+                             int Hp, int Wp, int head_dim, hipStream_t stream);
 int pa_attn_bwd_relpos(int dtype, const void* dG, const void* qkv, int64_t ldq, float* drcat, void* workspace,
                        int batch, int L, int heads, int Hp, int Wp, int head_dim, hipStream_t stream);
 
@@ -138,6 +140,10 @@
 int pa_decoder_tail_bwd_pointwise(int dtype, const float* dpred, const void* y3, const float* ln_gamma,
                                   const float* ln_beta, const float* w1, void* dy3, float* grads, void* workspace,
                                   int batch, int Hi, int Wi, float eps, hipStream_t stream);
+int64_t pa_decoder_tail_bwd_cs_workspace_bytes(int batch, int Hi, int Wi);
+int pa_decoder_tail_bwd_pointwise_cs(int dtype, const float* dpred, const void* y3, const float* ln_gamma,
+                                     const float* ln_beta, const float* w1, void* dy3, float* grads, float* dy3_colsum,
+                                     void* workspace, int batch, int Hi, int Wi, float eps, hipStream_t stream);
 int pa_conv3x3_dgrad_unshuffle(int dtype, const void* dy3, const void* wf, void* dE, int batch, int Hp, int Wp, int P,
                                hipStream_t stream);
 int64_t pa_conv3x3_wgrad_workspace_bytes(int batch, int Hi, int Wi);
diff --git a/painter_amd/csrc/attn3.h b/painter_amd/csrc/attn3.h
--- a/painter_amd/csrc/attn3.h
+++ b/painter_amd/csrc/attn3.h
@@ -11,3 +11,4 @@
                    float scale, hipStream_t st);
 int64_t attn3_relpos_partials_bytes(int Bn, int L, int H, int Hp, int Wp);
 int attn3_relpos_reduce(const float* part, float* drcat, float* tmp, int Bn, int L, int H, int Hp, int Wp, hipStream_t st);
+int attn3_param_reduce(const float* part, float* drcat, float* bias, float* tmp, int Bn, int L, int H, int Hp, int Wp, hipStream_t st);
diff --git a/painter_amd/csrc/attn3.hip b/painter_amd/csrc/attn3.hip
--- a/painter_amd/csrc/attn3.hip
+++ b/painter_amd/csrc/attn3.hip
@@ -180,13 +180,20 @@
 
 __device__ unsigned long long g_trace[2 * 2 * 64 * 8];
 constexpr int NSMAX = 12;
+__host__ __device__ inline int dq_lds_bytes(int Hp, int NRP, bool fuse) {
+    const int a = 2 * STAGE_QK + NW * Hp * 64 + PH * EIMG + ATT_HD * (NRP * 2 + 16);
+    const int b = fuse ? NW * ((NRP + 63) / 64 + 1) * IMG : 0;
+    return a > b ? a : b;
+}
+constexpr int DQ_BSUM_BYTES = NW * ATT_HD * 4;
 template <int MINW, bool NDL, bool TR = false, bool FUSE = false>
 __global__ __launch_bounds__(NT, MINW) void bwd_dq_kernel(const bf16* __restrict__ qkv, size_t ldq, const bf16* __restrict__ rcatT,
                                                           const bf16* __restrict__ dout, size_t lddo, const float* __restrict__ lse,
                                                           unsigned char* __restrict__ tables, bf16* __restrict__ dqkv,
                                                           bf16* __restrict__ dG, float* __restrict__ part, int L, int H, int Hp, int NRP,
                                                           float scale, int nblk, int xcd_map, int abl, int tile0, int pslot0,
-                                                          const bf16* __restrict__ oatt, size_t ldo, const float* __restrict__ rowskip) {
+                                                          const bf16* __restrict__ oatt, size_t ldo, const float* __restrict__ rowskip,
+                                                          float* __restrict__ bpart) {
     extern __shared__ __attribute__((aligned(16))) unsigned char smem[];
     const int tid = threadIdx.x, lane = tid & 63, wave = tid >> 6, g = lane >> 5, ql = lane & 31;
     const int trwg = blockIdx.x == 0 ? 0 : (blockIdx.x == gridDim.x / 2 ? 1 : -1);
@@ -224,6 +231,7 @@
         if constexpr (FUSE) {
             float4* pw = reinterpret_cast<float4*>(part + (size_t)(pslot0 + pslot) * NRP * ATT_HD);
             for (int c = tid; c < NRP * ATT_HD / 4; c += NT) pw[c] = make_float4(0.f, 0.f, 0.f, 0.f);
+            if (tid < ATT_HD) bpart[((size_t)bh * nblk + blk) * (3 * ATT_HD) + tid] = 0.f;
         }
         return;
     }
@@ -485,7 +493,10 @@
         if (!(abl & 4)) write_rows(stg, dqkv + (size_t)(b * L + qt * 32) * ldq + h * ATT_HD, ldq, lane);
     }
     if constexpr (FUSE) {
+        float (*bsum)[ATT_HD] = reinterpret_cast<float (*)[ATT_HD]>(smem + dq_lds_bytes(Hp, NRP, true));
+        bsum[wave][lane] = valid ? colsum_rows(stg, lane) : 0.f;
         __syncthreads();
+        if (wave == 0) bpart[((size_t)bh * nblk + blk) * (3 * ATT_HD) + lane] = ((bsum[0][lane] + bsum[1][lane]) + bsum[2][lane]) + bsum[3][lane];
         const int nimg = (NRP + 63) >> 6;
         unsigned char* wimg = smem + wave * (nimg + 1) * IMG;
         if (valid) {
@@ -519,11 +530,12 @@
 }
 
 constexpr int DKV_TW = 2 * IMG, DKV_TH = DKV_TW + 2048, DKV_ND = DKV_TH + 512, DKV_STAGE = DKV_ND + 128;
+constexpr int DKV_LDS = 2 * DKV_STAGE > NW * 2 * IMG ? 2 * DKV_STAGE : NW * 2 * IMG, DKV_BSUM_BYTES = 2 * NW * ATT_HD * 4;
 template <int MINW>
 __global__ __launch_bounds__(NT, MINW) void bwd_dkv_kernel(const bf16* __restrict__ qkv, size_t ldq, const bf16* __restrict__ dout,
                                                            size_t lddo, const unsigned char* __restrict__ tables, bf16* __restrict__ dqkv,
                                                            int L, int H, int Hp, float scale, int nblk, int xcd_map, int abl, int tile0,
-                                                           const float* __restrict__ rowskip) {
+                                                           const float* __restrict__ rowskip, float* __restrict__ bpart) {
     extern __shared__ __attribute__((aligned(16))) unsigned char smem[];
     const int tid = threadIdx.x, lane = tid & 63, wave = tid >> 6, g = lane >> 5, ql = lane & 31;
     int blk, bh;
@@ -541,6 +553,7 @@
             zero_rows(orow + D, ldq, lane);
             zero_rows(orow + 2 * D, ldq, lane);
         }
+        if (bpart != nullptr && tid < 2 * ATT_HD) bpart[((size_t)bh * nblk + blk) * (3 * ATT_HD) + ATT_HD + tid] = 0.f;
         return;
     }
     const int key = kt * 32 + ql;
@@ -694,6 +707,15 @@
         write_rows(stg, orow + D, ldq, lane);
         write_rows(stg + IMG, orow + 2 * D, ldq, lane);
     }
+    if (bpart != nullptr) {
+        float (*bsum)[NW][ATT_HD] = reinterpret_cast<float (*)[NW][ATT_HD]>(smem + DKV_LDS);
+        bsum[0][wave][lane] = valid ? colsum_rows(stg, lane) : 0.f;
+        bsum[1][wave][lane] = valid ? colsum_rows(stg + IMG, lane) : 0.f;
+        __syncthreads();
+        if (wave < 2)
+            bpart[((size_t)bh * nblk + blk) * (3 * ATT_HD) + (1 + wave) * ATT_HD + lane] =
+                ((bsum[wave][0][lane] + bsum[wave][1][lane]) + bsum[wave][2][lane]) + bsum[wave][3][lane];
+    }
 }
 
 __global__ void prep_kernel(const float* __restrict__ lse, const float* __restrict__ delta, unsigned char* __restrict__ tables, int L, int Hp,
@@ -802,10 +824,10 @@
 
 namespace a3 {
 constexpr int RED_ZC = 32;
-__global__ __launch_bounds__(256) void relpos_part_reduce_kernel(const float4* __restrict__ part, float4* __restrict__ tmp, int n4, int nz) {
+DEVI void relpos_part_reduce(const float4* __restrict__ part, float4* __restrict__ tmp, int n4, int nz, int zc) {
     __shared__ float4 sh[4][64];
     const int c = blockIdx.x * 64 + (threadIdx.x & 63), zl = threadIdx.x >> 6;
-    const int z0 = (int)((int64_t)nz * blockIdx.y / gridDim.y), z1 = (int)((int64_t)nz * (blockIdx.y + 1) / gridDim.y);
+    const int z0 = (int)((int64_t)nz * blockIdx.y / zc), z1 = (int)((int64_t)nz * (blockIdx.y + 1) / zc);
     float4 s = make_float4(0, 0, 0, 0);
     if (c < n4) {
 #pragma unroll 4
@@ -823,6 +845,40 @@
         tmp[(size_t)blockIdx.y * n4 + c] = t;
     }
 }
+__global__ __launch_bounds__(256) void relpos_part_reduce_kernel(const float4* __restrict__ part, float4* __restrict__ tmp, int n4, int nz) {
+    relpos_part_reduce(part, tmp, n4, nz, gridDim.y);
+}
+__global__ __launch_bounds__(256) void param_reduce_kernel(const float4* __restrict__ part, float4* __restrict__ tmp, int n4, int nz, int zc,
+                                                           const float* __restrict__ bpart, float* __restrict__ bias, int Bn, int H, int nblk) {
+    if ((int)blockIdx.y < zc) {
+        relpos_part_reduce(part, tmp, n4, nz, zc);
+        return;
+    }
+    __shared__ float tile[64][ATT_HD];
+    const int lane = threadIdx.x & 63, zl = threadIdx.x >> 6, nt = Bn * nblk;
+    for (int ph = blockIdx.x; ph < 3 * H; ph += gridDim.x) {
+        const int pt = ph / H, h = ph - pt * H;
+        const float* src = bpart + (size_t)pt * ATT_HD + lane;
+        float s = 0.f;
+        for (int t0 = 0; t0 < nt; t0 += 64) {
+            float v[16];
+#pragma unroll
+            for (int k = 0; k < 16; ++k) {
+                const int t = min(t0 + zl + 4 * k, nt - 1), b = t / nblk;
+                v[k] = src[((size_t)(b * H + h) * nblk + (t - b * nblk)) * (3 * ATT_HD)];
+            }
+#pragma unroll
+            for (int k = 0; k < 16; ++k) tile[zl + 4 * k][lane] = v[k];
+            __syncthreads();
+            if (zl == 0) {
+                const int n = min(64, nt - t0);
+                for (int j = 0; j < n; ++j) s += tile[j][lane];
+            }
+            __syncthreads();
+        }
+        if (zl == 0) bias[pt * (H * ATT_HD) + h * ATT_HD + lane] = s;
+    }
+}
 }
 extern "C" int pa_slab_reduce(const float* in, float* out, int64_t n, int nz, int64_t stride, int accumulate, hipStream_t st);
 static int a3_fuse_on() {
@@ -835,7 +891,7 @@
     if (!a3_fuse_on() || !attn3_ok(L, Hp, Wp)) return 0;
     const int NRP = pa_relpos_rows_padded(Hp, Wp);
     if (NRP > 16 * a3::NSMAX) return 0;
-    return a3_num_partials(Bn, L, H, Hp, Wp) * NRP * ATT_HD * sizeof(float);
+    return a3_num_partials(Bn, L, H, Hp, Wp) * (NRP + 3) * ATT_HD * sizeof(float);
 }
 int attn3_relpos_reduce(const float* part, float* drcat, float* tmp, int Bn, int L, int H, int Hp, int Wp, hipStream_t st) {
     using namespace a3;
@@ -846,6 +902,18 @@
               reinterpret_cast<float4*>(tmp), n4, nz);
     if (int e = (int)hipGetLastError()) return e;
     return pa_slab_reduce(tmp, drcat, (int64_t)n4 * 4, zc, (int64_t)n4 * 4, 0, st);
+}
+
+int attn3_param_reduce(const float* part, float* drcat, float* bias, float* tmp, int Bn, int L, int H, int Hp, int Wp, hipStream_t st) {
+    using namespace a3;
+    const int NRP = pa_relpos_rows_padded(Hp, Wp);
+    const int nz = (int)a3_num_partials(Bn, L, H, Hp, Wp), n4 = NRP * ATT_HD / 4;
+    const int zc = drcat == nullptr ? 0 : (nz < RED_ZC ? nz : RED_ZC);
+    if (zc == 0 && bias == nullptr) return 0;
+    PA_LAUNCH(param_reduce_kernel, dim3((n4 + 63) / 64, zc + (bias != nullptr ? 1 : 0)), dim3(256), 0, st, reinterpret_cast<const float4*>(part),
+              reinterpret_cast<float4*>(tmp), n4, nz, zc, part + (size_t)nz * NRP * ATT_HD, bias, Bn, H, a3_blocks(L));
+    if (int e = (int)hipGetLastError()) return e;
+    return zc == 0 ? 0 : pa_slab_reduce(tmp, drcat, (int64_t)n4 * 4, zc, (int64_t)n4 * 4, 0, st);
 }
 
 int attn3_bwd(const bf16* qkv, int64_t ldq, const bf16* rcatT, const bf16* dout, int64_t lddo, const float* lse, const float* delta,
@@ -865,36 +933,32 @@
     }
     const int tile0 = 0;
     const int nblk = a3_blocks(L);
+    float* bpart = part != nullptr ? part + (size_t)a3_num_partials(Bn, L, H, Hp, Wp) * NRP * ATT_HD : nullptr;
     static const int dq_w = [] { const char* v = getenv("PA_ATTN3_DQ_WAVES"); return v ? atoi(v) : 2; }();
     static const int dkv_w = [] { const char* v = getenv("PA_ATTN3_DKV_WAVES"); return v ? atoi(v) : 2; }();
     if (nblk > 0) {
         static const size_t pad = [] { const char* v = getenv("PA_ATTN3_LDS_PAD"); return v ? (size_t)atoi(v) : (size_t)0; }();
-        size_t smem = 2 * (size_t)STAGE_QK + (size_t)NW * Hp * 64 + PH * EIMG + (size_t)ATT_HD * (NRP * 2 + 16) + pad;
         const bool fuse = part != nullptr;
-        if (fuse) {
-            const size_t need = (size_t)NW * ((NRP + 63) / 64 + 1) * IMG;
-            if (smem < need) smem = need;
-        }
+        const size_t smem = (size_t)dq_lds_bytes(Hp, NRP, fuse) + (fuse ? DQ_BSUM_BYTES : 0) + pad;
         auto kern = fuse ? bwd_dq_kernel<2, A3_NDL, false, true>
                          : (g_attn_trace ? bwd_dq_kernel<2, true, true> : (dq_w == 3 ? bwd_dq_kernel<3, false> : bwd_dq_kernel<2, A3_NDL>));
         static bool done2 = false, done3 = false, donet = false, donef = false;
         if ((e = set_smem(reinterpret_cast<const void*>(kern), fuse ? donef : (g_attn_trace ? donet : (dq_w == 3 ? done3 : done2))))) return e;
         const char* ablv = getenv("PA_ATTN3_DQ_ABL");
         PA_LAUNCH(kern, dim3(nblk * Bn * H), dim3(NT), smem, st, qkv, (size_t)ldq, rcatT, dout, (size_t)lddo, lse, tb, dqkv, dG, part, L, H,
-                  Hp, NRP, scale, nblk, a3_xcd_map_on(), ablv ? atoi(ablv) : 0, tile0, 0, delta == nullptr ? out : nullptr, (size_t)ldo, rowskip);
+                  Hp, NRP, scale, nblk, a3_xcd_map_on(), ablv ? atoi(ablv) : 0, tile0, 0, delta == nullptr ? out : nullptr, (size_t)ldo, rowskip, bpart);
         if ((e = (int)hipGetLastError())) return e;
     }
     const int tile0_kv = 0, nblk_kv = a3_blocks(L);
     if (nblk_kv > 0) {
-        size_t smem = 2 * (size_t)DKV_STAGE;
-        if (smem < (size_t)NW * 2 * IMG) smem = (size_t)NW * 2 * IMG;
+        size_t smem = (size_t)DKV_LDS + DKV_BSUM_BYTES;
         static const size_t pad = [] { const char* v = getenv("PA_ATTN3_LDS_PAD"); return v ? (size_t)atoi(v) : (size_t)0; }();
         smem += pad;
         auto kern = dkv_w == 3 ? bwd_dkv_kernel<3> : bwd_dkv_kernel<2>;
         static bool done2 = false, done3 = false;
         if ((e = set_smem(reinterpret_cast<const void*>(kern), dkv_w == 3 ? done3 : done2))) return e;
         PA_LAUNCH(kern, dim3(nblk_kv * Bn * H), dim3(NT), smem, st, qkv, (size_t)ldq, dout, (size_t)lddo, tb, dqkv, L, H, Hp, scale, nblk_kv,
-                  a3_xcd_map_on(), [] { const char* v = getenv("PA_ATTN3_DKV_ABL"); return v ? atoi(v) : 0; }(), tile0_kv, rowskip);
+                  a3_xcd_map_on(), [] { const char* v = getenv("PA_ATTN3_DKV_ABL"); return v ? atoi(v) : 0; }(), tile0_kv, rowskip, bpart);
         if ((e = (int)hipGetLastError())) return e;
     }
     return 0;
diff --git a/painter_amd/csrc/attn_bwd.hip b/painter_amd/csrc/attn_bwd.hip
--- a/painter_amd/csrc/attn_bwd.hip
+++ b/painter_amd/csrc/attn_bwd.hip
@@ -613,6 +613,11 @@
     if (head_dim != ATT_HD || relpos_part == nullptr || attn3_relpos_partials_bytes(batch, L, heads, Hp, Wp) == 0) return (int)hipErrorInvalidValue;
     return attn3_relpos_reduce((const float*)relpos_part, drcat, (float*)workspace, batch, L, heads, Hp, Wp, st);
 }
+extern "C" int pa_attn_bwd_param_reduce(const void* relpos_part, float* drcat, float* dqkv_bias, void* workspace, int batch, int L, int heads,
+                                        int Hp, int Wp, int head_dim, hipStream_t st) {
+    if (head_dim != ATT_HD || relpos_part == nullptr || attn3_relpos_partials_bytes(batch, L, heads, Hp, Wp) == 0) return (int)hipErrorInvalidValue;
+    return attn3_param_reduce((const float*)relpos_part, drcat, dqkv_bias, (float*)workspace, batch, L, heads, Hp, Wp, st);
+}
 extern "C" int pa_attn_bwd_relpos(int dtype, const void* dG, const void* qkv, int64_t ldq, float* drcat, void* workspace, int batch, int L,
                                   int heads, int Hp, int Wp, int head_dim, hipStream_t st) {
     if (head_dim <= 0 || head_dim % 16) return (int)hipErrorInvalidValue;
diff --git a/painter_amd/csrc/attn_tile.h b/painter_amd/csrc/attn_tile.h
--- a/painter_amd/csrc/attn_tile.h
+++ b/painter_amd/csrc/attn_tile.h
@@ -147,6 +147,13 @@
     }
 }
 
+DEVI float colsum_rows(const unsigned char* stg, int lane) {
+    float s = 0.f;
+#pragma unroll
+    for (int r = 0; r < 32; ++r) s += (float)*reinterpret_cast<const bf16*>(stg + r * 128 + lane * 2);
+    return s;
+}
+
 DEVI void zero_rows(bf16* dst, size_t ld, int lane) {
 #pragma unroll
     for (int i = 0; i < 4; ++i) {
diff --git a/painter_amd/csrc/elementwise.hip b/painter_amd/csrc/elementwise.hip
--- a/painter_amd/csrc/elementwise.hip
+++ b/painter_amd/csrc/elementwise.hip
@@ -2,6 +2,7 @@
 #include "../../include/painter_hip.h"
 
 extern "C" int pa_slab_reduce(const float* in, float* out, int64_t n, int nz, int64_t stride, int accumulate, hipStream_t st);
+int pa_slab_reduce2(const float* in, float* out0, float* out1, int64_t n0, int64_t n, int nz, int64_t stride, hipStream_t st);
 
 __global__ void cast_bf16_kernel(const float* __restrict__ in, bf16* __restrict__ out, size_t n) {
     size_t i = ((size_t)blockIdx.x * blockDim.x + threadIdx.x) * 4;
@@ -339,7 +340,7 @@
 
 #define TAILP 324
 DEVI float oct_sum(float v) { v = quad_sum(v); v += lane_dpp<0x141>(v); return v; }
-template <typename T>
+template <typename T, bool CS = false>
 __global__ __launch_bounds__(256) void tail_bwd_kernel(const float* __restrict__ dpred, const T* __restrict__ y3, const float* __restrict__ gamma,
                                                        const float* __restrict__ beta, const float* __restrict__ w1, T* __restrict__ dy3,
                                                        float* __restrict__ part, int HW, int npix, float eps) {
@@ -358,6 +359,8 @@
     f32x2_t ag[4] = {zero2, zero2, zero2, zero2}, ab[4] = {zero2, zero2, zero2, zero2};
     f32x2_t aw[3][4] = {{zero2, zero2, zero2, zero2}, {zero2, zero2, zero2, zero2}, {zero2, zero2, zero2, zero2}};
     float ab1[3] = {0.f, 0.f, 0.f};
+    f32x2_t ar[4] = {zero2, zero2, zero2, zero2};
+    constexpr int NP = CS ? TAILP + 64 : TAILP;
     const int stride = gridDim.x * 32;
     struct In { uint4 a, b; float d0, d1, d2; };
     struct Pos { int pix, b, rem; };
@@ -443,15 +446,23 @@
 #pragma unroll
         for (int k = 0; k < 4; ++k) r[k] = rs2 * (__builtin_elementwise_fma(y[k], nm2, dxh[k]) - mm1);
         if constexpr (sizeof(T) == 2) {
-            *reinterpret_cast<uint4*>(dy3 + (size_t)pix * 64 + c0) = make_uint4(pack_bf16x2(r[0][0], r[0][1]), pack_bf16x2(r[1][0], r[1][1]),
-                                                                                 pack_bf16x2(r[2][0], r[2][1]), pack_bf16x2(r[3][0], r[3][1]));
+            const uint4 o = make_uint4(pack_bf16x2(r[0][0], r[0][1]), pack_bf16x2(r[1][0], r[1][1]), pack_bf16x2(r[2][0], r[2][1]), pack_bf16x2(r[3][0], r[3][1]));
+            *reinterpret_cast<uint4*>(dy3 + (size_t)pix * 64 + c0) = o;
+            if constexpr (CS) {
+                ar[0] = ar[0] + (f32x2_t){bf16_lo(o.x), bf16_hi(o.x)}; ar[1] = ar[1] + (f32x2_t){bf16_lo(o.y), bf16_hi(o.y)};
+                ar[2] = ar[2] + (f32x2_t){bf16_lo(o.z), bf16_hi(o.z)}; ar[3] = ar[3] + (f32x2_t){bf16_lo(o.w), bf16_hi(o.w)};
+            }
         } else {
+            if constexpr (CS) {
+#pragma unroll
+                for (int k = 0; k < 4; ++k) ar[k] = ar[k] + r[k];
+            }
             *reinterpret_cast<float4*>(dy3 + (size_t)pix * 64 + c0) = make_float4(r[0][0], r[0][1], r[1][0], r[1][1]);
             *reinterpret_cast<float4*>(dy3 + (size_t)pix * 64 + c0 + 4) = make_float4(r[2][0], r[2][1], r[3][0], r[3][1]);
         }
     }
     auto wsum = [&](float v) { v += lane_dpp<0x128>(v); v += lane_xor16(v); v += lane_xor32(v); return v; };
-    __shared__ float red[4][TAILP];
+    __shared__ float red[4][NP];
 #pragma unroll
     for (int k = 0; k < 4; ++k)
 #pragma unroll
@@ -461,13 +472,17 @@
                 const int c = c0 + 2 * k + e;
                 red[wave][c] = vg; red[wave][64 + c] = vb; red[wave][128 + c] = v0; red[wave][192 + c] = v1; red[wave][256 + c] = v2;
             }
+            if constexpr (CS) {
+                const float vr = wsum(ar[k][e]);
+                if (lane < 8) red[wave][TAILP + c0 + 2 * k + e] = vr;
+            }
         }
     {
         const float t0 = wsum(ab1[0]), t1 = wsum(ab1[1]), t2 = wsum(ab1[2]);
         if (lane == 0) { red[wave][320] = t0; red[wave][321] = t1; red[wave][322] = t2; red[wave][323] = 0.f; }
     }
     __syncthreads();
-    for (int i = threadIdx.x; i < TAILP; i += 256) part[(size_t)blockIdx.x * TAILP + i] = (red[0][i] + red[1][i]) + (red[2][i] + red[3][i]);
+    for (int i = threadIdx.x; i < NP; i += 256) part[(size_t)blockIdx.x * NP + i] = (red[0][i] + red[1][i]) + (red[2][i] + red[3][i]);
 }
 static int tail_bwd_blocks(int npix) {
     int b = (npix + 31) / 32;
@@ -487,6 +502,23 @@
     if (e) return e;
     return pa_slab_reduce(part, grads, TAILP, nb, TAILP, 0, st);
 }
+extern "C" int64_t pa_decoder_tail_bwd_cs_workspace_bytes(int batch, int Hi, int Wi) {
+    return (int64_t)tail_bwd_blocks(batch * Hi * Wi) * (TAILP + 64) * sizeof(float);
+}
+extern "C" int pa_decoder_tail_bwd_pointwise_cs(int dtype, const float* dpred, const void* y3, const float* ln_gamma, const float* ln_beta,
+                                                const float* w1, void* dy3, float* grads, float* dy3_colsum, void* workspace, int batch, int Hi, int Wi,
+                                                float eps, hipStream_t st) {
+    const int npix = batch * Hi * Wi, nb = tail_bwd_blocks(npix), NP = TAILP + 64;
+    if (dy3_colsum == nullptr) return (int)hipErrorInvalidValue;
+    float* part = reinterpret_cast<float*>(workspace);
+    if (dtype == PA_BF16)
+        PA_LAUNCH((tail_bwd_kernel<bf16, true>), dim3(nb), dim3(256), 0, st, dpred, (const bf16*)y3, ln_gamma, ln_beta, w1, (bf16*)dy3, part, Hi * Wi, npix, eps);
+    else
+        PA_LAUNCH((tail_bwd_kernel<float, true>), dim3(nb), dim3(256), 0, st, dpred, (const float*)y3, ln_gamma, ln_beta, w1, (float*)dy3, part, Hi * Wi, npix, eps);
+    int e = (int)hipGetLastError();
+    if (e) return e;
+    return pa_slab_reduce2(part, grads, dy3_colsum, TAILP, NP, nb, NP, st);
+}
 
 #define LIVE_NT 1024
 #define LIVE_MAX_ROWS 49152
diff --git a/painter_amd/engine.py b/painter_amd/engine.py
--- a/painter_amd/engine.py
+++ b/painter_amd/engine.py
@@ -406,16 +406,19 @@
             dpred, dpred_loss = ops.pred_bwd(S.pred, S.tgts, S.valid, S.mask, dloss, S.loss_out, dpatch, c.P, c.loss_func,
                                              want_loss_term=want_tgts and dloss is not None)
         w1 = P["decoder_pred.3.weight"].reshape(3, c.dec)
-        dy3, tg = ops.decoder_tail_bwd_pointwise(dpred, S.y3, P["decoder_pred.1.weight"], P["decoder_pred.1.bias"], w1, 1e-6)
+        cs3 = torch.empty((c.dec,), dtype=torch.float32, device=S.y3.device) if T == torch.bfloat16 and c.dec == 64 else None
+        dy3, tg = ops.decoder_tail_bwd_pointwise(dpred, S.y3, P["decoder_pred.1.weight"], P["decoder_pred.1.bias"], w1, 1e-6, colsum_out=cs3)
         G["decoder_pred.1.weight"] = tg[0:64]
         G["decoder_pred.1.bias"] = tg[64:128]
         G["decoder_pred.3.weight"] = tg[128:320].reshape(3, c.dec, 1, 1)
         G["decoder_pred.3.bias"] = tg[320:323]
         npix = B * c.H * c.W
-        if need("decoder_pred.0.weight") or need("decoder_pred.0.bias"):
+        if need("decoder_pred.0.weight") or (cs3 is None and need("decoder_pred.0.bias")):
             G["decoder_pred.0.weight"], G["decoder_pred.0.bias"] = st.run(
                 lambda: (ops.conv3x3_wgrad(dy3, S.E) if need("decoder_pred.0.weight") else None,
-                         ops.colsum(dy3.view(npix, c.dec)) if need("decoder_pred.0.bias") else None), dy3, S.E)
+                         ops.colsum(dy3.view(npix, c.dec)) if cs3 is None and need("decoder_pred.0.bias") else None), dy3, S.E)
+        if cs3 is not None:
+            G["decoder_pred.0.bias"] = cs3
         w_de = self.w("decoder_embed.weight", P)
         if dpatch is None and ops.decoder_live_ok(T, B, c.Hp, c.Wp, c.P, w_de.shape[1]):
             rowmap, live, count = ops.live_rows(S.mask, B, c.Hp, c.Wp)
@@ -508,11 +511,18 @@
         del dyA
         rcatT = self.relpos(pre, P, True)
         dqkv, dG = ops.attn_bwd_core(b.qkv, b.rcat, rcatT, b.ao, dao, b.lse, b.Bc, L, c.heads, c.Hp, c.Wp, c.scale, tables=b.atab, rowskip=sk_a)
-        if need(pre + "attn.rel_pos_h") or need(pre + "attn.rel_pos_w"):
-            drcat = st.run(lambda: ops.attn_bwd_relpos(dG, b.qkv, nrp, b.Bc, L, c.heads, c.Hp, c.Wp, out=fl["rel"].view(nrp, hd)), dG, b.qkv)
-            nh, nw = 2 * c.Hp - 1, 2 * c.Wp - 1
-            G[pre + "attn.rel_pos_h"] = drcat[:nh]
-            G[pre + "attn.rel_pos_w"] = drcat[nh:nh + nw]
+        want_rel = need(pre + "attn.rel_pos_h") or need(pre + "attn.rel_pos_w")
+        bias_fused = dG.dtype == torch.uint8
+        want_qb = bias_fused and need(pre + "attn.qkv.bias")
+        if want_rel or want_qb:
+            drcat = st.run(lambda: ops.attn_bwd_relpos(dG, b.qkv, nrp, b.Bc, L, c.heads, c.Hp, c.Wp, out=fl["rel"].view(nrp, hd),
+                                                       bias_out=fl["qkv"] if want_qb else None, want_tables=want_rel), dG, b.qkv)
+            if want_rel:
+                nh, nw = 2 * c.Hp - 1, 2 * c.Wp - 1
+                G[pre + "attn.rel_pos_h"] = drcat[:nh]
+                G[pre + "attn.rel_pos_w"] = drcat[nh:nh + nw]
+        if want_qb:
+            G[pre + "attn.qkv.bias"] = fl["qkv"]
         del dG
         tr("%d.dqkv" % i, dqkv)
         X.param_grads(pre + "attn.qkv.weight", pre + "attn.qkv.bias", dqkv, b.ln1, fl["qkv"])
diff --git a/painter_amd/ops.py b/painter_amd/ops.py
--- a/painter_amd/ops.py
+++ b/painter_amd/ops.py
@@ -327,7 +327,7 @@
     return rcatT
 
 
-def attn_bwd_core(qkv, rcat, rcatT, out, dout, lse, batch, L, heads, Hp, Wp, scale, tables=None, prep="fused", *, rowskip=None):
+def attn_bwd_core(qkv, rcat, rcatT, out, dout, lse, batch, L, heads, Hp, Wp, scale, tables=None, prep="fused", *, rowskip=None, part=None):
     T = qkv.dtype
     dev = qkv.device
     nrp, hd = rcat.shape
@@ -345,10 +345,13 @@
                                     stream()), "pa_attn_bwd_delta")
     dqkv = torch.empty_like(qkv)
     nb = lib.pa_attn_bwd_relpos_partials_bytes(code(T), batch, L, heads, Hp, Wp, hd) if tables is not None else 0
-    dG = part = None
+    dG = None
     if nb > 0:
-        part = torch.empty((nb,), dtype=torch.uint8, device=dev)
+        if part is None:
+            part = torch.empty((nb,), dtype=torch.uint8, device=dev)
+        assert part.dtype == torch.uint8 and part.numel() == nb and part.is_contiguous()
     else:
+        part = None
         dG = torch.empty((batch * L, heads * nrp), dtype=T, device=dev)
     aux = workspace(lib.pa_attn_bwd_aux_bytes(batch, L, heads, Hp, Wp), dev, slot=1)
     check(lib.pa_attn_bwd_skip(code(T), p(qkv), qkv.stride(0), p(rcat), p(rcatT), p(dout), dout.stride(0), p(lse), p(delta),
@@ -357,9 +360,20 @@
     return dqkv, (dG if part is None else part)
 
 
-def attn_bwd_relpos(dG, qkv, nrp, batch, L, heads, Hp, Wp, out=None):
+def attn_bwd_relpos(dG, qkv, nrp, batch, L, heads, Hp, Wp, out=None, bias_out=None, want_tables=True):
     T = qkv.dtype
     hd = qkv.shape[1] // (3 * heads)
+    if bias_out is not None:
+        if dG.dtype != torch.uint8:
+            raise ValueError("attn_bwd_relpos: bias_out needs the partials of the generation-3 backward")
+        assert bias_out.dtype == torch.float32 and bias_out.shape == (3 * heads * hd,) and bias_out.is_contiguous()
+        drcat = None
+        if want_tables:
+            drcat = out if out is not None else torch.empty((nrp, hd), dtype=torch.float32, device=qkv.device)
+            assert drcat.shape == (nrp, hd) and drcat.is_contiguous()
+        ws = workspace(lib.pa_attn_bwd_relpos_workspace_bytes(code(T), batch, L, heads, Hp, Wp, hd), qkv.device)
+        check(lib.pa_attn_bwd_param_reduce(p(dG), p(drcat), p(bias_out), p(ws), batch, L, heads, Hp, Wp, hd, stream()), "pa_attn_bwd_param_reduce")
+        return drcat
     drcat = out if out is not None else torch.empty((nrp, hd), dtype=torch.float32, device=qkv.device)
     assert drcat.shape == (nrp, hd) and drcat.is_contiguous()
     ws = workspace(lib.pa_attn_bwd_relpos_workspace_bytes(code(T), batch, L, heads, Hp, Wp, hd), qkv.device)
@@ -506,11 +520,17 @@
     return pred, y3
 
 
-def decoder_tail_bwd_pointwise(dpred, y3, gamma, beta, w1, eps):
+def decoder_tail_bwd_pointwise(dpred, y3, gamma, beta, w1, eps, colsum_out=None):
     B, Hi, Wi, C = y3.shape
     T = y3.dtype
     dy3 = torch.empty_like(y3)
     grads = torch.empty((324,), dtype=torch.float32, device=y3.device)
+    if colsum_out is not None:
+        assert colsum_out.dtype == torch.float32 and colsum_out.shape == (C,) and C == 64 and colsum_out.is_contiguous()
+        ws = workspace(lib.pa_decoder_tail_bwd_cs_workspace_bytes(B, Hi, Wi), y3.device)
+        check(lib.pa_decoder_tail_bwd_pointwise_cs(code(T), p(dpred), p(y3), p(gamma), p(beta), p(w1), p(dy3), p(grads), p(colsum_out), p(ws),
+                                                   B, Hi, Wi, float(eps), stream()), "pa_decoder_tail_bwd_pointwise_cs")
+        return dy3, grads
     ws = workspace(lib.pa_decoder_tail_bwd_workspace_bytes(B, Hi, Wi), y3.device)
     check(lib.pa_decoder_tail_bwd_pointwise(code(T), p(dpred), p(y3), p(gamma), p(beta), p(w1), p(dy3), p(grads), p(ws), B, Hi, Wi,
                                             float(eps), stream()), "pa_decoder_tail_bwd_pointwise")
```

Measured after the change: 164.2 images/sec (median of 4 runs). No clear change (-0.0%).
